# dayoladejo/GADMM

Measured on AMD Instinct MI355X. Metric: wall-clock to 1e-8 objective gap, GADMM linear regression (LinearRegression_Synthetic), lower is better.
Workload: dtype fp64; 1 GPU; model=LinearRegression_Synthetic GADMM closed-form, workers=24, features=50, samples_per_worker=50, global_batch=1200, seq_len=1, parallelism=chain24-over-1gpu

## Files before the change

csrc/kernels/chain_blocked.hip:

```cpp
#include "gadmm_common.h"
#include "gadmm_chain.h"
#include "persist_device.h"
#include "persist_launch.h"
#include <stdlib.h>

namespace {

constexpr int MAXW = 12;
constexpr int HIMG52 = 4 * 64 * 14;
constexpr int EPL = 256;
constexpr long DYN_LDS_BYTES = (long)MAXW * EPL * (16 + 8 + 4);
struct EpochLds {
  int4* sl;
  int2* fl;
  int* st;
};
__device__ __forceinline__ EpochLds epoch_lds(double* base, int v) {
  int4* sl = reinterpret_cast<int4*>(base);
  int2* fl = reinterpret_cast<int2*>(sl + MAXW * EPL);
  int* st = reinterpret_cast<int*>(fl + MAXW * EPL);
  return {sl + v * EPL, fl + v * EPL, st + v * EPL};
}

template <int QT>
__device__ __forceinline__ void quad_load_image(double (&m)[4][QT], const double* img) {
  const int lane = threadIdx.x & 63;
  const double2* p = reinterpret_cast<const double2*>(img) + lane;
#pragma unroll
  for (int t = 0; t < QT; t += 2)
#pragma unroll
    for (int r = 0; r < 4; ++r) {
      const double2 v = p[((t >> 1) * 4 + r) * 64];
      m[r][t] = v.x;
      if (t + 1 < QT) m[r][t + 1] = v.y;
    }
}

template <class PA>
__device__ __forceinline__ void stage_epochs(const PA& a, int q, const EpochLds& el, bool flush) {
  const int lane = threadIdx.x & 63;
  for (int e = lane; e < a.n_epochs; e += 64) {
    el.sl[e] = reinterpret_cast<const int4*>(a.ep_slots)[(long)e * a.n + q];
    if (flush) el.fl[e] = reinterpret_cast<const int2*>(a.ep_flush)[(long)e * a.n + q];
    el.st[e] = a.epoch_start[e];
  }
}
}



template <int QT, bool SYS, bool DYN = false, class PA = PersistArgs>
__device__ __forceinline__ void blocked_objective(const PA& a, double* lds, int v, int lane, int q,
                                                  unsigned long long deadline, __amdgpu_buffer_rsrc_t rob,
                                                  __amdgpu_buffer_rsrc_t rtab, bool local = false) {
  const int d = a.d, n = a.n;
  const long ring_base = 2L * n * 2 * d;
  const EpochLds el = epoch_lds(lds + MAXW * 64 + MAXW * QSTAGE, v);
  int* posl = reinterpret_cast<int*>(el.fl);
  if constexpr (DYN) {
    for (int e = lane; e < a.n_epochs; e += 64) {
      posl[e] = a.ep_pos[(long)e * n + q];
      el.st[e] = a.epoch_start[e];
    }
  }
  const PhaseSlot so = a.slots[DYN ? 0 : q];
  const int li = DYN ? q : so.li, gid = DYN ? q : so.gid;
  int row = DYN ? posl[0] : q;
  const bool in = lane < d;
  double Aq[4][QT];
  quad_load<QT>(Aq, a.A + (long)li * d * d, d, true);
  const double bo = in ? a.b[(long)li * d + lane] : 0.0;
  const double hy = 0.5 * a.yy[li];
  double* xo = lds + v * QSTAGE;
  int ep = 0, next_start = (DYN && a.n_epochs > 1) ? el.st[1] : 0x7fffffff;
  for (int it = a.start_iter;; ++it) {
    if (a.hard_stop > 0 && it > a.hard_stop) return;
    if constexpr (DYN) {
      if (it == next_start) {
        ++ep;
        next_start = ep + 1 < a.n_epochs ? el.st[ep + 1] : 0x7fffffff;
        row = posl[ep];
      }
    }
    const unsigned tag = make_tag(a.epoch, it);
    const long off = (ring_base + ((long)(it % a.ring) * n + row) * d + lane) * 16;
    double x = 0.0;
    for (int spin = 0;; ++spin) {
      const bool ok = !in || load_granule<SYS>(rtab, (int)off, tag, &x);
      if (__all(ok)) break;
      if ((spin & 7) == 7) {
        if (it - a.start_iter >= a.lag) {
          const unsigned long long dv = load_dec<SYS>(&a.decg[(it - a.lag) % a.ring]);
          if ((unsigned)(dv >> 32) == make_tag(a.epoch, it - a.lag) && (unsigned)(dv & 0xffffffffu) != 0u) return;
        }
        if (now_ticks() > deadline) return;
      }
      GADMM_POLL_PAUSE();
    }
    const double qv = quad_gemv<QT>(Aq, in ? x : 0.0, xo);
    const double part = in ? (0.5 * qv - bo) * x : 0.0;
    const double f = wave_sum_f64(part) + hy;
    if (lane == 0) put_granule<SYS>(local, rob, ((it % a.ring) * n + gid) * 16, tag, f);
  }
}

template <int DB, bool SYS, bool TL, bool DYN, bool HALO, bool SWEEP, class PA>
__device__ __forceinline__ void chain_blocked_body(const PA& a) {
  constexpr int QT = DB / 4;
  extern __shared__ __attribute__((aligned(16))) double lds[];
  __shared__ int abort_lds, stop_lds, stop_iter_lds;
  const int d = a.d, n = a.n;
  const int lane = threadIdx.x & 63;
  const int v = __builtin_amdgcn_readfirstlane(threadIdx.x >> 6);
  const int k = a.blk_k, L = a.blk_len, H = 2 * a.blk_k;
  const bool multi = a.nranks > 1;
  const int seg_lo = multi ? a.seg_lo : 0, seg_hi = multi ? a.seg_hi : n - 1;
  const int nseg = seg_hi - seg_lo + 1;
  const int W = (nseg + L - 1) / L;
  const int Wo = (nseg + MAXW - 1) / MAXW;
  const bool dl = SYS && multi && a.blk_dl != 0;
  const unsigned long long deadline = now_ticks() + (unsigned long long)a.timeout_ticks;
  const __amdgpu_buffer_rsrc_t rob = rsrc_of(a.objg);
  const __amdgpu_buffer_rsrc_t rtab = rsrc_of(a.blk_tab);
  const bool packed = SWEEP || (!SYS && a.xcd > 0);
  if (!SWEEP && packed && (blockIdx.x & 7u)) return;
  const int bid = packed ? (int)(blockIdx.x >> 3) : (int)blockIdx.x;
  if (SWEEP && bid > W + Wo) return;
  if (threadIdx.x == 0) {
    abort_lds = 0;
    stop_lds = 0;
  }
  lds_barrier();
  const long ring_base = 2L * n * 2 * d;
  const long etab_base = 2L * n * 2 * d + (long)a.ring * n * d;
  bool local = false;
  if (!SYS && a.xcd > 1) local = xcd_verdict(a.xchk, bid, W + Wo + 1, deadline, &stop_iter_lds, (unsigned)a.xtag);
  if (!SYS && bid == 0 && threadIdx.x == 0) a.ctl->placed = a.xcd > 0 ? (local ? 2 : 1) : 0;

  if (bid == W + Wo) {
    monitor_loop<SYS, GADMM_POLL_SLEEP>(a, lds, rob, deadline, a.start_iter, a.hard_stop,
                                        TL ? a.timeline + (long)bid * a.timeline_iters * 8 : nullptr, 8, v);
    return;
  }

  if (bid >= W) {
    const int q = seg_lo + (bid - W) * MAXW + v;
    if (q <= seg_hi) blocked_objective<QT, SYS, DYN>(a, lds, v, lane, q, deadline, rob, rtab, local);
    return;
  }

  const int g = bid;
  const int s0 = seg_lo + g * L, e0 = min(seg_hi + 1, s0 + L) - 1;
  const int hl = HALO && dl && seg_lo > 0 && (seg_lo % 2) == 1, hr = HALO && dl && seg_hi < n - 1 && (seg_hi % 2) == 1;
  const bool hosted = HALO && dl && (seg_hi - seg_lo + 1 + hl + hr > MAXW);
  const int hd = hosted ? (hr ? 1 : -1) : 0;
  const int hp = hd > 0 ? seg_hi + 1 : (hd < 0 ? seg_lo - 1 : 0);
  const int ra = max(dl ? seg_lo - (hosted ? 0 : hl) : 0, s0 - H), rb = min(dl ? seg_hi + (hosted ? 0 : hr) : n - 1, e0 + H);
  const int nv = rb - ra + 1;
  const int h0 = ra & 1;
  const int u = v < MAXW / 2 ? 2 * v + h0 : 2 * (v - MAXW / 2) + (1 - h0);
  const int p = ra + u;
  const bool active = u < nv;
  const bool owned = active && p >= s0 && p <= e0;
  PhaseSlot sl = DYN ? a.ep_slots[active ? p : 0] : a.slots[active ? p : 0];
  int li = sl.li, w = sl.gid;
  const bool has_l = active && sl.left >= 0, has_r = active && sl.right >= 0;
  const bool head = (p % 2) == 0;
  const int deg = (int)has_l + (int)has_r;
  const double rho = a.rho;
  const bool in = lane < d;
  int vdec = -1;
  for (int u = 0; u < nv && vdec < 0; ++u)
    if (((ra + u) % 2) == 0 && (ra + u < s0 || ra + u > e0)) vdec = u;
  if (vdec < 0 && nv < MAXW) vdec = nv;
  if (vdec < 0) vdec = (ra % 2 == 0) ? 0 : 1;
  const bool dec_wave = u == vdec;

  double* thS = lds;
  double* xs = thS + MAXW * 64;
  double* myx = xs + v * QSTAGE;
  const double* thL = thS + (u > 0 ? u - 1 : u) * 64;
  const double* thR = thS + (u + 1 < nv ? u + 1 : u) * 64;
  const bool nbl = has_l && u > 0, nbr = has_r && u + 1 < nv;
  const int hdir = (hosted && active && p == hp - hd) ? hd : 0;
  const int hq = (hosted && v >= MAXW / 2 && v < MAXW / 2 + 4) ? v - MAXW / 2 : -1;
  const bool rl = dl && has_l && p == ra && hdir != -1, rr = dl && has_r && p == rb && hdir != 1;
  const bool dlh = HALO && dl;
  const bool lb_tail = hl != 0, rb_tail = hr != 0;
  const bool pl = dlh ? (owned && !head && ((p == seg_lo && has_l) || (p == seg_lo + 1 && seg_lo > 0 && !lb_tail)))
                      : rl;
  const bool pr = dlh ? (owned && !head && ((p == seg_hi && has_r) || (p == seg_hi - 1 && seg_hi < n - 1 && !rb_tail)))
                      : rr;
  const bool rpush = dlh ? (pl || pr) : owned && (rl || rr);

  const EpochLds el = epoch_lds(lds + MAXW * 64 + MAXW * QSTAGE, v);
  if constexpr (DYN) {
    stage_epochs(a, active ? p : 0, el, active);
  }
  const int odist = u < s0 - ra ? (s0 - ra) - u : (u > e0 - ra ? u - (e0 - ra) : 0);
  const bool solver = active && odist <= (head ? 2 * k - 1 : 2 * k - 2);
  double Mq[4][QT];
  quad_load<QT>(Mq, a.Minv + ((long)li * a.nvar + a.deg_to_var[deg]) * (long)d * d, d, active);
  auto solve = [&](double r) -> double {
    const double y = quad_gemv<QT>(Mq, in ? r : 0.0, myx);
    return in ? y : 0.0;
  };
  double th = (active && in) ? a.theta[(long)w * d + lane] : 0.0;
  double mu = (active && in) ? a.mu[(long)li * d + lane] : 0.0;
  double bb = (active && in) ? a.b[(long)li * d + lane] : 0.0;
  thS[u * 64 + lane] = th;
  double* Mh = lds + MAXW * 64 + MAXW * QSTAGE;
  double* hst = Mh + HIMG52;
  bool hsl = false, hsr = false;
  if (HALO && hosted) {
    const PhaseSlot sh = a.slots[hp];
    hsl = sh.left >= 0;
    hsr = sh.right >= 0;
    if (hdir != 0) {
      const int deg_h = (int)hsl + (int)hsr;
      quad_store_lds<QT>(Mh, a.Minv + ((long)sh.li * a.nvar + a.deg_to_var[deg_h]) * (long)d * d, d, true);
      hst[lane] = in ? a.theta[(long)sh.gid * d + lane] : 0.0;
      hst[64 + (a.start_iter & 1) * 64 + lane] = in ? a.mu[(long)sh.li * d + lane] : 0.0;
      hst[192 + lane] = in ? a.b[(long)sh.li * d + lane] : 0.0;
    }
  }
  int pending = a.pending_in;
  int ep = 0, next_start = (DYN && a.n_epochs > 1) ? el.st[1] : 0x7fffffff;
  int next_x = a.start_iter + k, xc = 0;
  const int uo_lo = s0 - ra, uo_hi = e0 - ra;
  int blk0 = a.start_iter;
  if (threadIdx.x == 0) stop_iter_lds = 0;
  lds_barrier();

  auto publish = [&](int j) {
    const unsigned tag = make_tag(a.epoch, j + 1);
    const int sel = xc & 1;
    const int base = ((sel * n + p) * 2) * d;
    put_granule<SYS>(local, rtab, (base + lane) * 16, tag, th);
    put_granule<SYS>(local, rtab, (base + d + lane) * 16, tag, mu);
    for (int q = 0; q < a.blk_npeer; ++q)
      if (p >= a.blk_peer_lo[q] && p <= a.blk_peer_hi[q]) {
        const __amdgpu_buffer_rsrc_t rpe = rsrc_of(a.blk_peer_tab[q]);
        store_granule<SYS>(rpe, (base + lane) * 16, tag, th);
        store_granule<SYS>(rpe, (base + d + lane) * 16, tag, mu);
      }
  };
  unsigned long long dv_pref = 0;
  int it = a.start_iter;
  bool hard_stopped = false;
  long long ts[8] = {0, 0, 0, 0, 0, 0, 0, 0};
  const int ring_p = (int)((ring_base + (long)(active ? p : 0) * d + lane) * 16);
  const int ring_slot_bytes = n * d * 16;
  const bool ring_post = owned && in && !(TL && (a.dbg & 2));
  const int ring_l = (int)((ring_base + (long)(rl ? p - 1 : 0) * d + lane) * 16);
  const int ring_r = (int)((ring_base + (long)(rr ? p + 1 : 0) * d + lane) * 16);
  const __amdgpu_buffer_rsrc_t rdl0 = rsrc_of(pl && a.dl_tab[0] ? (const void*)a.dl_tab[0] : (const void*)a.blk_tab);
  const __amdgpu_buffer_rsrc_t rdl1 = rsrc_of(pr && a.dl_tab[1] ? (const void*)a.dl_tab[1] : (const void*)a.blk_tab);
  auto poll_remote = [&](int slot, int j, double& tl, double& tr) -> bool {
    const unsigned tag = make_tag(a.epoch, j);
    const int so = slot * ring_slot_bytes;
    for (int spin = 0;; ++spin) {
      bool g0 = true;
      if (in) {
        if (rl) g0 &= load_granule<SYS>(rtab, ring_l + so, tag, &tl);
        if (rr) g0 &= load_granule<SYS>(rtab, ring_r + so, tag, &tr);
      }
      if (__all(g0)) return true;
      if ((spin & 7) == 7 && now_ticks() > deadline) return false;
      GADMM_POLL_PAUSE();
    }
  };
  auto poll_far = [&](int slot, int j, double& tf) -> bool {
    const unsigned tag = make_tag(a.epoch, j);
    const int so = slot * ring_slot_bytes + (int)((ring_base + (long)(hp + hd) * d + lane) * 16);
    for (int spin = 0;; ++spin) {
      const bool g0 = !in || load_granule<SYS>(rtab, so, tag, &tf);
      if (__all(g0)) return true;
      if ((spin & 7) == 7 && now_ticks() > deadline) return false;
      GADMM_POLL_PAUSE();
    }
  };
  auto push_remote = [&](int slot, int j) {
    const unsigned tag = make_tag(a.epoch, j);
    const int off = ring_p + slot * ring_slot_bytes;
    if (pl) store_granule<SYS>(rdl0, off, tag, th);
    if (pr) store_granule<SYS>(rdl1, off, tag, th);
  };
  bool ring_defer = false;
  int rslot = a.start_iter % a.ring;
  int dslot = (a.start_iter + 1 - a.lag) % a.ring;
  if (dslot < 0) dslot += a.ring;
  for (;; ++it, rslot = rslot + 1 == a.ring ? 0 : rslot + 1, dslot = dslot + 1 == a.ring ? 0 : dslot + 1) {
    if (ring_defer) {
      put_granule<SYS>(local, rtab, ring_p + (rslot == 0 ? a.ring - 1 : rslot - 1) * ring_slot_bytes,
                       make_tag(a.epoch, it - 1), th);
      ring_defer = false;
    }
    if (it > a.max_iter + a.lag) break;
    if (a.hard_stop > 0 && it > a.hard_stop) {
      hard_stopped = true;
      break;
    }
    const bool stamp = TL && v == 0 && it - a.start_iter < a.timeline_iters;
    if (stamp) ts[0] = (long long)now_ticks();
    if constexpr (DYN) {
      if (it == next_start) {
        const unsigned tag = make_tag(a.epoch, it);
        const long eb = etab_base + (long)((ep + 1) & 1) * n * 2 * d;
        if (owned && in) {
          const long base = eb + (long)w * 2 * d;
          put_granule<SYS>(local, rtab, (int)((base + lane) * 16), tag, th);
          put_granule<SYS>(local, rtab, (int)((base + d + lane) * 16), tag, mu);
        }
        ++ep;
        next_start = ep + 1 < a.n_epochs ? el.st[ep + 1] : 0x7fffffff;
        if (active) {
          {
            const int4 s4 = el.sl[ep];
            sl.li = s4.x;
            sl.gid = s4.y;
          }
          const int2 of = el.fl[ep];
          li = sl.li;
          w = sl.gid;
          if (solver) {
            quad_load_image<QT>(Mq, a.minv_pad + ((long)li * a.nvar + a.deg_to_var[deg]) * (long)(512 * ((QT + 1) / 2)));
            bb = in ? a.b[(long)li * d + lane] : 0.0;
          }
          const bool fl = pending && of.x >= 0, fr = pending && of.y >= 0;
          double t0 = 0.0, t1 = 0.0, tl = 0.0, tr = 0.0;
          bool ok = true;
          for (int spin = 0;; ++spin) {
            bool g0 = true;
            if (in) {
              const long b0 = eb + (long)w * 2 * d;
              g0 &= load_granule<SYS>(rtab, (int)((b0 + lane) * 16), tag, &t0);
              g0 &= load_granule<SYS>(rtab, (int)((b0 + d + lane) * 16), tag, &t1);
              if (fl) g0 &= load_granule<SYS>(rtab, (int)((eb + (long)of.x * 2 * d + lane) * 16), tag, &tl);
              if (fr) g0 &= load_granule<SYS>(rtab, (int)((eb + (long)of.y * 2 * d + lane) * 16), tag, &tr);
            }
            if (__all(g0)) break;
            if ((spin & 7) == 7 && now_ticks() > deadline) {
              ok = false;
              break;
            }
            GADMM_POLL_PAUSE();
          }
          if (!ok && lane == 0) abort_lds = 1;
          th = in ? t0 : 0.0;
          double m = in ? t1 : 0.0;
          if (fl) m = m - rho * (tl - th);
          if (fr) m = m + rho * (th - tr);
          mu = in ? m : 0.0;
          thS[u * 64 + lane] = th;
        }
// ... 58 lines not shown
      if (has_l) r = r + rho * tl;
      if (has_r) r = r + rho * tr;
      if (stamp) ts[6] = (long long)now_ticks();
      th = solve(r);
      if (stamp) {
        asm volatile("" ::"v"(th));
        ts[7] = (long long)now_ticks();
      }
      if (rpush && in) push_remote(rslot, it);
      thS[u * 64 + lane] = th;
    }
    if (HALO && hq >= 0) {
      double tf = 0.0;
      if (hd > 0 ? hsr : hsl) {
        if (it == a.start_iter) {
          if (in) tf = a.theta[(long)(hp + hd) * d + lane];
        } else if (!poll_far(rslot == 0 ? a.ring - 1 : rslot - 1, it - 1, tf) && lane == 0) {
          abort_lds = 1;
        }
      }
      const double tn = thS[(hp - hd - ra) * 64 + lane];
      const double tl = hd > 0 ? tn : tf, tr = hd > 0 ? tf : tn;
      const double th_h = hst[lane];
      double m = hst[64 + (it & 1) * 64 + lane];
      if (pending) {
        if (hsl) m = m - rho * (tl - th_h);
        if (hsr) m = m + rho * (th_h - tr);
      }
      if (hq == 0) hst[64 + ((it + 1) & 1) * 64 + lane] = m;
      double r = hst[192 + lane] - m;
      if (hsl) r = r + rho * tl;
      if (hsr) r = r + rho * tr;
      hst[256 + hq * 64 + lane] = quad_rowgroup_lds<QT>(Mh, hq, in ? r : 0.0, myx);
    }
    pending = 1;
    lds_barrier();
    if (stamp) ts[4] = (long long)now_ticks();

    const bool xnext = !HALO && it + 1 == next_x && !(DYN && it + 1 == next_start);
    const bool tstamp = TL && v == MAXW / 2 + ((a.dbg >> 4) & 7) && it - a.start_iter < a.timeline_iters && g < 128;
    long long tt[4] = {0, 0, 0, 0};
    if (active && !head && u >= uo_lo - (slack - 1) && u <= uo_hi + (slack - 1)) {
      if (tstamp) tt[0] = (long long)now_ticks();
      double tl = nbl ? thL[lane] : 0.0, tr = nbr ? thR[lane] : 0.0;
      if (HALO && hdir != 0) {
        double pq[4] = {hst[256 + lane], hst[320 + lane], hst[384 + lane], hst[448 + lane]};
        const double y = quad_reduce(pq);
        const double th_h = in ? y : 0.0;
        hst[lane] = th_h;
        if (hdir > 0) tr = th_h;
        else tl = th_h;
      }
      if ((rl || rr) && !poll_remote(rslot, it, tl, tr) && lane == 0) abort_lds = 1;
      double r = bb - mu;
      if (has_l) r = r + rho * tl;
      if (has_r) r = r + rho * tr;
      if (tstamp) {
        asm volatile("" ::"v"(r));
        tt[1] = (long long)now_ticks();
      }
      const double tn = solve(r);
      if (tstamp) {
        asm volatile("" ::"v"(tn));
        tt[2] = (long long)now_ticks();
      }
      double m = mu;
      if (has_l) m = m - rho * (tl - tn);
      if (has_r) m = m + rho * (tn - tr);
      mu = m;
      th = tn;
      if (rpush && in) push_remote(rslot, it);
      thS[u * 64 + lane] = th;
      if (owned && in && xnext) publish(it);
      ring_defer = ring_post;
      if (a.rres && owned) {
        double rp = 0.0;
        if (in && has_l) rp = fma(tl - tn, tl - tn, rp);
        if (in && has_r) rp = fma(tn - tr, tn - tr, rp);
        const double rs = wave_sum_f64(rp);
        if (lane == 0 && it - 1 < a.max_iter) a.rres[(long)(it - 1) * n + w] = rs;
      }
      if (tstamp) tt[3] = (long long)now_ticks();
    } else if (active && owned && in) {
      if (xnext) publish(it);
      if (ring_post) put_granule<SYS>(local, rtab, ring_p + rslot * ring_slot_bytes, make_tag(a.epoch, it), th);
    }
    if (TL && g < 8 && it - a.start_iter < a.timeline_iters && lane == 0) {
      const long long t_end = (long long)now_ticks();
      a.timeline[((long)(160 + g * MAXW + v) * a.timeline_iters + (it - a.start_iter)) * 8] = t_end;
    }
    if (!(TL && (a.dbg & 1)) && dec_wave && !(active && !head) && lane == 0 && it + 1 - a.start_iter >= a.lag) {
      const int jdec = it + 1 - a.lag;
      const unsigned tj = make_tag(a.epoch, jdec);
      unsigned long long dv = dv_pref;
      if ((unsigned)(dv >> 32) != tj) dv = load_dec<SYS>(&a.decg[dslot]);
      for (int spin = 0; (unsigned)(dv >> 32) != tj; ++spin) {
        if ((spin & 7) == 7 && now_ticks() > deadline) {
          abort_lds = 1;
          break;
        }
        GADMM_POLL_PAUSE();
        dv = load_dec<SYS>(&a.decg[dslot]);
      }
      const unsigned code = (unsigned)(dv & 0xffffffffu);
      if (code && (unsigned)(dv >> 32) == tj) {
        stop_lds = (int)code;
        stop_iter_lds = jdec;
      }
      dv_pref = load_dec<SYS>(&a.decg[dslot + 1 == a.ring ? 0 : dslot + 1]);
    }
    lds_barrier();
    if (tstamp && lane == 0) {
      long long* tl = a.timeline + ((long)(128 + g) * a.timeline_iters + (it - a.start_iter)) * 8;
      for (int q = 0; q < 4; ++q) tl[q] = tt[q];
      tl[4] = (long long)now_ticks();
    }
    if (stamp && lane == 0) {
      long long* tl = a.timeline + ((long)g * a.timeline_iters + (it - a.start_iter)) * 8;
      for (int q = 0; q < 5; ++q) tl[q] = ts[q];
      tl[5] = (long long)now_ticks();
      tl[6] = ts[6];
      tl[7] = ts[7];
    }
    if (abort_lds || stop_lds) {
      ++it;
      break;
    }
  }

  if (ring_defer)
    put_granule<SYS>(local, rtab, ring_p + ((it - 1) % a.ring) * ring_slot_bytes, make_tag(a.epoch, it - 1), th);
  if (owned && in) {
    a.theta[(long)w * d + lane] = th;
    a.mu[(long)li * d + lane] = mu;
  }
  if (threadIdx.x == 0) {
    if (abort_lds) {
      a.ctl->done = 4;
    } else if (g == 0 && stop_lds) {
      a.ctl->done = stop_lds;
      a.ctl->conv_iter = stop_iter_lds;
      a.ctl->iter = it;
      a.ctl->pending = 1;
      a.ctl->monitored = stop_iter_lds;
    } else if (g == 0 && hard_stopped) {
      a.ctl->iter = it;
      a.ctl->pending = 1;
    }
  }
}

typedef __attribute__((address_space(4))) PersistArgs SweepArgs;

template <int DB, bool SYS, bool TL, bool DYN = false, bool HALO = false>
__global__ void __launch_bounds__(64 * MAXW) chain_blocked_kernel(PersistArgs a) {
  chain_blocked_body<DB, SYS, TL, DYN, HALO, false>(a);
}

template <int DB>
__global__ void __launch_bounds__(64 * MAXW) chain_blocked_sweep_kernel(const PersistArgs* __restrict__ batch, int nb) {
  const int j = (int)(blockIdx.x & 7u);
  if (j >= nb) return;
  chain_blocked_body<DB, false, false, false, false, true>(*(const SweepArgs*)(batch + j));
}

template <int DB>
__global__ void __launch_bounds__(64 * MAXW) chain_blocked_dyn_sweep_kernel(const PersistArgs* __restrict__ batch, int nb) {
  const int j = (int)(blockIdx.x & 7u);
  if (j >= nb) return;
  chain_blocked_body<DB, false, false, true, false, true>(*(const SweepArgs*)(batch + j));
}

constexpr int PWW = 8;
constexpr int PCAP = 2 * PWW;

template <int DB, bool SYS>
__global__ void __launch_bounds__(64 * PWW) chain_blocked_pair_kernel(PersistArgs a) {
  constexpr int QT = DB / 4;
  extern __shared__ __attribute__((aligned(16))) double lds[];
  __shared__ int abort_lds, stop_lds, stop_iter_lds;
  const int d = a.d, n = a.n;
  const int lane = threadIdx.x & 63;
  const int v = __builtin_amdgcn_readfirstlane(threadIdx.x >> 6);
  const int k = a.blk_k, L = a.blk_len, H = 2 * a.blk_k;
  const bool multi = a.nranks > 1;
  const int seg_lo = multi ? a.seg_lo : 0, seg_hi = multi ? a.seg_hi : n - 1;
  const int nseg = seg_hi - seg_lo + 1;
  const int W = (nseg + L - 1) / L;
  const int Wo = (nseg + PWW - 1) / PWW;
  const unsigned long long deadline = now_ticks() + (unsigned long long)a.timeout_ticks;
  const __amdgpu_buffer_rsrc_t rob = rsrc_of(a.objg);
  const __amdgpu_buffer_rsrc_t rtab = rsrc_of(a.blk_tab);
  if (threadIdx.x == 0) {
    abort_lds = 0;
    stop_lds = 0;
    stop_iter_lds = 0;
  }
  lds_barrier();
  if ((int)blockIdx.x == W + Wo) {
    monitor_loop<SYS, GADMM_POLL_SLEEP>(a, lds, rob, deadline, a.start_iter, a.hard_stop, nullptr, 0, v);
    return;
  }
  const long ring_base = 2L * n * 2 * d;
  if ((int)blockIdx.x >= W) {
    const int q = seg_lo + ((int)blockIdx.x - W) * PWW + v;
    if (q <= seg_hi) blocked_objective<QT, SYS>(a, lds, v, lane, q, deadline, rob, rtab);
    return;
  }

  const int g = blockIdx.x;
  const int s0 = seg_lo + g * L, e0 = min(seg_hi + 1, s0 + L) - 1;
  const int ra = max(0, s0 - H), rb = min(n - 1, e0 + H);
  const int nv = rb - ra + 1;
  const int uA = 2 * v;
  const bool aHead = ((ra + uA) & 1) == 0;
  const int uH = aHead ? uA : uA + 1, uT = aHead ? uA + 1 : uA;
  const bool actH = uH < nv, actT = uT < nv;
  const int pH = ra + uH, pT = ra + uT;
  const bool ownH = actH && pH >= s0 && pH <= e0, ownT = actT && pT >= s0 && pT <= e0;
  const PhaseSlot slH = a.slots[actH ? pH : 0], slT = a.slots[actT ? pT : 0];
  const bool hlH = actH && slH.left >= 0, hrH = actH && slH.right >= 0;
  const bool hlT = actT && slT.left >= 0, hrT = actT && slT.right >= 0;
  const double rho = a.rho;
  const bool in = lane < d;
  int vdec = 0;
  for (int vv = PWW - 1; vv >= 0; --vv) {
    const int pa = ra + 2 * vv, pb = pa + 1;
    if (2 * vv + 1 < nv && (pa < s0 || pa > e0) && (pb < s0 || pb > e0)) vdec = vv;
  }
  const bool dec_wave = v == vdec;

  double* thS = lds;
  double* bbS = thS + PCAP * 64;
  double* myx = bbS + PCAP * 64 + v * QSTAGE;
  const bool nblH = hlH && uH > 0, nbrH = hrH && uH + 1 < nv;
  const bool nblT = hlT && uT > 0, nbrT = hrT && uT + 1 < nv;

  double MH[3][QT], MT[3][QT], M3[QT];
  quad_load_pair<QT>(MH, MT, M3,
                     a.Minv + ((long)slH.li * a.nvar + a.deg_to_var[(int)hlH + (int)hrH]) * (long)d * d,
                     a.Minv + ((long)slT.li * a.nvar + a.deg_to_var[(int)hlT + (int)hrT]) * (long)d * d, d, actH,
                     actT);
  double thH = (actH && in) ? a.theta[(long)slH.gid * d + lane] : 0.0;
  double muH = (actH && in) ? a.mu[(long)slH.li * d + lane] : 0.0;
  double thT = (actT && in) ? a.theta[(long)slT.gid * d + lane] : 0.0;
  double muT = (actT && in) ? a.mu[(long)slT.li * d + lane] : 0.0;
  if (actH) {
    thS[uH * 64 + lane] = thH;
    bbS[uH * 64 + lane] = in ? a.b[(long)slH.li * d + lane] : 0.0;
  }
  if (actT) {
    thS[uT * 64 + lane] = thT;
    bbS[uT * 64 + lane] = in ? a.b[(long)slT.li * d + lane] : 0.0;
  }
  int pending = a.pending_in;
  lds_barrier();

  auto publish = [&](int j, int p, double th, double mu) {
    const unsigned tag = make_tag(a.epoch, j + 1);
    const int base = (((((j + 1 - a.start_iter) / k) & 1) * n + p) * 2) * d;
    store_granule<SYS>(rtab, (base + lane) * 16, tag, th);
    store_granule<SYS>(rtab, (base + d + lane) * 16, tag, mu);
    for (int q = 0; q < a.blk_npeer; ++q)
      if (p >= a.blk_peer_lo[q] && p <= a.blk_peer_hi[q]) {
        const __amdgpu_buffer_rsrc_t rpe = rsrc_of(a.blk_peer_tab[q]);
        store_granule<SYS>(rpe, (base + lane) * 16, tag, th);
        store_granule<SYS>(rpe, (base + d + lane) * 16, tag, mu);
      }
  };
  unsigned long long dv_pref = 0;
  int it = a.start_iter;
  for (;; ++it) {
    if (it > a.max_iter + a.lag) break;
    if (it > a.start_iter && (it - a.start_iter) % k == 0) {
      const bool needH = actH && !ownH, needT = actT && !ownT;
      if (needH || needT) {
        const unsigned tag = make_tag(a.epoch, it);
        const int bsel = ((it - a.start_iter) / k) & 1;
        const int baseH = ((bsel * n + pH) * 2) * d, baseT = ((bsel * n + pT) * 2) * d;
        double h0 = 0.0, h1 = 0.0, t0 = 0.0, t1 = 0.0;
        bool ok = true;
        for (int spin = 0;; ++spin) {
          bool g0 = true;
          if (in && needH) {
            g0 &= load_granule<SYS>(rtab, (baseH + lane) * 16, tag, &h0);
            g0 &= load_granule<SYS>(rtab, (baseH + d + lane) * 16, tag, &h1);
          }
          if (in && needT) {
            g0 &= load_granule<SYS>(rtab, (baseT + lane) * 16, tag, &t0);
            g0 &= load_granule<SYS>(rtab, (baseT + d + lane) * 16, tag, &t1);
          }
          if (__all(g0)) break;
          if ((spin & 7) == 7 && now_ticks() > deadline) {
            ok = false;
            break;
          }
          GADMM_POLL_PAUSE();
        }
        if (!ok && lane == 0) abort_lds = 1;
        if (needH) {
          thH = in ? h0 : 0.0;
          muH = in ? h1 : 0.0;
          thS[uH * 64 + lane] = thH;
        }
        if (needT) {
          thT = in ? t0 : 0.0;
          muT = in ? t1 : 0.0;
          thS[uT * 64 + lane] = thT;
        }
      }
      lds_barrier();
      if (abort_lds) break;
    }

    if (actH) {
      const double tl = nblH ? thS[(uH - 1) * 64 + lane] : 0.0, tr = nbrH ? thS[(uH + 1) * 64 + lane] : 0.0;
      double m = muH;
      if (pending) {
        if (hlH) m = m - rho * (tl - thH);
        if (hrH) m = m + rho * (thH - tr);
      }
      muH = m;
      double r = bbS[uH * 64 + lane] - m;
// ... 136 lines not shown
  if (pw == 1) {
    *pw_out = 1;
    return gadmm_chain_blocked_plan(n, d, want_k, k_out, len_out);
  }
  if (d > 52 || n < 2) return 0;
  int k = want_k > 0 ? want_k : 3;
  int len = PCAP - 4 * k;
  while (len < 1 && k > 1) {
    --k;
    len = PCAP - 4 * k;
  }
  if (len < 1) return 0;
  if (const char* e = getenv("GADMM_BLOCK_L")) {
    const int want_len = atoi(e);
    if (want_len >= 1 && want_len < len) len = want_len;
  }
  if (len > n) len = n;
  const int W = (n + len - 1) / len;
  if (W + (n + PWW - 1) / PWW + 1 > 256) return 0;
  *k_out = k;
  *len_out = len;
  *pw_out = 2;
  return W;
}

int gadmm_chain_blocked_pad_dim(int d) { return d <= 32 ? 32 : 52; }
long gadmm_chain_blocked_pad_len(int d) {
  const int qt = gadmm_chain_blocked_pad_dim(d) / 4;
  return 512L * ((qt + 1) / 2);
}
int gadmm_chain_blocked_max_epochs() { return EPL; }

int gadmm_pad_image_f64(const double* M, long mstride, const long long* src, long n_el, int batch, double* out,
                        hipStream_t st) {
  if (!M || !src || !out || n_el < 1 || batch < 1) {
    gadmm_set_error("pad_image: bad arguments");
    return -1;
  }
  const long tot = n_el * batch;
  const int grid = (int)((tot + 255) / 256 < 4096 ? (tot + 255) / 256 : 4096);
  hipLaunchKernelGGL(pad_image_kernel, dim3(grid), dim3(256), 0, st, M, mstride, src, n_el, batch, out);
  GADMM_CHECK(hipGetLastError());
  return 0;
}

int gadmm_chain_blocked_plan_dl(int nseg, int d, int want_k, int* k_out, int* len_out) {
  if (d > 52 || nseg < 1) return 0;
  const char* e = getenv("GADMM_DL_PLAN");
  const bool force_blocked = e && e[0] == 'b' && nseg >= 2;
  if (nseg <= MAXW && !force_blocked) {
    *k_out = 1 << 20;
    *len_out = nseg;
    return 1;
  }
  return gadmm_chain_blocked_plan(nseg, d, want_k, k_out, len_out);
}

long gadmm_chain_blocked_lds(int d, int len) {
  (void)d;
  (void)len;
  return (long)(MAXW * 64 + MAXW * QSTAGE) * 8;
}

long gadmm_chain_blocked_tab_granules(int n, int d, int ring) { return 2L * n * 2 * d + (long)ring * n * d; }
long gadmm_chain_blocked_tab_granules_dyn(int n, int d, int ring) { return 4L * n * 2 * d + (long)ring * n * d; }

int gadmm_chain_blocked_launch(const PersistArgs* args, hipStream_t st) {
  const PersistArgs& a = *args;
  const bool multi = a.nranks > 1;
  const bool dl = a.blk_dl != 0;
  if (dl) {
    const int nseg_dl = a.seg_hi - a.seg_lo + 1;
    const int W_dl = nseg_dl > 0 && a.blk_len > 0 ? (nseg_dl + a.blk_len - 1) / a.blk_len : 0;
    const int nhalo = a.dl_halo ? (int)(a.seg_lo > 0 && a.seg_lo % 2 == 1) + (int)(a.seg_hi < a.n - 1 && a.seg_hi % 2 == 1) : 0;
    const bool hosted_dl = a.dl_halo && nseg_dl + nhalo > MAXW;
    const long span = W_dl == 1 ? (hosted_dl ? nseg_dl : nseg_dl + nhalo) : (long)a.blk_len + 4L * a.blk_k;
    if (hosted_dl && (nhalo != 1 || nseg_dl < 8)) {
      gadmm_set_error("blocked chain kernel (data-local halo): a hosted halo needs one hosted side and >= 4 tails");
      return -1;
    }
    if (!multi || !a.sys_scope || a.blk_pw != 1 || a.n_epochs != 0 || a.blk_npeer != 0 || a.blk_k < 1 ||
        a.blk_len < 1 || nseg_dl < 1 || span > MAXW || (W_dl > 1 && a.ring < 2 * a.blk_k + 4) ||
        (a.seg_lo > 0 && !a.dl_tab[0]) || (a.seg_hi < a.n - 1 && !a.dl_tab[1]) ||
        (a.dl_halo && (W_dl != 1 || nseg_dl < 2 || a.d > 52))) {
      gadmm_set_error("blocked chain kernel (data-local): unsupported configuration (seg %d..%d, L=%d, k=%d)",
                      a.seg_lo, a.seg_hi, a.blk_len, a.blk_k);
      return -1;
    }
  }
  if (a.blk_k < 1 || a.blk_len < 1 || (!dl && a.blk_len + 4 * a.blk_k > (a.blk_pw == 2 ? PCAP : MAXW)) || a.d > 52 ||
      !a.blk_tab || !a.dec_push ||
      (!multi && (!a.has_monitor || a.n != a.n_local)) ||
      (multi && (a.seg_lo < 0 || a.seg_hi < a.seg_lo || a.seg_hi >= a.n || a.blk_npeer < 0 || a.blk_npeer > 8 ||
                 (a.blk_npeer > 0 && !a.blk_peer_tab) || a.start_iter != 1 || a.pending_in != 0 || !a.sys_scope))) {
    gadmm_set_error("blocked chain kernel: unsupported configuration");
    return -1;
  }
  if (a.lag < 1) {
    gadmm_set_error("blocked chain kernel: lag must be at least 1");
    return -1;
  }
  PersistArgs ka = a;
  void* kargs[] = {&ka};
  const int nseg = multi ? a.seg_hi - a.seg_lo + 1 : a.n;
  const int W = (nseg + a.blk_len - 1) / a.blk_len;
  if (a.blk_pw == 2 && a.n_epochs == 0) {
    if (a.blk_len + 4 * a.blk_k > PCAP || a.timeline) {
      gadmm_set_error("blocked chain kernel (pw=2): L + 4k > %d or timeline requested", PCAP);
      return -1;
    }
    const int Wo2 = (nseg + PWW - 1) / PWW;
    const int blocks2 = W + Wo2 + (a.has_monitor ? 1 : 0);
    long lds2 = (long)(2 * PCAP * 64 + PWW * QSTAGE) * 8;
    if (lds2 < (long)a.n * 8) lds2 = (long)a.n * 8;
    const void* fn2 = a.sys_scope ? (a.d <= 32 ? (const void*)chain_blocked_pair_kernel<32, true>
                                               : (const void*)chain_blocked_pair_kernel<52, true>)
                                  : (a.d <= 32 ? (const void*)chain_blocked_pair_kernel<32, false>
                                               : (const void*)chain_blocked_pair_kernel<52, false>);
    return gadmm_persist_launch({fn2, 64 * PWW, (size_t)lds2, blocks2, "blocked chain kernel", false}, &ka, kargs, st);
  }
  const int Wo = (nseg + MAXW - 1) / MAXW;
  const int blocks = W + Wo + (a.has_monitor ? 1 : 0);
  long lds = gadmm_chain_blocked_lds(a.d, a.blk_len);
  if (lds < (long)a.n * 8) lds = (long)a.n * 8;
  if (lds > 160 * 1024) {
    gadmm_set_error("blocked chain kernel: %ld B of LDS", lds);
    return -1;
  }
  const void* fn;
  const bool tl = a.timeline != nullptr;
  if (a.n_epochs > 0) {
    if (multi || tl || a.sys_scope || !a.epoch_start || !a.ep_slots || !a.ep_pos || !a.minv_pad || !a.ep_flush ||
        a.hard_stop < 0 || (a.hard_stop > 0 && a.hard_stop < a.start_iter) || a.n_epochs > EPL) {
      gadmm_set_error("blocked chain kernel: dynamic epochs need one GPU, epoch tables (at most %d epochs per "
                      "launch), the padded inverse image (gadmm_chain_blocked_pad_len), no timeline", EPL);
      return -1;
    }
    lds = gadmm_chain_blocked_lds(a.d, a.blk_len) + DYN_LDS_BYTES;
    fn = a.d <= 32 ? (const void*)chain_blocked_kernel<32, false, false, true>
                   : (const void*)chain_blocked_kernel<52, false, false, true>;
  } else if (a.sys_scope && dl && a.dl_halo) {
    if (tl) {
      gadmm_set_error("blocked chain kernel: no timeline build of the data-local halo mode");
      return -1;
    }
    fn = a.d <= 32 ? (const void*)chain_blocked_kernel<32, true, false, false, true>
                   : (const void*)chain_blocked_kernel<52, true, false, false, true>;
    lds += (long)(HIMG52 + 512) * 8;
  } else if (a.sys_scope) {
    if (tl) fn = a.d <= 32 ? (const void*)chain_blocked_kernel<32, true, true> : (const void*)chain_blocked_kernel<52, true, true>;
    else fn = a.d <= 32 ? (const void*)chain_blocked_kernel<32, true, false> : (const void*)chain_blocked_kernel<52, true, false>;
  } else {
    if (tl) fn = a.d <= 32 ? (const void*)chain_blocked_kernel<32, false, true> : (const void*)chain_blocked_kernel<52, false, true>;
    else fn = a.d <= 32 ? (const void*)chain_blocked_kernel<32, false, false> : (const void*)chain_blocked_kernel<52, false, false>;
  }
  {
    const char* e = getenv("GADMM_BLK_DBG");
    ka.dbg = e ? atoi(e) : 0;
  }
  return gadmm_persist_launch({fn, 64 * MAXW, (size_t)lds, blocks, "blocked chain kernel", true}, &ka, kargs, st);
}

int gadmm_chain_blocked_sweep_capacity() { return 8; }

int gadmm_chain_blocked_sweep_launch(const PersistArgs* batch, int nb, PersistArgs* host_stage, PersistArgs* dev_stage,
                                     hipStream_t st) {
  if (nb < 1 || nb > gadmm_chain_blocked_sweep_capacity()) {
    gadmm_set_error("blocked sweep: %d solves, one launch takes 1..%d", nb, gadmm_chain_blocked_sweep_capacity());
    return -1;
  }
  if (!batch || !host_stage || !dev_stage) {
    gadmm_set_error("blocked sweep: null batch or staging buffer");
    return -1;
  }
  int blocks[8], max_blocks = 0, sum_blocks = 0;
  long lds = gadmm_chain_blocked_lds(0, 0);
  for (int j = 1; j < nb; ++j)
    if ((batch[j].d <= 32) != (batch[0].d <= 32)) {
      gadmm_set_error("blocked sweep: solves of different register classes (d = %d and %d; d <= 32 or 33..52)",
                      batch[0].d, batch[j].d);
      return -1;
    }
  for (int j = 0; j < nb; ++j) {
    const PersistArgs& a = batch[j];
    if (a.nranks > 1 || a.sys_scope || a.n_epochs > 0 || a.blk_pw == 2 || a.timeline || a.blk_dl || a.dl_halo ||
        a.blk_npeer != 0 || a.hard_stop != 0 || a.cont) {
      gadmm_set_error("blocked sweep: solve %d is multi-rank, system-scope, dynamic, paired-wave, instrumented or "
                      "data-local (one-GPU static 12-wave solves only)", j);
      return -1;
    }
    if (!a.xchk) {
      gadmm_set_error("blocked sweep: solve %d has no placement-check buffer (xchk)", j);
      return -1;
    }
    if (a.blk_k < 1 || a.blk_len < 1 || a.blk_len + 4 * a.blk_k > MAXW || a.d < 1 || a.d > 52 || a.n < 2 ||
        !a.blk_tab || !a.dec_push || !a.objg || !a.decg || !a.ctl || !a.trace || !a.theta || !a.mu || !a.slots ||
        !a.Minv || !a.A || !a.b || !a.yy || !a.has_monitor || a.n != a.n_local) {
      gadmm_set_error("blocked sweep: solve %d: unsupported configuration", j);
      return -1;
    }
    if (a.lag < 1 || a.ring <= a.lag + 1 || a.start_iter + a.max_iter + a.lag >= (1 << 20)) {
      gadmm_set_error("blocked sweep: solve %d: ring/lag/tag range", j);
      return -1;
    }
    for (int i = 0; i < j; ++i) {
      const PersistArgs& o = batch[i];
      if (o.ctl == a.ctl || o.trace == a.trace || o.theta == a.theta || o.mu == a.mu || o.blk_tab == a.blk_tab ||
          o.objg == a.objg || o.decg == a.decg || o.xchk == a.xchk || (a.tstamp && o.tstamp == a.tstamp)) {
        gadmm_set_error("blocked sweep: solves %d and %d share a buffer that both write", i, j);
        return -1;
      }
    }
    const int W = (a.n + a.blk_len - 1) / a.blk_len, Wo = (a.n + MAXW - 1) / MAXW;
    blocks[j] = W + Wo + 1;
    if (blocks[j] > XCHK) {
      gadmm_set_error("blocked sweep: solve %d has %d workgroups, the placement check holds %d", j, blocks[j], XCHK);
      return -1;
    }
    sum_blocks += blocks[j];
    if (blocks[j] > max_blocks) max_blocks = blocks[j];
    if (lds < (long)a.n * 8) lds = (long)a.n * 8;
  }
  if (lds > 160 * 1024) {
    gadmm_set_error("blocked sweep: %ld B of LDS", lds);
    return -1;
  }
  const void* fn = batch[0].d <= 32 ? (const void*)chain_blocked_sweep_kernel<32> : (const void*)chain_blocked_sweep_kernel<52>;
  const long cap = gadmm_resident_capacity(fn, 64 * MAXW, (size_t)lds);
  const long cus_xcd = gadmm_cu_count() / 8;
  if (sum_blocks > cap) {
    gadmm_set_error("blocked sweep: %d workgroups but only %ld can be resident", sum_blocks, cap);
    return -2;
  }
  for (int j = 0; j < nb; ++j)
    if (blocks[j] > cus_xcd) {
      gadmm_set_error("blocked sweep: solve %d has %d workgroups but an XCD has %ld CUs", j, blocks[j], cus_xcd);
      return -2;
    }
  if (lds > 65536) GADMM_CHECK(hipFuncSetAttribute(fn, hipFuncAttributeMaxDynamicSharedMemorySize, (int)lds));
  int dbg = 0, xenv = -1;
  if (const char* e = getenv("GADMM_BLK_DBG")) dbg = atoi(e);
  if (const char* e = getenv("GADMM_XCD")) xenv = atoi(e);
  for (int j = 0; j < nb; ++j) {
    PersistArgs& ka = host_stage[j];
    ka = batch[j];
    ka.dbg = dbg;
    const int x = xenv >= 0 ? xenv : ka.xcd;
    ka.xcd = x >= 2 ? 2 : 1;
    ka.xtag = (int)gadmm_next_xtag();
  }
  GADMM_CHECK(hipMemcpyAsync(dev_stage, host_stage, (size_t)nb * sizeof(PersistArgs), hipMemcpyHostToDevice, st));
  const PersistArgs* dbatch = dev_stage;
  void* kargs[] = {&dbatch, &nb};
  GADMM_CHECK(hipLaunchKernel(fn, dim3(8 * max_blocks), dim3(64 * MAXW), kargs, (size_t)lds, st));
  GADMM_CHECK(hipGetLastError());
  return 0;
}

int gadmm_chain_blocked_dyn_sweep_launch(const PersistArgs* batch, int nb, PersistArgs* host_stage,
                                         PersistArgs* dev_stage, hipStream_t st) {
  if (nb < 1 || nb > gadmm_chain_blocked_sweep_capacity()) {
    gadmm_set_error("blocked dynamic sweep: %d solves, one launch takes 1..%d", nb, gadmm_chain_blocked_sweep_capacity());
    return -1;
  }
  if (!batch || !host_stage || !dev_stage) {
    gadmm_set_error("blocked dynamic sweep: null batch or staging buffer");
    return -1;
  }
  int blocks[8], max_blocks = 0, sum_blocks = 0;
  long lds = gadmm_chain_blocked_lds(0, 0) + DYN_LDS_BYTES;
  for (int j = 1; j < nb; ++j)
    if ((batch[j].d <= 32) != (batch[0].d <= 32)) {
      gadmm_set_error("blocked dynamic sweep: solves of different register classes (d = %d and %d; d <= 32 or "
                      "33..52)", batch[0].d, batch[j].d);
      return -1;
    }
  for (int j = 0; j < nb; ++j) {
    const PersistArgs& a = batch[j];
    if (a.n_epochs < 1) {
      gadmm_set_error("blocked dynamic sweep: solve %d is static (no epochs): it belongs in the static sweep", j);
      return -1;
    }
    if (a.nranks > 1 || a.sys_scope || a.blk_pw == 2 || a.timeline || a.blk_dl || a.dl_halo || a.blk_npeer != 0) {
      gadmm_set_error("blocked dynamic sweep: solve %d is multi-rank, system-scope, paired-wave, instrumented or "
                      "data-local (one-GPU 12-wave solves only)", j);
      return -1;
    }
    if (a.n_epochs > EPL) {
      gadmm_set_error("blocked dynamic sweep: solve %d has %d epochs, a launch stages at most %d", j, a.n_epochs, EPL);
      return -1;
    }
    if (!a.epoch_start || !a.ep_slots || !a.ep_pos || !a.ep_flush || !a.minv_pad) {
      gadmm_set_error("blocked dynamic sweep: solve %d lacks epoch tables or the padded inverse image "
                      "(gadmm_chain_blocked_pad_len)", j);
      return -1;
    }
    if (a.hard_stop < 0 || (a.hard_stop > 0 && a.hard_stop < a.start_iter)) {
      gadmm_set_error("blocked dynamic sweep: solve %d: hard stop %d before its start %d", j, a.hard_stop, a.start_iter);
      return -1;
    }
    if (!a.xchk) {
      gadmm_set_error("blocked dynamic sweep: solve %d has no placement-check buffer (xchk)", j);
      return -1;
    }
    if (a.blk_k < 1 || a.blk_len < 1 || a.blk_len + 4 * a.blk_k > MAXW || a.d < 1 || a.d > 52 || a.n < 2 ||
        !a.blk_tab || !a.dec_push || !a.objg || !a.decg || !a.ctl || !a.trace || !a.theta || !a.mu || !a.slots ||
// ... 67 lines not shown
```

csrc/kernels/gram.hip:

```cpp
#include <stdlib.h>
#include "gadmm_common.h"

namespace {

constexpr int BK = 16;
constexpr int PAD = 16;

__device__ __forceinline__ void tri_of(int t, int& ti, int& tj) {
  ti = (int)((sqrt(8.0 * t + 1.0) - 1.0) * 0.5);
  while ((ti + 1) * (ti + 2) / 2 <= t) ++ti;
  while (ti * (ti + 1) / 2 > t) --ti;
  tj = t - ti * (ti + 1) / 2;
}

__device__ __forceinline__ void tile_of(int tile, int nt, int ST, int& ti, int& tj) {
  if (ST <= 1 || nt <= ST) {
    tri_of(tile, ti, tj);
    return;
  }
  const int nbr = (nt + ST - 1) / ST;
  int base = 0;
  for (int I = 0; I < nbr; ++I) {
    const int rows = (I + 1) * ST <= nt ? ST : nt - I * ST;
    const int rlo = I * ST;
    const int in_row = rows * rlo + rows * (rows + 1) / 2;
    if (tile >= base + in_row) {
      base += in_row;
      continue;
    }
    const int off = tile - base;
    const int full = I * ST * rows;
    if (off < full) {
      const int J = off / (rows * ST), o = off % (rows * ST);
      ti = rlo + o / ST;
      tj = J * ST + o % ST;
    } else {
      int a, b;
      tri_of(off - full, a, b);
      ti = rlo + a;
      tj = rlo + b;
    }
    return;
  }
  ti = tj = 0;
}

template <int BT, int NT>
struct GramTile {
  static constexpr int NWAVE = NT / 64;
  static constexpr int WR = NWAVE / 2;
  static constexpr int WTR = BT / WR;
  static constexpr int WTC = BT / 2;
  static constexpr int TMR = WTR / 16;
  static constexpr int TMC = WTC / 16;
  static constexpr int LDSROW = BT + PAD;
  static constexpr int PER_THREAD = BK * BT / NT;
};

template <int BT, int NT, bool DIAG, bool CLAMP>
__device__ __forceinline__ void gram_slabs(const double* __restrict__ H, const double* __restrict__ yv, int d,
                                           long kbeg, long kend, long nfull, int row0, int col0,
                                           double (*lds)[2 * BK * GramTile<BT, NT>::LDSROW],
                                           f64x4 (&acc)[GramTile<BT, NT>::TMR][GramTile<BT, NT>::TMC]) {
  using T = GramTile<BT, NT>;
  const int tid = threadIdx.x, lane = tid & 63, wid = tid >> 6;
  const int wr = wid >> 1, wc = wid & 1;
  double ri[T::PER_THREAD], rj[T::PER_THREAD];
  auto fetch_in = [&](long k0) {
#pragma unroll
    for (int p = 0; p < T::PER_THREAD / 2; ++p) {
      const int e2 = tid + NT * p;
      const int r = e2 / (BT / 2), c = (e2 % (BT / 2)) * 2;
      const double* src = H + (k0 + r) * (long)d;
      ri[2 * p] = src[row0 + c];
      ri[2 * p + 1] = src[row0 + c + 1];
      if constexpr (!DIAG) {
        rj[2 * p] = src[col0 + c];
        rj[2 * p + 1] = src[col0 + c + 1];
      }
    }
  };
  auto fetch_cl = [&](long k0) {
#pragma unroll
    for (int p = 0; p < T::PER_THREAD / 2; ++p) {
      const int e2 = tid + NT * p;
      const int r = e2 / (BT / 2), c = (e2 % (BT / 2)) * 2;
      const long k = k0 + r;
      const long kk = k < kend ? k : (kend - 1);
      const double yk = yv[kk];
      const bool kin = k < kend;
#pragma unroll
      for (int q = 0; q < 2; ++q) {
        const int ca = row0 + c + q, cb = col0 + c + q;
        const double va = H[kk * d + (ca < d ? ca : d - 1)];
        ri[2 * p + q] = kin ? (ca < d ? va : (ca == d ? yk : 0.0)) : 0.0;
        if constexpr (!DIAG) {
          const double vb = H[kk * d + (cb < d ? cb : d - 1)];
          rj[2 * p + q] = kin ? (cb < d ? vb : (cb == d ? yk : 0.0)) : 0.0;
        }
      }
    }
  };
  double yr[CLAMP ? T::PER_THREAD / 2 : 1];
  long kraw = 0;
  auto fetch_raw = [&](long k0) {
    kraw = k0;
#pragma unroll
    for (int p = 0; p < T::PER_THREAD / 2; ++p) {
      const int e2 = tid + NT * p;
      const int r = e2 / (BT / 2), c = (e2 % (BT / 2)) * 2;
      const long k = k0 + r;
      const long kk = k < kend ? k : (kend - 1);
      yr[p] = yv[kk];
#pragma unroll
      for (int q = 0; q < 2; ++q) {
        const int ca = row0 + c + q, cb = col0 + c + q;
        ri[2 * p + q] = H[kk * d + (ca < d ? ca : d - 1)];
        if constexpr (!DIAG) rj[2 * p + q] = H[kk * d + (cb < d ? cb : d - 1)];
      }
    }
  };
  auto select_raw = [&]() {
#pragma unroll
    for (int p = 0; p < T::PER_THREAD / 2; ++p) {
      const int e2 = tid + NT * p;
      const int r = e2 / (BT / 2), c = (e2 % (BT / 2)) * 2;
      const bool kin = kraw + r < kend;
#pragma unroll
      for (int q = 0; q < 2; ++q) {
        const int ca = row0 + c + q, cb = col0 + c + q;
        ri[2 * p + q] = kin ? (ca < d ? ri[2 * p + q] : (ca == d ? yr[p] : 0.0)) : 0.0;
        if constexpr (!DIAG) rj[2 * p + q] = kin ? (cb < d ? rj[2 * p + q] : (cb == d ? yr[p] : 0.0)) : 0.0;
      }
    }
  };
  auto stash = [&](int buf) {
    if constexpr (CLAMP) select_raw();
    double* Si = lds[buf];
    double* Sj = lds[buf] + BK * T::LDSROW;
#pragma unroll
    for (int p = 0; p < T::PER_THREAD / 2; ++p) {
      const int e2 = tid + NT * p;
      const int r = e2 / (BT / 2), c = (e2 % (BT / 2)) * 2;
      *reinterpret_cast<double2*>(Si + r * T::LDSROW + c) = make_double2(ri[2 * p], ri[2 * p + 1]);
      if constexpr (!DIAG) *reinterpret_cast<double2*>(Sj + r * T::LDSROW + c) = make_double2(rj[2 * p], rj[2 * p + 1]);
    }
  };
  auto mma = [&](int buf) {
    const double* Ci = lds[buf];
    const double* Cb = DIAG ? Ci : lds[buf] + BK * T::LDSROW;
#pragma unroll
    for (int ks = 0; ks < BK / 4; ++ks) {
      const int kr = ks * 4 + (lane >> 4);
      double a[T::TMR], b[T::TMC];
#pragma unroll
      for (int t = 0; t < T::TMR; ++t) a[t] = Ci[kr * T::LDSROW + wr * T::WTR + t * 16 + (lane & 15)];
#pragma unroll
      for (int t = 0; t < T::TMC; ++t) b[t] = Cb[kr * T::LDSROW + wc * T::WTC + t * 16 + (lane & 15)];
#pragma unroll
      for (int x = 0; x < T::TMR; ++x)
#pragma unroll
        for (int yq = 0; yq < T::TMC; ++yq)
          acc[x][yq] = __builtin_amdgcn_mfma_f64_16x16x4f64(a[x], b[yq], acc[x][yq], 0, 0, 0);
    }
  };

  auto fetch = [&](long k0) {
    if constexpr (CLAMP) fetch_raw(k0);
    else fetch_in(k0);
  };
  int cur = 0;
  long k0 = kbeg;
  if (nfull > 0) {
    fetch(k0);
    stash(0);
    lds_barrier();
    for (long s = 1; s < nfull; ++s) {
      fetch(k0 + BK);
      mma(cur);
      stash(cur ^ 1);
      lds_barrier();
      cur ^= 1;
      k0 += BK;
    }
    mma(cur);
    lds_barrier();
    cur ^= 1;
    k0 += BK;
  }
  for (; k0 < kend; k0 += BK) {
    if constexpr (CLAMP) fetch_raw(k0);
    else fetch_cl(k0);
    stash(cur);
    lds_barrier();
    mma(cur);
    cur ^= 1;
  }
}

template <int BT, int NT>
__global__ void __launch_bounds__(NT)
gram_aug_kernel(const double* __restrict__ X, const double* __restrict__ Y, int m, int d,
                int ntiles, int ksplit, long rows_per_split,
                double* __restrict__ A, double* __restrict__ B, double* __restrict__ YY,
                double* __restrict__ slab, int nt, int ST) {
  using T = GramTile<BT, NT>;
  __shared__ __attribute__((aligned(16))) double lds[2][2 * BK * T::LDSROW];

  const int nwg = gridDim.x;
  const int gid = xcd_remap(blockIdx.x, nwg);
  const int tile = gid % ntiles;
  const int rest = gid / ntiles;
  const int split = rest % ksplit;
  const int n = rest / ksplit;

  int ti, tj;
  tile_of(tile, nt, ST, ti, tj);
  const bool diag = (ti == tj);
  const int row0 = ti * BT, col0 = tj * BT;

  const double* H = X + (long)n * m * d;
  const double* yv = Y + (long)n * m;
  const long kbeg = (long)split * rows_per_split;
  long kend = kbeg + rows_per_split;
  if (kend > m) kend = m;

  const int tid = threadIdx.x, lane = tid & 63, wid = tid >> 6;
  const int wr = wid >> 1, wc = wid & 1;
  const int D = d + 1;

  f64x4 acc[T::TMR][T::TMC];
#pragma unroll
  for (int a = 0; a < T::TMR; ++a)
#pragma unroll
    for (int b = 0; b < T::TMC; ++b) acc[a][b] = f64x4{0.0, 0.0, 0.0, 0.0};

  const bool cols_in = (row0 + BT <= d) && (diag || col0 + BT <= d);
  const long nfull = kend > kbeg ? (kend - kbeg) / BK : 0;
  if (kbeg < kend) {
    if (cols_in) {
      if (diag) gram_slabs<BT, NT, true, false>(H, yv, d, kbeg, kend, nfull, row0, col0, lds, acc);
      else gram_slabs<BT, NT, false, false>(H, yv, d, kbeg, kend, nfull, row0, col0, lds, acc);
    } else {
      if (diag) gram_slabs<BT, NT, true, true>(H, yv, d, kbeg, kend, nfull, row0, col0, lds, acc);
      else gram_slabs<BT, NT, false, true>(H, yv, d, kbeg, kend, nfull, row0, col0, lds, acc);
    }
  }

#pragma unroll
  for (int x = 0; x < T::TMR; ++x)
#pragma unroll
    for (int yq = 0; yq < T::TMC; ++yq)
#pragma unroll
      for (int reg = 0; reg < 4; ++reg) {
        const int lr = wr * T::WTR + x * 16 + (lane >> 4) + 4 * reg;
        const int lc = wc * T::WTC + yq * 16 + (lane & 15);
        const double v = acc[x][yq][reg];
        if (ksplit > 1) {
          slab[(((long)n * ntiles + tile) * ksplit + split) * (BT * BT) + lr * BT + lc] = v;
          continue;
        }
        const int r = row0 + lr, c = col0 + lc;
        if (r >= D || c >= D || c > r) continue;
        if (r < d && c < d) {
          double* An = A + (long)n * d * d;
          An[(long)r * d + c] = v;
          An[(long)c * d + r] = v;
        } else if (r == d && c < d) {
          B[(long)n * d + c] = v;
        } else if (r == d && c == d) {
          YY[n] = v;
        }
      }
}

template <int BT>
__global__ void __launch_bounds__(256)
gram_reduce_kernel(const double* __restrict__ slab, int d, int ntiles, int ksplit,
                   double* __restrict__ A, double* __restrict__ B, double* __restrict__ YY, int nt, int ST) {
  const int tile = blockIdx.x, n = blockIdx.y;
  int ti, tj;
  tile_of(tile, nt, ST, ti, tj);
  const int D = d + 1;
  const double* s = slab + ((long)n * ntiles + tile) * ksplit * (BT * BT);
  for (int e = threadIdx.x; e < BT * BT; e += blockDim.x) {
    const int lr = e / BT, lc = e % BT;
    const int r = ti * BT + lr, c = tj * BT + lc;
    if (r >= D || c >= D || c > r) continue;
    double v = 0.0;
    for (int k = 0; k < ksplit; ++k) v += s[(long)k * BT * BT + e];
    if (r < d && c < d) {
      double* An = A + (long)n * d * d;
      An[(long)r * d + c] = v;
      An[(long)c * d + r] = v;
    } else if (r == d && c < d) {
      B[(long)n * d + c] = v;
    } else if (r == d && c == d) {
      YY[n] = v;
    }
  }
}

template <int BT>
int launch_gram(const double* X, const double* Y, int N, int m, int d, int ksplit, double* A,
                double* B, double* YY, double* slab, hipStream_t st) {
  const int D = d + 1;
  const int nt = (D + BT - 1) / BT;
  const int ntiles = nt * (nt + 1) / 2;
  if (ksplit < 1) ksplit = 1;
  long rows = ((long)m + ksplit - 1) / ksplit;
  rows = ((rows + BK - 1) / BK) * BK;
  ksplit = (int)(((long)m + rows - 1) / rows);
  if (ksplit < 1) ksplit = 1;
  const long nwg = (long)ntiles * ksplit * N;
  static const int nt_env = getenv("GADMM_GRAM_NT") ? atoi(getenv("GADMM_GRAM_NT")) : 0;
  const int nthr = nt_env == 256 || nt_env == 512 ? nt_env : (BT == 128 ? 512 : 256);
  const int ST = 0;
  if (nthr == 512)
    hipLaunchKernelGGL((gram_aug_kernel<BT, 512>), dim3((unsigned)nwg), dim3(512), 0, st, X, Y, m, d, ntiles, ksplit,
                       rows, A, B, YY, slab, nt, ST);
  else
    hipLaunchKernelGGL((gram_aug_kernel<BT, 256>), dim3((unsigned)nwg), dim3(256), 0, st, X, Y, m, d, ntiles, ksplit,
                       rows, A, B, YY, slab, nt, ST);
  if (ksplit > 1) {
    hipLaunchKernelGGL(gram_reduce_kernel<BT>, dim3(ntiles, N), dim3(256), 0, st, slab, d, ntiles,
                       ksplit, A, B, YY, nt, ST);
  }
  GADMM_CHECK(hipGetLastError());
  return 0;
}

}

extern "C" {

long gadmm_gram_workspace(int N, int m, int d, int ksplit) {
  if (ksplit <= 1) return 0;
  const int BT = (d + 1 <= 64) ? 64 : 128;
  const int nt = (d + 1 + BT - 1) / BT;
  return (long)N * (nt * (nt + 1) / 2) * ksplit * BT * BT;
}

int gadmm_gram_pick_ksplit(int N, int m, int d) {
  const int BT = (d + 1 <= 64) ? 64 : 128;
  const int nt = (d + 1 + BT - 1) / BT;
  const long tiles = (long)N * (nt * (nt + 1) / 2);
  int cus = gadmm_cu_count();
  if (cus <= 0) cus = 256;
  const long slots = (long)cus * 2;
  long maxk = (m + 255) / 256;
  if (maxk > 64) maxk = 64;
  if (maxk < 1) maxk = 1;
  static const double target = getenv("GADMM_GRAM_EFF") ? atof(getenv("GADMM_GRAM_EFF")) : 0.97;
  long best = 1;
  double best_eff = 0.0;
  for (long k = 1; k <= maxk; ++k) {
    const long W = tiles * k;
    const long rounds = (W + slots - 1) / slots;
    const double eff = (double)W / (double)(rounds * slots);
    if (eff > best_eff + 1e-9) {
      best_eff = eff;
      best = k;
    }
    if (eff >= target && W >= slots) {
      best = k;
      break;
    }
  }
  return (int)best;
}

int gadmm_gram_f64(const double* X, const double* Y, int N, int m, int d, int ksplit, double* A,
                   double* B, double* YY, double* slab, hipStream_t st) {
  if (N <= 0 || m <= 0 || d <= 0) return 0;
  if (ksplit > 1 && slab == nullptr) {
    gadmm_set_error("gram: ksplit=%d needs a workspace", ksplit);
    return -1;
  }
  if (d + 1 <= 64) return launch_gram<64>(X, Y, N, m, d, ksplit, A, B, YY, slab, st);
  return launch_gram<128>(X, Y, N, m, d, ksplit, A, B, YY, slab, st);
}

}
```

csrc/kernels/spd_inverse.hip:

```cpp
#include "gadmm_common.h"
#include <stdlib.h>

namespace {

__global__ void __launch_bounds__(1024)
spd_inverse_gj_kernel(const double* __restrict__ A, const double* __restrict__ shift, int d,
                      int nvar, double* __restrict__ out, int* __restrict__ status) {
  extern __shared__ __attribute__((aligned(16))) double M[];
  __shared__ double piv_s;
  const int n = blockIdx.x, v = blockIdx.y;
  const double s = shift[n * nvar + v];
  const double* An = A + (long)n * d * d;
  const int dd = d * d;
  for (int e = threadIdx.x; e < dd; e += blockDim.x) {
    const int i = e / d, j = e % d;
    M[e] = An[e] + (i == j ? s : 0.0);
  }
  __syncthreads();
  for (int k = 0; k < d; ++k) {
    if (threadIdx.x == 0) {
      const double pk = M[k * d + k];
      if (!(pk > 0.0) && status) atomicExch(status, 1);
      piv_s = 1.0 / pk;
    }
    __syncthreads();
    const double p = piv_s;
    for (int j = threadIdx.x; j < d; j += blockDim.x)
      if (j != k) M[k * d + j] *= p;
    __syncthreads();
    for (int e = threadIdx.x; e < dd; e += blockDim.x) {
      const int i = e / d, j = e % d;
      if (i != k && j != k) M[e] -= M[i * d + k] * M[k * d + j];
    }
    __syncthreads();
    for (int i = threadIdx.x; i < d; i += blockDim.x) M[i * d + k] = (i == k) ? p : -M[i * d + k] * p;
    __syncthreads();
  }
  double* o = out + ((long)n * nvar + v) * dd;
  for (int e = threadIdx.x; e < dd; e += blockDim.x) {
    const int i = e / d, j = e % d;
    o[e] = 0.5 * (M[e] + M[j * d + i]);
  }
}

__global__ void __launch_bounds__(256)
spd_inverse_gj64_kernel(const double* __restrict__ A, const double* __restrict__ shift, int d, int nvar,
                        double* __restrict__ out, int* __restrict__ status) {
  __shared__ double M[64 * 64];
  __shared__ double piv_s;
  const int n = blockIdx.x, v = blockIdx.y;
  const double s = shift[n * nvar + v];
  const double* An = A + (long)n * d * d;
  const int j = threadIdx.x & 63, rb = threadIdx.x >> 6;
  const bool inj = j < d;
  for (int i = rb; i < d; i += 4)
    if (inj) M[i * d + j] = An[i * d + j] + (i == j ? s : 0.0);
  __syncthreads();
  for (int k = 0; k < d; ++k) {
    if (rb == 0) {
      const double pk = M[k * d + k];
      const double p = 1.0 / pk;
      if (j == 0) {
        if (!(pk > 0.0) && status) atomicExch(status, 1);
        piv_s = p;
      }
      if (inj && j != k) M[k * d + j] *= p;
    }
    __syncthreads();
    const double p = piv_s;
    const double mkj = inj ? M[k * d + j] : 0.0;
    double aik[16];
#pragma unroll
    for (int q = 0; q < 16; ++q) {
      const int i = rb + 4 * q;
      aik[q] = i < d ? M[i * d + k] : 0.0;
    }
#pragma unroll
    for (int q = 0; q < 16; ++q) {
      const int i = rb + 4 * q;
      if (i < d && inj) {
        if (j == k) M[i * d + k] = (i == k) ? p : -aik[q] * p;
        else if (i != k) M[i * d + j] -= aik[q] * mkj;
      }
    }
    __syncthreads();
  }
  double* o = out + ((long)n * nvar + v) * d * d;
  for (int i = rb; i < d; i += 4)
    if (inj) o[i * d + j] = 0.5 * (M[i * d + j] + M[j * d + i]);
}

__device__ __forceinline__ double readlane_f64(double v, int l) {
  const long long b = __double_as_longlong(v);
  const int lo = __builtin_amdgcn_readlane((int)b, l), hi = __builtin_amdgcn_readlane((int)(b >> 32), l);
  return __longlong_as_double(((long long)hi << 32) | (unsigned)lo);
}

template <int NW>
__global__ void __launch_bounds__(64 * NW)
spd_inverse_reg64_kernel(const double* __restrict__ A, const double* __restrict__ shift, int d, int nvar,
                         double* __restrict__ out, int* __restrict__ status) {
  constexpr int NC = 64 / NW;
  __shared__ double Ms[64 * 65];
  __shared__ double colv[2][65];
  const int n = blockIdx.x, v = blockIdx.y;
  const double s = shift[n * nvar + v];
  const double* An = A + (long)n * d * d;
  const int i = threadIdx.x & 63, w = threadIdx.x >> 6;
  double h[NC];
#pragma unroll
  for (int c = 0; c < NC; ++c) {
    const int j = w + NW * c;
    h[c] = (i < d && j < d) ? An[i * d + j] + (i == j ? s : 0.0) : 0.0;
  }
  if (w == 0) {
    colv[0][i] = h[0];
    const double p0 = 1.0 / readlane_f64(h[0], 0);
    if (i == 0) colv[0][64] = p0;
  }
  __syncthreads();
  bool bad = false;
  for (int k = 0; k < d; ++k) {
    const double* cb = colv[k & 1];
    const double pk = cb[k], aik = cb[i], p = cb[64];
    bad |= !(pk > 0.0);
#pragma unroll
    for (int c = 0; c < NC; ++c) {
      const int j = w + NW * c;
      const double mkj = readlane_f64(h[c], k) * p;
      double val = h[c];
      if (j == k) val = (i == k) ? p : -aik * p;
      else if (i == k) val = mkj;
      else val -= aik * mkj;
      h[c] = val;
    }
    const int kn = k + 1;
    if (kn < d && w == kn % NW) {
      double nxt = 0.0;
#pragma unroll
      for (int c = 0; c < NC; ++c) nxt = (c == kn / NW) ? h[c] : nxt;
      colv[kn & 1][i] = nxt;
      const double pn = 1.0 / readlane_f64(nxt, kn);
      if (i == 0) colv[kn & 1][64] = pn;
    }
    __syncthreads();
  }
  if (threadIdx.x == 0 && bad && status) atomicExch(status, 1);
#pragma unroll
  for (int c = 0; c < NC; ++c) Ms[i * 65 + w + NW * c] = h[c];
  __syncthreads();
  double* o = out + ((long)n * nvar + v) * d * d;
  for (int r = w; r < d; r += NW)
    if (i < d) o[r * d + i] = 0.5 * (Ms[r * 65 + i] + Ms[i * 65 + r]);
}

}

extern "C" int gadmm_spd_inverse_small_f64(const double* A, const double* shift, int N, int d, int nvar,
                                           double* out, int* status, hipStream_t st) {
  if (d > 128) {
    gadmm_set_error("spd_inverse_small: d=%d > 128 (use the blocked path)", d);
    return -1;
  }
  if (N <= 0) return 0;
  const char* gje = getenv("GADMM_GJ64");
  const bool gj64 = !(gje && gje[0] == '0');
  const char* rge = getenv("GADMM_INV_REG");
  const bool reg = !(rge && rge[0] == '0');
  if (d <= 64 && gj64 && reg) {
    hipLaunchKernelGGL(spd_inverse_reg64_kernel<8>, dim3(N, nvar), dim3(512), 0, st, A, shift, d, nvar, out, status);
    GADMM_CHECK(hipGetLastError());
    return 0;
  }
  if (d <= 64 && gj64) {
    hipLaunchKernelGGL(spd_inverse_gj64_kernel, dim3(N, nvar), dim3(256), 0, st, A, shift, d, nvar, out, status);
    GADMM_CHECK(hipGetLastError());
    return 0;
  }
  const size_t lds = (size_t)d * d * sizeof(double);
  const int threads = d <= 32 ? 256 : 1024;
  if (lds > 65536)
    GADMM_CHECK(hipFuncSetAttribute((const void*)spd_inverse_gj_kernel,
                                    hipFuncAttributeMaxDynamicSharedMemorySize, (int)lds));
  hipLaunchKernelGGL(spd_inverse_gj_kernel, dim3(N, nvar), dim3(threads), lds, st, A, shift, d, nvar, out,
                     status);
  GADMM_CHECK(hipGetLastError());
  return 0;
}

#include "quad_gemv.h"

namespace {
template <int T>
__global__ void __launch_bounds__(64) quad_gemv_test_kernel(const double* M, const double* x, double* y, int rows,
                                                            int cols) {
  __shared__ __attribute__((aligned(16))) double st[QSTAGE];
  const int b = blockIdx.x, lane = threadIdx.x;
  const double* Mb = M + (long)b * rows * cols;
  double m[4][T];
  const int i = lane & 15, c = lane >> 4;
#pragma unroll
  for (int r = 0; r < 4; ++r)
#pragma unroll
    for (int t = 0; t < T; ++t) {
      const int row = i + 16 * r, col = c + 4 * t;
      m[r][t] = (row < rows && col < cols) ? Mb[(long)row * cols + col] : 0.0;
    }
  const double xv = lane < cols ? x[(long)b * cols + lane] : 0.0;
  const double v = quad_gemv<T>(m, xv, st);
  if (lane < rows) y[(long)b * rows + lane] = v;
}
}

extern "C" int gadmm_quad_gemv_test(const double* M, const double* x, double* y, int batch, int rows, int cols,
                                    hipStream_t st) {
  if (rows < 1 || rows > 64 || cols < 1 || cols > 64 || batch < 1) {
    gadmm_set_error("quad_gemv_test: rows/cols must be in [1, 64]");
    return -1;
  }
  if (cols <= 32) hipLaunchKernelGGL(quad_gemv_test_kernel<8>, dim3(batch), dim3(64), 0, st, M, x, y, rows, cols);
  else if (cols <= 52) hipLaunchKernelGGL(quad_gemv_test_kernel<13>, dim3(batch), dim3(64), 0, st, M, x, y, rows, cols);
  else hipLaunchKernelGGL(quad_gemv_test_kernel<16>, dim3(batch), dim3(64), 0, st, M, x, y, rows, cols);
  GADMM_CHECK(hipGetLastError());
  return 0;
}
```

gadmm_amd/algorithms/gadmm.py:

```python
from __future__ import annotations

import time
from typing import List, Optional, Sequence

import numpy as np
import torch

from ..parallel.comm import Comm, LocalComm
from ..parallel.topology import rechain_iterations, PathSchedule, Placement, chain_plan
from .base import global_objective_and_residual, RunResult, Stopper, total_bytes, global_objective, run_bytes
from ..utils import timing as _timing
from ..utils.timing import roctx_range
from ..utils.env import getenv


def _gather_rows(theta: torch.Tensor, ids: List[int]) -> torch.Tensor:
    idx = torch.tensor([max(i, 0) for i in ids], dtype=torch.long, device=theta.device)
    rows = theta.index_select(0, idx)
    mask = torch.tensor([1.0 if i >= 0 else 0.0 for i in ids], dtype=theta.dtype, device=theta.device)
    return rows * mask.unsqueeze(-1), mask


def chain_admm(model, local_ids: Sequence[int], n_total: int, rho: float, obj0: float, tol: float,
               max_iter: int, comm: Optional[Comm] = None, placement: Optional[Placement] = None,
# ... 349 lines not shown
        if native.available():
            with roctx_range("%s native-Q N=%d b=%d" % (name, n_total, bits)):
                return _chain_admm_native_quant(model, local_ids, n_total, rho, obj0, tol, max_iter, placement,
                                                schedule, cost_quirk, name, engine_opts or {}, bits, seed)
        if backend == "native":
            raise RuntimeError("native backend requested but unavailable for this comm/device")
        why = "native library unavailable"
    elif backend == "native":
        raise RuntimeError("Q-GADMM: the native backend does not cover this case (%s)" % why)
    res = _chain_admm_torch(model, local_ids, n_total, rho, obj0, tol, max_iter, comm, placement, schedule,
                            local_solver, step, max_inner, inner_tol, cost_quirk, name, record_theta, state,
                            check_exchange, failures, quantize=(bits, seed))
    res.extra["quant_fallback"] = why
    return res


def _chain_admm_native_quant(model, local_ids, n_total, rho, obj0, tol, max_iter, placement, schedule, cost_quirk,
                             name, opts, bits, seed) -> RunResult:
    from ..engine.chain_engine import NativeChainEngine, ResidencyError, HandoffTimeout
    from . import quantize as Q

    d = model.d
    block = int(opts.get("block", 32))
    key = ("quant", n_total, tuple(map(int, local_ids)), float(rho), int(max_iter), block, bits, seed,
           int(opts.get("xcd", 2)))
    cache = getattr(model, "_chain_engines", None)
    eng = cache.get(key) if cache is not None else None
    if eng is None:
        eng = NativeChainEngine(model.X, model.y, local_ids, n_total, "linear", rho=rho, obj0=obj0, tol=tol,
                                max_iter=max_iter, block=block, precomputed=(model.A, model.b, model.yy),
                                xcd=int(opts.get("xcd", 2)), quant=(bits, seed))
        if opts.get("cache", True):
            if cache is None:
                cache = {}
                model._chain_engines = cache
            cache[key] = eng
    else:
        eng.set_targets(obj0, tol)
    eng.set_path(schedule.path, placement, 0)
    eng.reset()
    torch.cuda.synchronize(model.device)
    t0 = time.perf_counter()
    r = None
    kernel = None
    engine_kind = None
    if opts.get("persistent", "auto") in (True, "auto") and eng.persistent_q_eligible():
        try:
            r = eng.run_persistent(fetch_trace=True)
            engine_kind, kernel = "persistent", eng.last_kernel
        except (ResidencyError, HandoffTimeout) as e:
            eng.reset()
            engine_kind = "graph(fallback: %s)" % type(e).__name__
    if r is None:
        r = eng.run(use_graph=opts.get("graph", True))
        kernel = "graph-Q"
        if engine_kind is None:
            engine_kind = "graph" if eng.graph_ok() else "eager"
        eng.stream.synchronize()
    wall = time.perf_counter() - t0
    iters, done = int(r.iters), int(r.done)
    tr, tt = eng.traces(iters)
    per = float(np.sum(schedule.cost)) * ((n_total + 1) // 2 if cost_quirk else 1)
    G = Q.granules_per_row(d, bits)
    res = RunResult(algorithm=name, obj=tr, loss=np.abs(tr - obj0), iters=iters, converged=(done == 1), wall_s=wall,
                    time_trace=tt, comm_units=np.arange(1, iters + 1, dtype=np.float64) * n_total,
                    com_cost=np.arange(1, iters + 1) * per, bytes_sent=0, bytes_total=0, primal_res=None,
                    extra={"backend": "native", "engine": engine_kind, "kernel": kernel, "rank": 0, "nranks": 1,
                           "solver": "closed", "monitor_bytes": 0, "wire_bytes": 0, "transport": "local",
                           "obj_mode": eng.obj_mode_name, "engine_obj": eng, "q_granules": G,
                           "q_wire_bytes": iters * n_total * G * 16,
                           "placed": int(getattr(eng, "last_placed", 0)) if engine_kind == "persistent" else 0})
    _quant_accounting(res, bits, seed, n_total, d)
    return res


_RECHAINS: dict = {}


def _rechains(max_iter: int, coherence) -> np.ndarray:
    key = (int(max_iter), float(coherence))
    r = _RECHAINS.get(key)
    if r is None:
        r = rechain_iterations(max_iter, coherence)
        r.setflags(write=False)
        if len(_RECHAINS) < 64:
            _RECHAINS[key] = r
    return r


def _max_epochs(eng) -> int:
    v = eng.__dict__.get("_max_epochs")
    if v is None:
        v = eng._max_epochs = int(eng.lib.gadmm_chain_blocked_max_epochs())
    return v


def _dyn_early_draw(eng, schedule, max_iter, fabric, n_total):
    if not eng.dynamic_eligible(fabric):
        return None
    rechains = _rechains(max_iter, schedule.coherence)
    if len(rechains) >= (1 << 20):
        return None
    hints = eng.__dict__.get("_dyn_epoch_hint", {})
    hk = (float(schedule.coherence), schedule.kind, int(max_iter), int(n_total))
    chunk = max(16, int(hints[hk]) + 8) if hk in hints else 128
    if eng.dynamic_uses_blocked(fabric, schedule.coherence):
        chunk = min(chunk, _max_epochs(eng) - 1)
    E_total = 1 + len(rechains)
    e1 = min(chunk, E_total)
    look = e1 if e1 < E_total else e1 - 1
    if look <= 0:
        return None
    saved = schedule.save()
    join = schedule.prefetch_async(look)
    if join is None:
        return None
    return saved, look, join


def _static_schedule(schedule, max_iter) -> bool:
    return not schedule.coherence or not np.isfinite(schedule.coherence) or schedule.coherence <= 0 \
        or schedule.coherence >= max_iter + 1


def _chain_admm_native(model, local_ids, n_total, rho, obj0, tol, max_iter, comm, placement, schedule, local_solver,
                       step, max_inner, inner_tol, cost_quirk, name, opts, state=None):
    from ..engine.chain_engine import NativeChainEngine, ResidencyError, HandoffTimeout

    _timing.host_stamp("native:start")
    rank = comm.rank
    rcomm = comm if comm.nranks > 1 else None
    fabric = opts.get("fabric")
    kind = "linear" if local_solver == "closed" else "logistic"
    block = int(opts.get("block", 16 if comm.nranks > 1 else (8 if kind == "logistic" else 32)))
    pre = (model.A, model.b, model.yy) if kind == "linear" else None
    key = (kind, local_solver, n_total, tuple(map(int, local_ids)), float(rho), int(max_iter), block,
           float(step), int(max_inner), float(inner_tol), float(getattr(model, "lam", 0.0)),
           opts.get("chord"), bool(opts.get("residual", True)))
    cache = getattr(model, "_chain_engines", None) if rcomm is None else None
    eng = cache.get(key) if cache is not None else None
    fresh = eng is None
    refresh = bool(opts.get("refresh", False)) and kind == "linear"
    if eng is None and refresh:
        from ..ops.linalg import gram
        gram(model.X, model.y, out=(model.A, model.b, model.yy))
    early = None
    if eng is not None and state is None and not _static_schedule(schedule, max_iter) \
            and opts.get("persistent", "auto") in (True, "auto") and "epoch_chunk" not in opts \
            and getenv("GADMM_DGADMM_EARLY", "1") != "0":
        early = _dyn_early_draw(eng, schedule, max_iter, fabric, n_total)
        _timing.host_stamp("native:early_draw")
    try:
        if eng is not None and refresh:
            eng.refresh(model.X, model.y)
            _timing.host_stamp("native:refresh")
        if eng is None:
            eng = NativeChainEngine(model.X, model.y, local_ids, n_total, kind, rho=rho, obj0=obj0, tol=tol,
                                    max_iter=max_iter, lam=getattr(model, "lam", 0.0), step=step, max_inner=max_inner,
                                    inner_tol=inner_tol, comm=rcomm, block=block, precomputed=pre,
                                    local_solver="newton" if local_solver == "newton" else "gd",
                                    chord=None if opts.get("chord") is None else float(opts["chord"]),
                                    residual=bool(opts.get("residual", True)),
                                    obj_mode=str(opts.get("obj_mode", "auto")))
            if rcomm is None and opts.get("cache", True):
                if cache is None:
                    cache = {}
                    model._chain_engines = cache
                cache[key] = eng
        else:
            eng.set_targets(obj0, tol)
        _timing.host_stamp("native:engine")
        eng.set_path(schedule.path, placement, rank)
        _timing.host_stamp("native:set_path")
        start = 1 if state is None else int(state[2])
        static = _static_schedule(schedule, max_iter)
        if state is not None and not (static and comm.nranks == 1):
            raise ValueError("native resume: one rank, static chain")

        def load_state():
            eng.reset(start_iter=start)
            if state is not None:
                eng.stream.wait_stream(torch.cuda.current_stream(model.device))
                with torch.cuda.stream(eng.stream):
                    eng.theta.copy_(state[0].to(eng.theta.device, torch.float64).reshape(eng.theta.shape))
                    eng.mu.copy_(state[1].to(eng.mu.device, torch.float64).reshape(eng.mu.shape))

        load_state()
        _timing.host_stamp("native:reset")
        stop_iter = int(opts.get("stop_iter", 0))
        if fresh or state is not None:
            torch.cuda.synchronize(model.device)
    except BaseException:
        if early is not None:
            early[2]()
            schedule.restore(early[0])
        raise
    if fabric is not None and comm.nranks > 1:
        import torch.distributed as dist
        elig = opts.get("persistent", "auto") in (True, "auto") and (
            eng.persistent_eligible(fabric) if static else eng.dynamic_eligible(fabric))
        t = torch.tensor([0.0 if elig else 1.0], dtype=torch.float64)
        dist.all_reduce(t, group=getattr(comm, "control_group", None))
        if float(t.item()) != 0.0:
            eng.close()
            fb = opts.get("fallback_comm")
            if fb is None:
                raise RuntimeError("%s: the xGMI kernel is not eligible on some rank and no data-plane "
                                   "fallback was given" % name)
            o2 = {k: v for k, v in opts.items() if k not in ("fabric", "fallback_comm")}
            res = _chain_admm_native(model, local_ids, n_total, rho, obj0, tol, max_iter, fb, placement, schedule,
                                     local_solver, step, max_inner, inner_tol, cost_quirk, name, o2, state=state)
            res.extra["fabric_fallback"] = "xgmi kernel not eligible on some rank: %s" % getattr(fb, "backend", "")
            return res
    t0 = time.perf_counter()
    cc = 0.0
    com_cost = []
    n_heads = (n_total + 1) // 2
    p2p = 0
    mon = 0
    wire = 0
    want_persistent = opts.get("persistent", "auto") in (True, "auto")
    if static:
        r = None
        engine_kind = None
        if want_persistent and stop_iter <= 0 and eng.persistent_eligible(fabric):
            try:
                r = eng.run_persistent(fabric=fabric, start_iter=start, fetch_trace=True)
                engine_kind = "persistent"
            except (ResidencyError, HandoffTimeout) as e:
                if comm.nranks > 1:
                    raise
                load_state()
                engine_kind = "graph(fallback: %s)" % type(e).__name__
        if r is None:
            r = eng.run(stop_iter=stop_iter, use_graph=opts.get("graph", True))
            if engine_kind is None:
                engine_kind = "graph" if eng.graph_ok() else "eager"
        iters, done = r.iters, r.done
        p2p, mon, wire = r.p2p_bytes, r.monitor_bytes, r.wire_bytes
        per = float(np.sum(schedule.cost)) * (n_heads if cost_quirk else 1)
        com_cost = np.arange(1, iters - start + 2) * per
        if local_solver == "newton" and not opts.get("_exact_retry"):
            fails = int(eng.ctl[7].item())
            chord_used = eng.chord_persistent if engine_kind == "persistent" else eng.chord
            if comm.nranks > 1:
                import torch.distributed as dist
                t = torch.tensor([float(fails)], dtype=torch.float64)
                dist.all_reduce(t, group=getattr(comm, "control_group", None))
                fails = int(t.item())
            if fails > 0 and chord_used > 0.0:
                res2 = _chain_admm_native(model, local_ids, n_total, rho, obj0, tol, max_iter, comm, placement,
                                          schedule, local_solver, step, max_inner, inner_tol, cost_quirk, name,
                                          dict(opts, chord=0.0, cache=False, _exact_retry=fails), state=state)
                res2.extra["chord_fallback"] = "%d unconverged chord-Newton local solves: re-run exact" % fails
                return res2
    elif want_persistent and eng.dynamic_eligible(fabric) \
            and len(_rechains(max_iter, schedule.coherence)) < (1 << 20):
        engine_kind = "persistent-dynamic"
        rechains = _rechains(max_iter, schedule.coherence)
        hint_key = (float(schedule.coherence), schedule.kind, int(max_iter), int(n_total))
        hints = eng.__dict__.setdefault("_dyn_epoch_hint", {})
        if "epoch_chunk" in opts:
            chunk = max(1, int(opts["epoch_chunk"]))
        elif hint_key in hints:
            chunk = max(16, int(hints[hint_key]) + 8)
        else:
            chunk = 128
        use_blk = eng.dynamic_uses_blocked(fabric, schedule.coherence)
        cap = _max_epochs(eng) - 1 if use_blk else 1 << 30
        chunk = min(chunk, cap)
        saved = early[0] if early is not None else schedule.save()
        E_total = 1 + len(rechains)
        Pall = np.empty((E_total, n_total), dtype=np.int64)
        Pall[0] = saved[1]
        ep_start = np.concatenate([np.ones(1, dtype=np.int64), rechains])
        drawn_C = []
        n_drawn = [1]

        pend = [early]

        def ensure(upto):
            need = upto + 1 - n_drawn[0]
            if pend[0] is not None:
                e_ = pend[0]
                pend[0] = None
                if n_drawn[0] == 1 and need >= e_[1]:
                    Pn_, Cn_ = e_[2]()
                    Pall[1:1 + e_[1]] = Pn_
                    n_drawn[0] += e_[1]
                    drawn_C.append(Cn_)
                    need -= e_[1]
                else:
                    e_[2]()
                    schedule.restore(e_[0])
            if need > 0:
                Pn_, Cn_ = schedule.prefetch_arrays(need)
                Pall[n_drawn[0]:n_drawn[0] + need] = Pn_
                n_drawn[0] += need
                drawn_C.append(Cn_)

        e0, start_iter, pending_in, cont = 0, 1, 0, False
        done = iters = 0
        last_launched = 0
        pre = {}
        ep_all = ep_start

        def cost_arrays():
# ... 453 lines not shown
```

gadmm_amd/engine/chain_engine.py:

```python
from __future__ import annotations

import ctypes
from dataclasses import dataclass
from typing import List, Optional, Sequence

import numpy as np
import torch

from ..ops import native
from ..utils import timing as _timing
from ..ops.linalg import gram, spd_inverse, sym_pack
from ..parallel.topology import Placement, chain_plan, RankPlan
from ..utils.env import getenv


class ResidencyError(RuntimeError):
    """A persistent kernel's workgroups cannot all be resident on this device at once."""


class HandoffTimeout(RuntimeError):
    """A persistent kernel's hand-off spin passed its deadline (done == 4) on some workgroup."""


@dataclass
# ... 116 lines not shown
        if force_monitor:
            if comm is None:
                raise ValueError("force_monitor needs a communicator")
            self.nranks = 2
        self.block = int(block)
        self.ring = max(self.block, 1)
        self.stream = stream if stream is not None else torch.cuda.Stream(self.device)
        self.stream.wait_stream(torch.cuda.current_stream(self.device))
        self.rho, self.obj0, self.tol, self.max_iter = float(rho), float(obj0), float(tol), int(max_iter)
        dev, f64 = self.device, torch.float64
        d, nl = self.d, self.n_local

        with torch.cuda.stream(self.stream):
            self.theta = torch.zeros((self.n_total, d), dtype=f64, device=dev)
            self.mu = torch.zeros((nl, d), dtype=f64, device=dev)
            self.objw = torch.zeros((nl,), dtype=f64, device=dev)
            mi = self.max_iter
            self._rb = torch.zeros((8 + 2 * mi,), dtype=f64, device=dev)
            self.ctl = self._rb[0:4].view(torch.int32)
            self.t0stamp = self._rb[4:5].view(torch.int64)
            self.trace = self._rb[8:8 + mi]
            self.trace.fill_(float("nan"))
            self.part = torch.zeros((self.ring * self.n_total,), dtype=f64, device=dev)
            self.reduced = torch.zeros((self.ring * self.n_total,), dtype=f64, device=dev)
            self.lgid = torch.tensor(self.local_ids, dtype=torch.int32, device=dev)
            self.tstamp = self._rb[8 + mi:8 + 2 * mi].view(torch.int64)
            self.slots = torch.zeros((max(2 * nl, 2) * 4,), dtype=torch.int32, device=dev)
            self.inner_iters = torch.zeros((max(nl, 1),), dtype=torch.int32, device=dev)
            self.A = self.b = self.yy = self.Minv = None
            self.X = self.Y = None
            self.rbuf = None
            self.hinv = torch.zeros((nl, 64 * 64 + 8), dtype=f64, device=dev) \
                if local_solver == "newton" and nl > 0 else None
            self.newton_img = torch.zeros((max(nl, 1) * int(native.require().gadmm_newton_rec_scratch_doubles()),),
                                          dtype=f64, device=dev) if local_solver == "newton" and nl > 0 else None
            self.chord = 0.02 if chord is None else float(chord)
            self.chord_persistent = 0.3 if chord is None else float(chord)
            self.xcd = int(xcd)
            self.rres = torch.zeros((self.max_iter * self.n_total,), dtype=f64, device=dev) if residual else None
            self.theta_true = self.q_msg = None
            if self.quant is not None:
                self.theta_true = torch.zeros((nl, d), dtype=f64, device=dev)
                self.q_msg = torch.zeros((self.n_total, 1 + self.q_words), dtype=torch.int64, device=dev)
            if d > 256:
                stride = int(native.require().gadmm_chain_big_rbuf_stride(d))
                self.rbuf = torch.zeros((max(nl, 1) * stride,), dtype=f64, device=dev)
            elif local_solver == "newton" and getenv("GADMM_NEWTON_TL") == "1":
                self.rbuf = torch.zeros((max(nl, 1) * 50 * 5,), dtype=torch.int64, device=dev)
            if model == "linear":
                if precomputed is not None:
                    self.A, self.b, self.yy = precomputed
                else:
                    self.A, self.b, self.yy = gram(X_loc, y_loc)
                self._shared_inverses = inverses is not None
                if inverses is not None:
                    self.Minv, self.nvar, self.deg_to_var = inverses[0], int(inverses[1]), tuple(inverses[2])
                    self._minv_version = 1
                else:
                    self._build_inverses()
            elif model == "logistic":
                self.X = X_loc.contiguous()
                self.Y = y_loc.contiguous()
                self.nvar, self.deg_to_var = 1, (0, 0, 0)
            else:
                raise ValueError("unknown model %r" % model)

        args = native.PhaseArgs()
        args.d, args.n_local = d, nl
        args.nvar = self.nvar if model == "linear" else 1
        for i, v in enumerate(self.deg_to_var if model == "linear" else (0, 0, 0)):
            args.deg_to_var[i] = v
        args.model = native.MODEL_LINEAR if model == "linear" else native.MODEL_LOGISTIC
        args.Minv = native.ptr(self.hinv if self.hinv is not None else self._kernel_minv())
        args.A = native.ptr(self.A)
        args.b = native.ptr(self.b)
        args.yy = native.ptr(self.yy)
        args.mu = self.mu.data_ptr()
        args.theta = self.theta.data_ptr()
        args.rho = self.rho
        args.objw = self.objw.data_ptr()
        args.ctl = self.ctl.data_ptr()
        args.trace = self.trace.data_ptr()
        args.part = self.part.data_ptr()
        args.ring = self.ring
        args.max_iter = self.max_iter
        args.obj0, args.tol = self.obj0, self.tol
        args.X = native.ptr(self.X)
        args.Y = native.ptr(self.Y)
        args.m = self.m
        args.max_inner = int(max_inner)
        args.lam, args.step, args.inner_tol = float(lam), float(step), float(inner_tol)
        if local_solver == "newton":
            args.step = self.chord
        args.inner_iters = self.inner_iters.data_ptr()
        args.rbuf = native.ptr(self.rbuf)
        if obj_mode not in ("auto", "exact", "identity"):
            raise ValueError("unknown obj_mode %r" % obj_mode)
        args.obj_mode = 0 if (obj_mode == "exact" or (obj_mode == "auto" and d <= 256)) else 1
        self.obj_mode_name = "exact" if args.obj_mode == 0 else "identity"
        args.solver = 1 if local_solver == "newton" else 0
        args.n_total = self.n_total
        args.lgid = self.lgid.data_ptr()
        args.tstamp = self.tstamp.data_ptr()
        args.rres = native.ptr(self.rres)
        if self.quant is not None:
            args.q_bits, args.q_seed = self.quant
            args.q_true, args.q_msg = self.theta_true.data_ptr(), self.q_msg.data_ptr()
        desc = native.EngineDesc()
        desc.base = args
        desc.d_slots = self.slots.data_ptr()
        desc.reduced = self.reduced.data_ptr()
        desc.comm = comm.handle if comm is not None else None
        desc.stream = self.stream.cuda_stream
        desc.nranks = self.nranks
        desc.xport = self.xport
        self._desc = desc
        self.handle = self.lib.gadmm_chain_engine_create(ctypes.byref(desc))
        if not self.handle:
            native.check(-1, "chain_engine_create")
        self.plan: Optional[RankPlan] = None
        self.path: Optional[List[int]] = None
        self._pbuf = None

    def _build_inverses(self, in_place: bool = False, check: bool = True):
        self._minv_version = getattr(self, "_minv_version", 0) + 1
        rho = self.rho
        if self.n_total == 1:
            shifts, self.deg_to_var = [0.0], (0, 0, 0)
        elif self.n_total == 2:
            shifts, self.deg_to_var = [rho], (0, 0, 0)
        else:
            shifts, self.deg_to_var = [rho, 2.0 * rho], (0, 0, 1)
        self.nvar = len(shifts)
        key = (tuple(shifts), self.A.shape[0])
        if getattr(self, "_shift_key", None) != key or not in_place:
            self._refresh_fast = None
        if getattr(self, "_shift_key", None) != key:
            self._shift_key = key
            self._shifts = torch.tensor(shifts, dtype=torch.float64, device=self.device).unsqueeze(0).expand(
                self.A.shape[0], -1).contiguous()
            self._inv_status = torch.zeros((1,), dtype=torch.int32, device=self.device)
        st = None if check else self._inv_status
        if in_place and self.Minv is not None:
            spd_inverse(self.A, self._shifts, out=self.Minv, check_status=check, status=st)
        else:
            self.Minv = spd_inverse(self.A, self._shifts, check_status=check, status=st)
        if self.d > 256:
            self.Mpk = sym_pack(self.Minv, out=self.Mpk if in_place and getattr(self, "Mpk", None) is not None
                                else None)

    def _kernel_minv(self):
        return getattr(self, "Mpk", None) if self.d > 256 else self.Minv

    def refresh(self, X_loc: torch.Tensor, y_loc: torch.Tensor):
        if getattr(self, "_shared_inverses", False):
            raise RuntimeError("this engine's inverses belong to a shared table: refresh its owner")
        fast = getattr(self, "_refresh_fast", None)
        if fast is not None and fast[0] is X_loc and fast[1] is y_loc:
            lib, g_args, i_args = fast[2], fast[3], fast[4]
            native.check(lib.gadmm_gram_f64(*g_args), "gram_f64")
            native.check(lib.gadmm_spd_inverse_small_f64(*i_args), "spd_inverse_small_f64")
            self._minv_version = getattr(self, "_minv_version", 0) + 1
            pf = getattr(self, "_pad_fast", None)
            if pf is not None and pf[0] is self.Minv and pf[1] is getattr(self, "_minv_pad", None):
                native.check(lib.gadmm_pad_image_f64(*pf[2]), "pad_image")
                self._minv_pad_version = self._minv_version
            return
        if (self.model == "linear" and X_loc.is_cuda and self.d <= 128 and X_loc.dtype == torch.float64
                and y_loc.dtype == torch.float64 and X_loc.is_contiguous() and y_loc.is_contiguous()
                and tuple(X_loc.shape) == (self.n_local, self.m, self.d) and self.Minv is not None
                and getattr(self, "_shifts", None) is not None and getattr(self, "_inv_status", None) is not None):
            lib = self.lib
            N, m, d = int(X_loc.shape[0]), int(X_loc.shape[1]), int(X_loc.shape[2])
            ks = int(lib.gadmm_gram_pick_ksplit(N, m, d))
            ws_n = int(lib.gadmm_gram_workspace(N, m, d, ks))
            self._refresh_ws = torch.empty((max(ws_n, 1),), dtype=torch.float64, device=self.device) \
                if ws_n > 0 else None
            st = self.stream.cuda_stream
            g_args = (X_loc.data_ptr(), y_loc.data_ptr(), N, m, d, ks, self.A.data_ptr(), self.b.data_ptr(),
                      self.yy.data_ptr(), self._refresh_ws.data_ptr() if self._refresh_ws is not None else None, st)
            i_args = (self.A.data_ptr(), self._shifts.data_ptr(), N, d, int(self._shifts.shape[1]),
                      self.Minv.data_ptr(), self._inv_status.data_ptr(), st)
            self._refresh_fast = (X_loc, y_loc, lib, g_args, i_args)
            return self.refresh(X_loc, y_loc)
        with torch.cuda.stream(self.stream):
            if self.model == "linear":
                gram(X_loc, y_loc, out=(self.A, self.b, self.yy))
                self._build_inverses(in_place=True, check=False)
            else:
                self.X.copy_(X_loc)
                self.Y.copy_(y_loc)

    def set_rho(self, rho: float):
        if getattr(self, "_shared_inverses", False):
            raise RuntimeError("this engine's inverses belong to a shared table: rho is fixed")
        self.rho = float(rho)
        if self.model == "linear":
            with torch.cuda.stream(self.stream):
                self._build_inverses()
            self._desc.base.Minv = self._kernel_minv().data_ptr()
        self._desc.base.rho = self.rho
        self._recreate()

    def _recreate(self):
        self.lib.gadmm_chain_engine_destroy(self.handle)
        self.handle = self.lib.gadmm_chain_engine_create(ctypes.byref(self._desc))
        if self.plan is not None:
            self._install(self.plan)
            self._plan_dirty = False

    def set_targets(self, obj0: float, tol: float, max_iter: Optional[int] = None):
        self.obj0, self.tol = float(obj0), float(tol)
        if max_iter is not None and max_iter != self.max_iter:
            raise ValueError("max_iter is fixed at construction (trace buffer size)")
        native.check(self.lib.gadmm_chain_engine_set_scalars(self.handle, self.rho, self.obj0, self.tol,
                                                             self.max_iter), "set_scalars")
        self._desc.base.obj0, self._desc.base.tol = self.obj0, self.tol

    def set_path(self, path: Sequence[int], placement: Placement, rank: int):
        pl = path.tolist() if isinstance(path, np.ndarray) else [int(w) for w in path]
        ok = getattr(self, "_owner_memo", None)
        if ok is None or ok[0] is not placement:
            ok = (placement, tuple(int(o) for o in placement.owner))
            self._owner_memo = ok
        key = (tuple(pl), int(rank), ok[1])
        memo = self.__dict__.setdefault("_plan_memo", {})
        plan = memo.get(key)
        if plan is None:
            plan = chain_plan(pl, placement, rank)
            lidx = {w: i for i, w in enumerate(self.local_ids)}
            for s in plan.head + plan.tail:
                if self.local_ids[s.li] != s.gid or lidx[s.gid] != s.li:
                    raise ValueError("placement/local_ids mismatch")
            if len(memo) > 4096:
                memo.clear()
            memo[key] = plan
        if plan is not getattr(self, "plan", None):
            self._plan_dirty = True
        self.plan = plan
        self.path = pl
        self.rank = rank
        self._placement_owner = list(ok[1])

    def _sync_plan(self):
        if getattr(self, "_plan_dirty", False) and self.plan is not None:
            self._install(self.plan)
            self._plan_dirty = False

    def _install(self, plan: RankPlan):
        def slots(lst):
            arr = (native.PhaseSlot * max(len(lst), 1))()
            for i, s in enumerate(lst):
                arr[i].li, arr[i].gid, arr[i].left, arr[i].right = s.li, s.gid, s.left, s.right
            return arr

        def ops(lst):
            arr = (native.XchgOp * max(len(lst), 1))()
            for i, (peer, row, snd) in enumerate(lst):
                arr[i].peer, arr[i].row, arr[i].is_send, arr[i].count = peer, row, snd, 0
            return arr

        if len(plan.head) + len(plan.tail) > 2 * max(self.n_local, 1):
            raise ValueError("plan larger than slot buffer")
        rc = self.lib.gadmm_chain_engine_set_plan(self.handle, len(plan.head), slots(plan.head), len(plan.tail),
                                                  slots(plan.tail), len(plan.xchg_head), ops(plan.xchg_head),
                                                  len(plan.xchg_tail), ops(plan.xchg_tail))
        native.check(rc, "set_plan")

    def reset(self, start_iter: int = 1, pending: int = 0, zero_state: bool = True):
        self._tr_valid = False
        if self.xport:
            native.check(self.lib.gadmm_ipc_new_epoch(self.xport, self.stream.cuda_stream), "ipc_new_epoch")
        if not zero_state:
            native.check(self.lib.gadmm_write_stamp(self.t0stamp.data_ptr(), self.stream.cuda_stream), "write_stamp")
        if self.hinv is not None and zero_state:
            with torch.cuda.stream(self.stream):
                self.hinv[:, 64 * 64].zero_()
        if self.rres is not None and zero_state:
            with torch.cuda.stream(self.stream):
                self.rres.zero_()
        if zero_state:
            native.check(self.lib.gadmm_chain_reset_state_stamp(
                self.ctl.data_ptr(), int(start_iter), int(pending), self.theta.data_ptr(), self.theta.numel(),
                self.mu.data_ptr(), self.mu.numel(), self.trace.data_ptr(), self.trace.numel(),
                self.part.data_ptr(), self.part.numel(), self.t0stamp.data_ptr(), self.stream.cuda_stream),
                "reset_state")
        else:
            native.check(self.lib.gadmm_chain_engine_reset(self.handle, int(start_iter), int(pending)), "reset")

    def exchange(self, which: str = "tail"):
        self._sync_plan()
        native.check(self.lib.gadmm_chain_engine_exchange(self.handle, 0 if which == "head" else 1), "exchange")

    def flush_duals(self):
        self._sync_plan()
        native.check(self.lib.gadmm_chain_engine_flush(self.handle), "flush")

    def run(self, stop_iter: int = 0, use_graph: bool = True, block: Optional[int] = None) -> EngineRun:
        self._tr_valid = False
        st = native.RunStats()
        blk = self.block if block is None else int(block)
        if blk > self.ring and self.nranks > 1:
            raise ValueError("block must be <= ring for multi-rank runs")
        self._sync_plan()
        tmo = float(getattr(self.comm, "timeout_s", 0.0) or 0.0) if getattr(self.comm, "backend", "") == "rccl" else 0.0
        native.check(self.lib.gadmm_chain_engine_set_timeout(self.handle, tmo), "chain_engine_set_timeout")
        rc = self.lib.gadmm_chain_engine_run(self.handle, blk, int(stop_iter), 1 if use_graph else 0,
                                             ctypes.byref(st))
        native.check(rc, "chain_engine_run")
        return EngineRun(st.iters, st.done, st.iterations_launched, st.replays, st.wall_ms, st.p2p_bytes,
                         st.p2p_msgs, st.monitor_bytes, st.wire_bytes)

    def resident_capacity(self, dynamic: bool = False, sys_scope: bool = False) -> int:
        key = (bool(dynamic), bool(sys_scope), getenv("GADMM_CU_BUDGET"), getenv("GADMM_PERSIST_LDS"))
        memo = self.__dict__.setdefault("_cap_memo", {})
        if key not in memo:
            pa = native.PersistArgs()
            pa.d, pa.n, pa.nvar, pa.obj_mode = self.d, self.n_total, self.nvar, self._obj_mode(dynamic)
            pa.n_epochs = 1 if dynamic else 0
            pa.sys_scope = 1 if sys_scope else 0
            memo[key] = int(self.lib.gadmm_chain_persistent_capacity(ctypes.byref(pa)))
        return memo[key]

    def _logi_args(self) -> native.LogiArgs:
        g = native.LogiArgs()
        b = self._desc.base
        g.X, g.Y, g.m, g.max_inner = native.ptr(self.X), native.ptr(self.Y), self.m, int(b.max_inner)
        g.lam, g.step, g.inner_tol = float(b.lam), float(b.step), float(b.inner_tol)
        if self.local_solver == "newton":
            g.step = self.chord_persistent
        g.inner_iters = self.inner_iters.data_ptr()
        g.scratch = self.newton_img.data_ptr() if self.newton_img is not None else None
        return g

    def persistent_q_eligible(self) -> bool:
        if self.quant is None or self.plan is None or self.path is None or self.model != "linear":
            return False
        if self.nranks != 1 or self.n_local != self.n_total or self.d > 64:
            return False
        key = ("q", getenv("GADMM_CU_BUDGET"))
        memo = self.__dict__.setdefault("_cap_memo", {})
        if key not in memo:
            pa = native.PersistArgs()
            pa.d, pa.n = self.d, self.n_total
            memo[key] = int(self.lib.gadmm_chain_persistent_q_capacity(ctypes.byref(pa)))
        return self.n_local + 1 <= memo[key]

    def _run_persistent_q(self, lag: int, timeout_s: float, start_iter: int, fetch_trace: bool) -> EngineRun:
        import time as _time
        if not self.persistent_q_eligible():
            raise RuntimeError("persistent Q kernel not eligible for this engine/config")
        if start_iter != 1:
            raise ValueError("persistent Q kernel: a fresh solve only (start_iter 1)")
        ring = lag + 4
        pa, slots, pos, _ = self._persist_args(lag, ring, timeout_s, start_iter, 0, None, False, 0, False)
        G = self.q_words + 1
        if getattr(self, "_qg", None) is None:
            with torch.cuda.stream(self.stream):
                self._qg = torch.zeros((self.n_total * G * 4,), dtype=torch.int32, device=self.device)
        pa.obj_mode = 0
        pa.qg, pa.q_true = self._qg.data_ptr(), self.theta_true.data_ptr()
        pa.q_bits, pa.q_seed = self.quant
        self.last_kernel = "persistent-Q(b=%d,G=%d)" % (self.quant[0], G)
        t0 = _time.perf_counter()
        rc = int(self.lib.gadmm_chain_persistent_q_launch(ctypes.byref(pa), self.stream.cuda_stream))
        if rc == -2:
            raise ResidencyError(self.lib.gadmm_last_error().decode())
        native.check(rc, "chain_persistent_q_launch")
        fetch = self._queue_readback(fetch_trace)
        self.stream.synchronize()
        self._tr_valid = fetch
        t1 = _time.perf_counter()
        self.last_timeline = self.last_timeline_slots = None
        done, conv, nxt = self._decode_ctl("persistent Q kernel")
        return EngineRun(conv, done, nxt - start_iter, 1, (t1 - t0) * 1e3, 0, 0, 0, 0)

    def persistent_eligible(self, fabric=None) -> bool:
        if self.plan is None or self.path is None:
            return False
        if self.quant is not None:
            return fabric is None and self.persistent_q_eligible()
        if self.nranks != 1 and fabric is None:
            return False
        if self.model == "logistic":
            if max(self.d, self.m) > 64:
                return False
            pa = native.PersistArgs()
            pa.d, pa.n, pa.sys_scope = self.d, self.n_total, 1 if fabric is not None else 0
            g = self._logi_args()
            if self.local_solver == "newton":
                if getenv("GADMM_NEWTON_PERSISTENT", "1") == "0":
                    return False
                cap = int(self.lib.gadmm_chain_persistent_newton_capacity(ctypes.byref(pa), ctypes.byref(g)))
            else:
                cap = int(self.lib.gadmm_chain_persistent_logistic_capacity(ctypes.byref(pa), ctypes.byref(g)))
            return self.n_local + 1 <= cap
        if self.model != "linear":
            return False
        if self._lds_need(False, self._obj_mode()) <= 0:
            return False
        return self.n_local + 1 <= self.resident_capacity(sys_scope=fabric is not None)

    def _lds_need(self, dynamic: bool, obj_mode: int) -> int:
        memo = self.__dict__.setdefault("_lds_memo", {})
        key = (bool(dynamic), int(obj_mode))
        v = memo.get(key)
        if v is None:
            v = int(self.lib.gadmm_chain_persistent_lds_dyn(self.d, obj_mode, self.nvar) if dynamic
                    else self.lib.gadmm_chain_persistent_lds(self.d, obj_mode))
            memo[key] = v
        return v

    def _obj_mode(self, dynamic: bool = False) -> int:
        return 0 if self._lds_need(dynamic, 0) > 0 else 1

    BLOCKED_DYN_MIN_COHERENCE = 3

    def dynamic_uses_blocked(self, fabric=None, coherence=None) -> bool:
        plan = self.blocked_plan(fabric) if self.model == "linear" else None
        if plan is None or plan[3] != 1 or self.n_local != self.n_total:
            return False
        env = getenv("GADMM_BLOCKED_DYN", "")
        if env in ("0", "1"):
            return env == "1"
        return coherence is not None and float(coherence) >= self.BLOCKED_DYN_MIN_COHERENCE

    def dynamic_eligible(self, fabric=None) -> bool:
        if self.model != "linear" or self.quant is not None:
            return False
        if self.nranks != 1 and (fabric is None or getattr(fabric, "table_slots", 1) < 2):
            return False
        if self.nranks == 1 and self.n_local != self.n_total:
            return False
        if self._lds_need(True, self._obj_mode(True)) <= 0:
            return False
        return self.n_local + 1 <= self.resident_capacity(dynamic=True, sys_scope=fabric is not None)

    def blocked_plan(self, fabric=None, timeline: bool = False):
        if fabric is not None or self.nranks > 1 or self.d > 64 or getenv("GADMM_BLOCKED", "1") == "0" \
                or self.quant is not None:
            return None
        key = (bool(timeline), getenv("GADMM_BLOCK_K"), getenv("GADMM_BLOCK_L"),
               getenv("GADMM_BLOCK_PW"), getenv("GADMM_CU_BUDGET"))
        memo = self.__dict__.setdefault("_plan2_memo", {})
        if key not in memo:
            kk, ll, pp = ctypes.c_int(0), ctypes.c_int(0), ctypes.c_int(0)
            want = int(getenv("GADMM_BLOCK_K", "0"))
            W = int(self.lib.gadmm_chain_blocked_plan2(self.n_total, self.d, want, 1 if timeline else 0,
                                                       ctypes.byref(kk), ctypes.byref(ll), ctypes.byref(pp)))
            memo[key] = (kk.value, ll.value, W, pp.value) if W > 0 else None
        return memo[key]

    def _persist_args(self, lag, ring, timeout_s, start_iter, pending_in, fabric, dynamic, hard_stop, cont):
        dev = self.device
        pk = (id(self.plan), tuple(self.path))
        memo = getattr(self, "_slot_memo", None)
        if memo is None or memo[0] != pk:
            pos_of = {g: i for i, g in enumerate(self.path)}
            sl = sorted(self.plan.head + self.plan.tail, key=lambda s: pos_of[s.gid])
            memo = (pk, sl, [pos_of[s.gid] for s in sl], tuple((s.li, s.gid, s.left, s.right) for s in sl), self.plan)
            self._slot_memo = memo
        _, slots, pos, slot_key, _ = memo
        key = (ring, slot_key, id(fabric), dynamic)
        if getattr(self, "_pbuf", None) is None or self._pbuf[0] != key:
            with torch.cuda.stream(self.stream):
                slot_t = torch.tensor([[s.li, s.gid, s.left, s.right] for s in slots], dtype=torch.int32,
                                      device=dev).reshape(-1)
                pos_t = torch.tensor(pos, dtype=torch.int32, device=dev)
                if fabric is None:
                    thg = torch.zeros(((ring if dynamic else 1) * self.n_total * self.d * 4,),
                                      dtype=torch.int32, device=dev)
                    objg = torch.zeros((ring * self.n_total * 4,), dtype=torch.int32, device=dev)
                    decg = torch.zeros((ring,), dtype=torch.int64, device=dev)
                    ptrs = (thg.data_ptr(), objg.data_ptr(), decg.data_ptr())
                    push = None
                    dec_push = torch.tensor([decg.data_ptr()], dtype=torch.int64, device=dev)
                    keep = (thg, objg, decg)
                elif dynamic:
                    if getattr(fabric, "table_slots", 1) < ring:
                        raise RuntimeError("fabric theta tables hold %d slots, D-GADMM needs %d"
                                           % (getattr(fabric, "table_slots", 1), ring))
                    push = None
                else:
                    owner = self._placement_owner
                    pl = []
                    for s in slots:
                        peers = sorted({int(owner[u]) for u in (s.left, s.right) if u >= 0} - {self.rank})
                        ps = [fabric.thg_peer[r] for r in peers] + [0, 0]
                        pl += ps[:2]
                    push = torch.tensor(pl, dtype=torch.int64, device=dev)
                if fabric is not None:
                    ptrs = (fabric.thg.ptr.value, fabric.objg_mon, fabric.decg.ptr.value)
                    dec_push = torch.tensor(fabric.dec_all if fabric.dec_all else [0], dtype=torch.int64,
                                            device=dev)
                    keep = (torch.tensor(fabric.table_ptrs(), dtype=torch.int64, device=dev),) \
                        if dynamic else ()
            self._pbuf = (key, slot_t, pos_t, ptrs, push, dec_push, keep, [0])
        _, slot_t, pos_t, ptrs, push, dec_push, keep, epoch_box = self._pbuf
        if cont:
            epoch = self._salt
            native.check(self.lib.gadmm_chain_engine_reset(self.handle, int(start_iter), int(pending_in)), "reset")
        elif fabric is not None:
            epoch = fabric.next_epoch()
        else:
            epoch_box[0] = epoch_box[0] % 4095 + 1
            epoch = epoch_box[0]
        self._salt = epoch
        if fabric is None and getattr(self, "_xchk", None) is None:
            with torch.cuda.stream(self.stream):
                self._xchk = torch.zeros((256 * 4,), dtype=torch.int32, device=dev)
        objs = (self._pbuf, self.Minv, self.A, self.b, self.yy, self.theta, self.mu, self.trace, self.ctl,
                self.tstamp, self.rres, fabric, getattr(self, "_xchk", None))
        nums = (int(lag), ring, self.rho, self.obj0, self.tol, float(timeout_s), dynamic, self.rank,
                self.nranks, int(self.xcd), self.nvar, tuple(self.deg_to_var), self.max_iter, len(slots))
        tmpl = self.__dict__.get("_pa_tmpl")
        if tmpl is None or tmpl[1] != nums or any(x is not y for x, y in zip(tmpl[0], objs)):
            pt = native.PersistArgs()
            pt.d, pt.n, pt.n_local, pt.max_iter = self.d, self.n_total, len(slots), self.max_iter
            pt.lag, pt.ring, pt.nvar, pt.obj_mode = int(lag), ring, self.nvar, self._obj_mode(dynamic)
            for i, v in enumerate(self.deg_to_var):
                pt.deg_to_var[i] = v
            pt.has_monitor = 1 if (fabric is None or self.rank == 0) else 0
            pt.nranks = 1 if fabric is None else self.nranks
            pt.sys_scope = 0 if fabric is None else 1
            pt.rho, pt.obj0, pt.tol = self.rho, self.obj0, self.tol
            pt.timeout_ticks = int(timeout_s * 1e8)
            pt.slots, pt.pos = slot_t.data_ptr(), pos_t.data_ptr()
            pt.Minv, pt.A, pt.b, pt.yy = native.ptr(self.Minv), native.ptr(self.A), native.ptr(self.b), native.ptr(self.yy)
            pt.theta, pt.mu = self.theta.data_ptr(), self.mu.data_ptr()
            pt.thg, pt.objg, pt.decg = ptrs
            pt.push = push.data_ptr() if push is not None else None
            pt.dec_push = dec_push.data_ptr()
            pt.trace, pt.ctl = self.trace.data_ptr(), self.ctl.data_ptr()
            pt.tstamp = self.tstamp.data_ptr()
            pt.rres = native.ptr(self.rres)
            if fabric is None:
                pt.xchk, pt.xcd = self._xchk.data_ptr(), int(self.xcd)
            tmpl = (objs, nums, pt)
            self._pa_tmpl = tmpl
        pa = native.PersistArgs.from_buffer_copy(tmpl[2])
        pa.start_iter, pa.pending_in, pa.epoch = int(start_iter), int(pending_in), int(epoch)
        pa.hard_stop, pa.cont = int(hard_stop), 1 if cont else 0
        return pa, slots, pos, keep

    def _attach_blocked(self, pa, plan, ring, dynamic):
        ng = int((self.lib.gadmm_chain_blocked_tab_granules_dyn if dynamic else
                  self.lib.gadmm_chain_blocked_tab_granules)(self.n_total, self.d, ring))
        if getattr(self, "_blk_tab", None) is None or self._blk_tab.numel() != ng * 4:
            with torch.cuda.stream(self.stream):
                self._blk_tab = torch.zeros((ng * 4,), dtype=torch.int32, device=self.device)
        pa.blk_k, pa.blk_len, pa.blk_pw = plan[0], plan[1], plan[3]
        pa.blk_tab = self._blk_tab.data_ptr()

    def _queue_readback(self, fetch_trace: bool) -> bool:
        nt = self.trace.numel()
        fetch = fetch_trace and nt <= 16384
        if getattr(self, "_rb_host", None) is None:
            self._rb_host = torch.empty(self._rb.shape, dtype=torch.float64, pin_memory=True)
            self._rb_host_np = self._rb_host.numpy()
            self._ctl_host = self._rb_host[0:4].view(torch.int32)
        nb = self._rb.numel() * 8 if fetch else 32
        native.check(self.lib.gadmm_readback_d2h(self._rb_host.data_ptr(), self._rb.data_ptr(), nb,
                                                 self.stream.cuda_stream), "readback")
        return fetch

    def _decode_ctl(self, what: str = "persistent chain kernel"):
        c = self._ctl_host.tolist()
        done, conv, nxt = c[1], c[2], c[0]
        self.last_placed = c[6]
        if done == 4:
            raise HandoffTimeout("%s timed out (hand-off never completed)" % what)
        return done, conv, nxt

    def prepare_blocked(self, lag: int = 4, timeout_s: float = 20.0, start_iter: int = 1):
        if self.nranks != 1 or self.n_local != self.n_total or not self.persistent_eligible(None):
            raise ValueError("persistent kernel not eligible for this engine/config")
        plan = self.blocked_plan(None) if self.model == "linear" else None
        if plan is None or plan[3] != 1:
            raise ValueError("no 12-wave blocked plan for this engine (n=%d, d=%d)" % (self.n_total, self.d))
        lag = max(lag, 8)
        ring = lag + 4
        pa, _, _, _ = self._persist_args(lag, ring, timeout_s, start_iter, 0, None, False, 0, False)
        self._attach_blocked(pa, plan, ring, False)
        return pa, plan

    def _stage_epochs_fused(self, pa, starts: np.ndarray, P: np.ndarray, start_iter: int, cont: bool):
        E, n = P.shape
        total = E + 7 * E * n
        stage = getattr(self, "_ep_stage", None)
        if stage is None or stage[0].numel() < total:
            cap = max(total, 4096)
            h_t = torch.empty((cap,), dtype=torch.int32, pin_memory=True)
            d_t = torch.empty((cap,), dtype=torch.int32, device=self.device)
            stage = (h_t, d_t, h_t.numpy(), h_t.data_ptr(), d_t.data_ptr())
            self._ep_stage = stage
        if len(starts) != E:
            raise ValueError("epochs: one chain per start")
        got = int(self.lib.gadmm_epoch_stage_blocked(starts.ctypes.data, P.ctypes.data, E, n, int(start_iter),
                                                     1 if cont else 0, stage[3], stage[0].numel(), stage[4],
                                                     self.stream.cuda_stream))
        if got < 0:
            raise ValueError(self.lib.gadmm_last_error().decode())
        dptr = stage[4]
        pa.n_epochs = E
        pa.epoch_start, pa.ep_slots = dptr, dptr + 4 * E
        pa.ep_pos, pa.ep_flush = dptr + 4 * (E + 4 * E * n), dptr + 4 * (E + 5 * E * n)

    def _attach_minv_pad(self, pa):
        if getattr(self, "_minv_pad", None) is None or self._minv_pad_version != self._minv_version:
            pf = getattr(self, "_pad_fast", None)
            if pf is not None and pf[0] is self.Minv and pf[1] is self._minv_pad:
                native.check(self.lib.gadmm_pad_image_f64(*pf[2]), "pad_image")
            else:
                with torch.cuda.stream(self.stream):
                    self._minv_pad = quad_pad_image(self.Minv.reshape(self.n_local * self.nvar, self.d, self.d),
                                                    int(self.lib.gadmm_chain_blocked_pad_dim(self.d)),
                                                    out=getattr(self, "_minv_pad", None))
                src = _QUAD_SRC.get((self.d, int(self.lib.gadmm_chain_blocked_pad_dim(self.d)), self.device))
                if src is not None and self.Minv.is_contiguous():
                    self._pad_fast = (self.Minv, self._minv_pad,
                                      (self.Minv.data_ptr(), self.d * self.d, src.data_ptr(), int(src.numel()),
                                       self.n_local * self.nvar, self._minv_pad.data_ptr(),
                                       self.stream.cuda_stream))
            self._minv_pad_version = self._minv_version
        pa.minv_pad = self._minv_pad.data_ptr()

    def prepare_blocked_dyn(self, starts: np.ndarray, P: np.ndarray, lag: int = 4, timeout_s: float = 20.0,
                            start_iter: int = 1, pending_in: int = 0, hard_stop: int = 0, cont: bool = False):
        if self.nranks != 1 or not self.dynamic_eligible(None):
            raise ValueError("dynamic persistent kernel not eligible for this engine/config")
        plan = self.blocked_plan(None) if self.model == "linear" else None
        if plan is None or plan[3] != 1:
            raise ValueError("no 12-wave blocked plan for this engine (n=%d, d=%d)" % (self.n_total, self.d))
        lag = max(lag, 8)
        ring = lag + 4
        pa, _, _, _ = self._persist_args(lag, ring, timeout_s, start_iter, pending_in, None, True, hard_stop, cont)
        self._stage_epochs_fused(pa, starts, P, start_iter, cont)
        self._attach_blocked(pa, plan, ring, True)
        self._attach_minv_pad(pa)
        return pa, plan

    def finish_blocked(self, start_iter: int, wall_ms: float, fetch: bool, what: str) -> EngineRun:
        self._tr_valid = fetch
        self.last_timeline = self.last_timeline_slots = None
        done, conv, nxt = self._decode_ctl(what)
        return EngineRun(conv, done, nxt - start_iter, 1, wall_ms, 0, 0, 0, 0)

    def adopt_stream(self, stream: torch.cuda.Stream):
        stream.wait_stream(self.stream)
        self.stream = stream
        self._desc.stream = stream.cuda_stream
        self._refresh_fast = None
        self._pad_fast = None
        self._recreate()

    def run_persistent(self, lag: int = 4, timeout_s: float = 20.0, start_iter: int = 1,
                       pending_in: int = 0, fabric=None, timeline_iters: int = 0,
                       epochs: Optional[Sequence] = None, hard_stop: int = 0, cont: bool = False,
                       fetch_trace: bool = False, blocked_dyn: Optional[bool] = None,
                       on_enqueued=None) -> EngineRun:
        _timing.host_stamp("rp:start")
        if self.quant is not None:
            if fabric is not None or epochs is not None or pending_in or hard_stop or cont or timeline_iters:
                raise RuntimeError("persistent Q kernel: a static chain on one GPU, one launch per solve")
            return self._run_persistent_q(lag, timeout_s, start_iter, fetch_trace)
        if epochs is not None:
            if not self.dynamic_eligible(fabric):
                raise RuntimeError("dynamic persistent kernel not eligible for this engine/config")
        elif not self.persistent_eligible(fabric):
            raise RuntimeError("persistent kernel not eligible for this engine/config")
        plan = self.blocked_plan(fabric, timeline=timeline_iters > 0) if self.model == "linear" else None
        if blocked_dyn is None:
            blocked_dyn = self.dynamic_uses_blocked(fabric)
        if epochs is not None and (not blocked_dyn or timeline_iters > 0):
            plan = None
        if plan is not None:
            lag = max(lag, 8)
        ring = lag + 4
        dev = self.device
        pa, slots, pos, keep = self._persist_args(lag, ring, timeout_s, start_iter, pending_in, fabric,
                                                  epochs is not None, hard_stop, cont)
        _timing.host_stamp("rp:args")
        fused = epochs is not None and plan is not None and fabric is None and isinstance(epochs, tuple) \
            and len(epochs) == 2 and isinstance(epochs[1], np.ndarray) and isinstance(epochs[0], np.ndarray) \
            and epochs[0].dtype == np.int64 and epochs[1].dtype == np.int64 and epochs[1].flags.c_contiguous \
            and epochs[0].flags.c_contiguous
        if fused:
            self._stage_epochs_fused(pa, epochs[0], epochs[1], start_iter, cont)
        elif epochs is not None:
            if isinstance(epochs, tuple) and len(epochs) == 2 and isinstance(epochs[1], np.ndarray):
                starts = np.asarray(epochs[0], dtype=np.int64)
                P = np.asarray(epochs[1], dtype=np.int64)
            else:
                starts = np.asarray([int(e[0]) for e in epochs], dtype=np.int64)
                P = np.asarray([list(e[1]) for e in epochs], dtype=np.int64)
            if (starts[0] > int(start_iter) if cont else starts[0] != int(start_iter)) or np.any(starts[1:] <= starts[:-1]):
                raise ValueError("epochs must start at start_iter (continuations: at or before it) and increase")
            E, n = P.shape
            if E != len(starts):
                raise ValueError("epochs: one chain per start")
            loc = np.asarray([int(w) for w in self.local_ids], dtype=np.int64)
            if plan is not None:
                P = np.ascontiguousarray(P)
                es = np.empty((E * n * 4,), dtype=np.int32)
                pp = np.empty((E * n,), dtype=np.int32)
                fl = np.empty((E * n * 2,), dtype=np.int32)
                native.check(self.lib.gadmm_epoch_tables_blocked(P.ctypes.data, E, n, es.ctypes.data, pp.ctypes.data,
                                                                 fl.ctypes.data), "epoch_tables_blocked")
            else:
                P = np.ascontiguousarray(P)
                es = np.empty((E * len(loc) * 4,), dtype=np.int32)
                pp = np.empty((E * len(loc),), dtype=np.int32)
                native.check(self.lib.gadmm_epoch_tables(P.ctypes.data, E, n, loc.ctypes.data, len(loc),
                                                         es.ctypes.data, pp.ctypes.data), "epoch_tables")
            if fabric is not None:
                owner = np.asarray(self._placement_owner, dtype=np.int64)
                sl4 = es.reshape(E, len(loc), 4)
                mask = np.zeros((E, len(loc)), dtype=np.int64)
                for col in (2, 3):
                    nb = sl4[:, :, col].astype(np.int64)
                    ow = np.where(nb >= 0, owner[np.maximum(nb, 0)], self.rank)
                    mask |= np.where(ow != self.rank, np.left_shift(1, ow), 0)
                pm = mask.astype(np.int32).reshape(-1)
            else:
                pm = np.zeros((0,), dtype=np.int32)
            if plan is None:
                fl = np.zeros((0,), dtype=np.int32)
            ns, nes = len(starts), es.size
            total = ns + nes + pp.size + pm.size + fl.size
            stage = getattr(self, "_ep_stage", None)
            if stage is None or stage[0].numel() < total:
                cap = max(total, 4096)
                h_t = torch.empty((cap,), dtype=torch.int32, pin_memory=True)
                d_t = torch.empty((cap,), dtype=torch.int32, device=dev)
                stage = (h_t, d_t, h_t.numpy(), h_t.data_ptr(), d_t.data_ptr())
                self._ep_stage = stage
            host, hptr, dptr = stage[2], stage[3], stage[4]
            o_es, o_pp, o_pm, o_fl = ns, ns + nes, ns + nes + pp.size, total - fl.size
            host[:ns] = starts
            host[o_es:o_pp] = es
            host[o_pp:o_pm] = pp
            host[o_pm:o_fl] = pm
            host[o_fl:total] = fl
            native.check(self.lib.gadmm_memcpy_h2d_async(dptr, hptr, total * 4, self.stream.cuda_stream), "h2d")
            if fl.size:
                pa.ep_flush = dptr + 4 * o_fl
            pa.n_epochs = len(starts)
            pa.epoch_start, pa.ep_slots, pa.ep_pos = dptr, dptr + 4 * o_es, dptr + 4 * o_pp
            if fabric is not None:
                pa.ep_push, pa.peer_thg = dptr + 4 * o_pm, keep[0].data_ptr()
        _timing.host_stamp("rp:tables")
        tl = None
        if timeline_iters > 0:
            with torch.cuda.stream(self.stream):
                tl = torch.zeros((max(len(slots), 256) + 1, int(timeline_iters), 8), dtype=torch.int64, device=dev)
            pa.timeline, pa.timeline_iters = tl.data_ptr(), int(timeline_iters)
        import time as _time
        if plan is not None:
            self._attach_blocked(pa, plan, ring, epochs is not None)
            if epochs is not None:
                self._attach_minv_pad(pa)
        self.last_kernel = ("blocked%s(k=%d,L=%d,W=%d,pw=%d)" % ((("-dyn" if epochs is not None else ""),) + tuple(plan))
                            if plan is not None else "per-worker")
        t0 = _time.perf_counter()
        rc = None
        _timing.host_stamp("rp:prelaunch")
        if plan is not None:
            rc = int(self.lib.gadmm_chain_blocked_launch(ctypes.byref(pa), self.stream.cuda_stream))
            _timing.host_stamp("rp:launched")
            if rc == -2 and epochs is None:
                plan, rc = None, None
                self.last_kernel = "per-worker"
            else:
                native.check(rc, "chain_blocked_launch")
        if plan is None and self.model == "logistic":
            if epochs is not None:
                raise RuntimeError("persistent logistic kernel: static chains only")
            self._logi = self._logi_args()
            if self.local_solver == "newton":
                which = int(self.lib.gadmm_chain_persistent_newton_kernel(ctypes.byref(pa), ctypes.byref(self._logi)))
                self.last_kernel = "per-worker-newton" + {1: "(one-wave)", 2: "(pipeline)"}.get(which, "")
                launch = self.lib.gadmm_chain_persistent_newton_launch
            else:
                self.last_kernel = "per-worker-logistic"
                launch = self.lib.gadmm_chain_persistent_logistic_launch
            rc = int(launch(ctypes.byref(pa), ctypes.byref(self._logi), self.stream.cuda_stream))
            if rc == -2:
                raise ResidencyError(self.lib.gadmm_last_error().decode())
            native.check(rc, "chain_persistent_logistic_launch")
        elif plan is None:
            rc = int(self.lib.gadmm_chain_persistent_launch(ctypes.byref(pa), self.stream.cuda_stream))
            if rc == -2:
                raise ResidencyError(self.lib.gadmm_last_error().decode())
            native.check(rc, "chain_persistent_launch")
        fetch = self._queue_readback(fetch_trace)
        _timing.host_stamp("rp:copies_queued")
        if on_enqueued is not None:
            on_enqueued()
            _timing.host_stamp("rp:overlapped")
        self.stream.synchronize()
        _timing.host_stamp("rp:synced")
        self._tr_valid = fetch
        t1 = _time.perf_counter()
        self.last_timeline = tl.cpu().numpy() if tl is not None else None
        self.last_timeline_slots = [(s.gid, p) for s, p in zip(slots, pos)] if tl is not None else None
        done, conv, nxt = self._decode_ctl()
        last = conv if done in (1, 2, 3) else (int(hard_stop) if hard_stop > 0 else conv)
        p2p = msgs = mon = 0
        if fabric is not None and last >= start_iter:
            conv_b = last
            ran = conv_b - start_iter + 1
            if epochs is None:
                owner = self._placement_owner
                per_it = sum(len({int(owner[u]) for u in (s.left, s.right) if u >= 0} - {self.rank}) for s in slots)
# ... 69 lines not shown
```

gadmm_amd/engine/multigpu.py:

```python
from __future__ import annotations

import sys
import time
from dataclasses import dataclass
from typing import Optional, Sequence

import numpy as np
import torch
import torch.distributed as dist


@dataclass
class SolveOut:
    iters: int
    done: int
    theta_bytes: int
    wire_bytes: int
    monitor_bytes: int


def all_ok(flag: bool, world: int) -> bool:
    if world == 1:
        return flag
    t = torch.tensor([0.0 if flag else 1.0], dtype=torch.float64)
# ... 13 lines not shown
    return st


class DistributedChainSolver:
    def __init__(self, X_loc: torch.Tensor, y_loc: torch.Tensor, local: Sequence[int], n_total: int, placement,
                 rank: int, world: int, device: torch.device, rho: float, obj0: float, tol: float,
                 max_iter: int = 20000, engine: str = "auto", fabric: str = "auto", share: bool = False,
                 block: int = 0, halo_data=None, timeout_s: float = 20.0, use_graph: bool = True,
                 dl_halo: Optional[bool] = None, strict: bool = False, halo_k: int = 0, halo_pw: int = 0,
                 plane=None):
        from .chain_engine import NativeChainEngine

        self.X, self.y = X_loc, y_loc
        self.local = [int(w) for w in local]
        self.n, self.placement, self.rank, self.world, self.device = n_total, placement, rank, world, device
        self.rho, self.obj0, self.tol, self.max_iter = rho, obj0, tol, max_iter
        self.share, self.fabric_req, self.timeout_s, self.use_graph = share, fabric, timeout_s, use_graph
        self.block = block if block > 0 else (32 if world == 1 else 16)
        self.d = int(X_loc.shape[2])
        self.path = list(range(n_total))
        self.eng = self.comm = self.fab = self.blk = None
        self.kind, self.persistent, self.replicated_bytes = "local", False, 0
        self.fallbacks = []
        self.dl_halo = dl_halo
        self.plane, self._own_comm = plane, True
        self.delay_next_s = 0.0
        self._NCE = NativeChainEngine
        if world == 1:
            self.eng = self._engine(None)
            self.persistent = engine in ("auto", "persistent") and self.eng.persistent_eligible()
        elif engine == "replicated-halo":
            from .blocked_xgmi import BlockedXgmiEngine
            if halo_data is None:
                raise ValueError("replicated-halo needs the halo workers' shards (halo_data=(X_all, y_all))")
            self.blk = BlockedXgmiEngine(halo_data[0], halo_data[1], n_total, placement, rank, rho, obj0, tol,
                                         max_iter, device, stream=solver_stream(device), want_k=halo_k,
                                         want_pw=halo_pw)
            self.replicated_bytes = self.blk.replicated_shard_bytes()
            self.persistent = True
            self.kind = "xgmi(replicated-halo,k=%d,pw=%d)" % (self.blk.k, self.blk.pw)
        else:
            if fabric in ("auto", "xgmi") and engine in ("auto", "persistent", "blocked-dl"):
                self._try_blocked_dl()
            if self.blk is None and fabric in ("auto", "xgmi") and engine in ("auto", "persistent", "per-worker"):
                self._try_xgmi()
            if self.eng is None and self.blk is None:
                if strict and engine != "graph":
                    raise RuntimeError("engine %r unavailable on some rank" % engine)
                self._graph_engine()

    def _engine(self, comm):
        e = self._NCE(self.X, self.y, self.local, self.n, "linear", rho=self.rho, obj0=self.obj0, tol=self.tol,
                      max_iter=self.max_iter, comm=comm, block=self.block, stream=solver_stream(self.device))
        e.set_path(self.path, self.placement, self.rank)
        return e

    def _try_blocked_dl(self):
        from .blocked_xgmi import BlockedXgmiEngine

        lo, hi = min(self.local), max(self.local)
        eligible = self.local == list(range(lo, hi + 1)) and self.d <= 52 and self.n >= 2
        if not all_ok(eligible, self.world):
            return
        try:
            blk = BlockedXgmiEngine(self.X, self.y, self.n, self.placement, self.rank, self.rho, self.obj0, self.tol,
                                    self.max_iter, self.device, data_local=True, dl_halo=self.dl_halo,
                                    stream=solver_stream(self.device))
        except Exception as e:
            if self.rank == 0:
                print("DistributedChainSolver: data-local blocked fabric unavailable (%s)" % e, file=sys.stderr)
            return
        self.blk, self.persistent = blk, True
        self.kind = "xgmi(blocked-dl-halo)" if blk._halo_mode() else "xgmi(blocked-dl)"
        self.replicated_bytes = blk.replicated_shard_bytes()

    def _try_xgmi(self):
        from ..parallel.comm import RankInfo
        from ..parallel.xgmi import XgmiFabric

        ok, err = False, ""
        eng = self._engine(RankInfo(self.rank, self.world))
        try:
            need = sorted({int(self.placement.owner[u]) for w in self.local for u in (w - 1, w + 1)
                           if 0 <= u < self.n} - {self.rank})
            self.fab = XgmiFabric(self.n, self.d, 8, self.rank, self.world, self.device, peers_needed=need)
            ok = eng.persistent_eligible(self.fab)
            err = "" if ok else "persistent kernel not eligible (residency)"
        except Exception as e:
            err = str(e)
        if all_ok(ok, self.world):
            self.eng, self.persistent, self.kind = eng, True, "xgmi"
            return
        if self.rank == 0:
            print("DistributedChainSolver: xgmi fabric unavailable (%s); graph engine" % (err or "another rank"),
                  file=sys.stderr)
        if self.fab is not None:
            self.fab.close()
        self.fab = None
        eng.close()

    def _graph_engine(self, force_ipc: bool = False):
        from ..parallel.dataplane import make_data_plane
        fabric = "ipc" if force_ipc else self.fabric_req
        if getattr(self, "plane", None) is not None and not (force_ipc and getattr(self.plane, "backend", "") != "ipc"):
            self.comm, self._own_comm = self.plane, False
        else:
            self.comm, self._own_comm = make_data_plane(fabric, self.world, self.device, self.share, self.n,
                                                        self.d, self.block, timeout_s=self.timeout_s), True
        self.kind = self.comm.selection["data_plane"]
        if getattr(self.comm, "backend", "") == "host-gloo":
            self.eng = TorchPathEngine(self.X, self.y, self.local, self.n, self.placement, self.comm, self.rho,
                                       self.obj0, self.tol, self.max_iter)
        else:
            self.eng = self._engine(self.comm)
        self.persistent = False

    def can_fall_back(self) -> bool:
        return self.world > 1 and (self.persistent or self.kind == "rccl")

    def fall_back(self, why: str):
        self.fallbacks.append(why)
        from_rccl = (not self.persistent) and self.kind == "rccl"
        if self.blk is not None:
            self.blk.close()
            self.blk = None
        if self.fab is not None:
            self.fab.close()
            self.fab = None
        if self.eng is not None:
            self.eng.close()
            self.eng = None
        if self.comm is not None:
            if from_rccl:
                self.comm.abort()
            own = getattr(self, "_own_comm", True)
            if own or from_rccl:
                self.comm.close()
            if not own:
                self.plane = None
            self.comm = None
        self._graph_engine(force_ipc=from_rccl)

    def solve(self) -> SolveOut:
        if self.delay_next_s > 0:
            time.sleep(self.delay_next_s)
            self.delay_next_s = 0.0
        if self.blk is not None:
            self.blk.refresh()
            it, done, self.last_wall_ms = self.blk.run(timeout_s=self.timeout_s)
            if done == 4:
                raise RuntimeError("blocked kernel: a hand-off timed out")
            pay = self.blk.exchange_bytes_per_solve(it)
            return SolveOut(it, done, pay, 2 * pay, self.blk.monitor_bytes_per_solve(it))
        self.eng.refresh(self.X, self.y)
        self.eng.reset()
        if self.persistent:
            r = self.eng.run_persistent(fabric=self.fab, timeout_s=self.timeout_s)
        else:
            r = self.eng.run(use_graph=self.use_graph)
        self.last_wall_ms = float(getattr(r, "wall_ms", 0.0))
        return SolveOut(r.iters, r.done, r.p2p_bytes, r.wire_bytes, r.monitor_bytes)

    def guarded_solve(self) -> SolveOut:
        try:
            return self.solve()
        except RuntimeError as e:
            print("DistributedChainSolver[rank %d]: %s" % (self.rank, e), file=sys.stderr)
            return SolveOut(0, 4, 0, 0, 0)

    def solve_agreed(self) -> SolveOut:
        out = self.guarded_solve()
        if all_ok(out.done == 1, self.world):
            return out
        if self.can_fall_back():
            self.fall_back("%s solve failed on some rank (done=%d here)" % (self.kind, out.done))
            out = self.guarded_solve()
        return out

    @property
    def kernel(self) -> Optional[str]:
        if not self.persistent:
            return None
        return self.blk.last_kernel if self.blk is not None else getattr(self.eng, "last_kernel", None)

    def engine_name(self) -> str:
        if self.persistent:
            return "persistent"
        return "graph" if (self.eng is not None and self.eng.graph_ok() and self.use_graph) else "eager"

    def objective_trace(self, iters: int):
        return self.blk.objective_trace(iters) if self.blk is not None else self.eng.objective_trace(iters)

    def close(self):
        for o in (self.eng, self.blk, self.fab, self.comm if getattr(self, "_own_comm", True) else None):
            if o is not None:
                o.close()
        self.eng = self.blk = self.fab = self.comm = None


class TorchPathEngine:

    def __init__(self, X, y, local, n_total, placement, comm, rho, obj0, tol, max_iter):
        from ..models import LinearRegression
        self.X, self.y, self.local, self.n, self.placement, self.comm = X, y, list(local), n_total, placement, comm
        self.rho, self.obj0, self.tol, self.max_iter = rho, obj0, tol, max_iter
        self.model = LinearRegression(X, y)
        self.last = None

    def refresh(self, X, y):
        from ..ops.linalg import gram
        gram(X, y, out=(self.model.A, self.model.b, self.model.yy))
        self.model._chol = {}

    def reset(self, start_iter: int = 1):
        self.last = None

    def run(self, stop_iter: int = 0, use_graph: bool = True):
        import time as _t
        from ..algorithms.gadmm import chain_admm
        t0 = _t.perf_counter()
        snap = self.comm.stats.snapshot()
        r = chain_admm(self.model, self.local, self.n, self.rho, self.obj0, self.tol, self.max_iter, comm=self.comm,
                       placement=self.placement, backend="torch")
        self.last = r
        pay = int(self.comm.stats.delta(snap)["bytes_sent"])
        mon = int(self.comm.stats.delta(snap)["monitor_bytes"])

        class _R:
            pass
        o = _R()
        o.iters, o.done = int(r.iters), (1 if r.converged else 2)
        o.p2p_bytes, o.wire_bytes, o.monitor_bytes = pay, pay, mon
        o.wall_ms = (_t.perf_counter() - t0) * 1e3
        return o

    def objective_trace(self, upto=None):
        tr = self.last.obj if self.last is not None else np.zeros(0)
        return tr if upto is None else tr[:upto]

    def traces(self, upto: int):
        return self.objective_trace(upto), np.asarray(self.last.time_trace[:upto])

    def graph_ok(self) -> bool:
        return False

    def close(self):
        self.last = None


def node_chain_admm(model, local_ids: Sequence[int], n_total: int, placement, rank: int, world: int,
                    device: torch.device, rho: float, obj0: float, tol: float, max_iter: int,
                    fabric: str = "auto", share: bool = False, plane=None, timeout_s: float = 20.0,
                    name: str = "GADMM"):
    import numpy as np
    from ..algorithms.base import RunResult

    local = [int(w) for w in local_ids]
    sol = DistributedChainSolver(model.X, model.y, local, n_total, placement, rank, world, device, rho, obj0, tol,
                                 max_iter=max_iter, fabric=fabric, share=share, timeout_s=timeout_s, plane=plane)
    try:
        if sol.blk is not None:
            sol.blk.stamps = True
        out = sol.guarded_solve()
        if not all_ok(out.done in (1, 2), world) and sol.can_fall_back():
            sol.fall_back("%s solve failed on some rank (done=%d here)" % (sol.kind, out.done))
            out = sol.guarded_solve()
        if not all_ok(out.done in (1, 2), world):
            raise RuntimeError("node GADMM solve failed (done=%d here, engine %s)" % (out.done, sol.kind))
        iters = int(out.iters)
        if sol.blk is not None:
            tr, tt = sol.blk.objective_trace(iters), sol.blk.time_trace(iters)
        else:
            tr, tt = sol.eng.traces(iters)
        buf = torch.from_numpy(np.stack([np.asarray(tr, np.float64), np.asarray(tt, np.float64)]))
        dist.broadcast(buf, src=0)
        tr, tt = buf[0].numpy().copy(), buf[1].numpy().copy()
        tot = torch.tensor([float(out.theta_bytes), float(out.wire_bytes), float(out.monitor_bytes),
                            float(sol.replicated_bytes)], dtype=torch.float64)
        dist.all_reduce(tot)
        transport = "xgmi" if sol.persistent else sol.kind
        res = RunResult(algorithm=name, obj=tr, loss=np.abs(tr - obj0), iters=iters, converged=(out.done == 1),
                        wall_s=float(getattr(sol, "last_wall_ms", 0.0)) / 1e3, time_trace=tt,
                        comm_units=np.arange(1, iters + 1, dtype=np.float64) * n_total,
                        com_cost=np.zeros(iters), bytes_sent=int(out.theta_bytes), bytes_total=int(tot[0].item()),
                        extra={"backend": "native", "engine": sol.engine_name(), "kernel": sol.kernel or "",
                               "engine_kind": sol.kind, "transport": transport, "rank": rank, "nranks": world,
                               "solver": "closed", "wire_bytes": int(out.wire_bytes),
                               "monitor_bytes": int(out.monitor_bytes),
                               "wire_bytes_all_ranks": int(tot[1].item()),
                               "monitor_bytes_all_ranks": int(tot[2].item()),
                               "replicated_shard_bytes": int(tot[3].item()),
                               "fallbacks": "; ".join(sol.fallbacks)})
        return res
    finally:
        sol.close()
```

gadmm_amd/ops/native.py:

```python
from __future__ import annotations

import ctypes
import os
from typing import Optional

import torch

_LIB_PATH = os.environ.get("GADMM_NATIVE_LIB") or os.path.join(
    os.path.dirname(os.path.dirname(os.path.abspath(__file__))), "_native", "libgadmm_native.so")
_lib: Optional[ctypes.CDLL] = None
_load_error: Optional[str] = None

c_int, c_long, c_double, c_void_p, c_char_p = ctypes.c_int, ctypes.c_long, ctypes.c_double, ctypes.c_void_p, ctypes.c_char_p
c_longlong = ctypes.c_longlong


class PhaseSlot(ctypes.Structure):
    _fields_ = [("li", c_int), ("gid", c_int), ("left", c_int), ("right", c_int)]


class XchgOp(ctypes.Structure):
    _fields_ = [("peer", c_int), ("row", c_int), ("is_send", c_int), ("count", c_int)]


# ... 38 lines not shown
    _fields_ = [
        ("alg", c_int), ("model", c_int), ("n", c_int), ("d", c_int), ("m", c_int), ("max_iter", c_int),
        ("faithful", c_int), ("jacobi", c_int), ("has_tol", c_int), ("ring", c_int),
        ("epoch", ctypes.c_uint), ("slots", c_int),
        ("step", c_double), ("lam", c_double), ("obj0", c_double), ("tol", c_double), ("thrd", c_double),
        ("timeout_ticks", c_longlong),
        ("A", c_void_p), ("b", c_void_p), ("yy", c_void_p), ("X", c_void_p), ("Y", c_void_p),
        ("hsq", c_void_p), ("sched", c_void_p), ("tab", c_void_p), ("part", c_void_p),
        ("obj_trace", c_void_p), ("cnt_trace", c_void_p), ("time_trace", c_void_p), ("theta_out", c_void_p),
        ("ctl", c_void_p), ("xchk", c_void_p), ("xcd", c_int), ("pad_x", c_int),
        ("nranks", c_int), ("my_rank", c_int), ("w_lo", c_int), ("n_local", c_int),
        ("has_monitor", c_int), ("pad_m", c_int),
        ("owner", c_void_p), ("tab_push", c_void_p), ("wmon", c_void_p), ("wstop", c_void_p),
        ("wpush", c_void_p), ("pushc", c_void_p),
    ]


class RunStats(ctypes.Structure):
    _fields_ = [("iters", c_int), ("done", c_int), ("iterations_launched", c_int), ("replays", c_int),
                ("wall_ms", c_double), ("p2p_bytes", c_longlong), ("p2p_msgs", c_longlong),
                ("monitor_bytes", c_longlong), ("wire_bytes", c_longlong)]


class PersistArgs(ctypes.Structure):
    _fields_ = [
        ("d", c_int), ("n", c_int), ("n_local", c_int), ("start_iter", c_int), ("max_iter", c_int),
        ("lag", c_int), ("ring", c_int), ("nvar", c_int), ("obj_mode", c_int), ("deg_to_var", c_int * 3),
        ("pending_in", c_int), ("has_monitor", c_int), ("nranks", c_int), ("sys_scope", c_int),
        ("epoch", ctypes.c_uint), ("blk_pw", c_int),
        ("rho", c_double), ("obj0", c_double), ("tol", c_double), ("timeout_ticks", c_longlong),
        ("slots", c_void_p), ("pos", c_void_p), ("Minv", c_void_p), ("A", c_void_p), ("b", c_void_p),
        ("yy", c_void_p), ("theta", c_void_p), ("mu", c_void_p), ("thg", c_void_p), ("push", c_void_p),
        ("objg", c_void_p), ("decg", c_void_p), ("dec_push", c_void_p), ("trace", c_void_p), ("ctl", c_void_p),
        ("timeline", c_void_p), ("timeline_iters", c_int), ("blk_k", c_int), ("blk_len", c_int), ("n_epochs", c_int),
        ("blk_tab", c_void_p), ("epoch_start", c_void_p), ("ep_slots", c_void_p), ("ep_pos", c_void_p),
        ("seg_lo", c_int), ("seg_hi", c_int), ("blk_npeer", c_int), ("dbg", c_int),
        ("blk_peer_lo", c_int * 8), ("blk_peer_hi", c_int * 8), ("blk_peer_tab", c_void_p),
        ("tstamp", c_void_p), ("ep_push", c_void_p), ("peer_thg", c_void_p), ("rres", c_void_p),
        ("hard_stop", c_int), ("cont", c_int),
        ("xchk", c_void_p), ("xcd", c_int), ("xtag", c_int),
        ("blk_dl", c_int), ("dl_halo", c_int), ("dl_tab", c_void_p * 2), ("minv_pad", c_void_p),
        ("ep_flush", c_void_p),
        ("qg", c_void_p), ("q_true", c_void_p), ("q_bits", c_int), ("q_seed", ctypes.c_ulonglong),
    ]


class LogiArgs(ctypes.Structure):
    _fields_ = [("X", c_void_p), ("Y", c_void_p), ("m", c_int), ("max_inner", c_int),
                ("lam", c_double), ("step", c_double), ("inner_tol", c_double), ("inner_iters", c_void_p),
                ("scratch", c_void_p)]


class StarArgs(ctypes.Structure):
    _fields_ = [
        ("d", c_int), ("n", c_int), ("n_local", c_int), ("max_iter", c_int),
        ("lag", c_int), ("ring", c_int), ("has_monitor", c_int), ("nranks", c_int),
        ("sys_scope", c_int), ("hub_rank", c_int), ("my_rank", c_int), ("timeline_iters", c_int),
        ("epoch", ctypes.c_uint), ("pad1", c_int),
        ("rho", c_double), ("obj0", c_double), ("tol", c_double), ("timeout_ticks", c_longlong),
        ("gid", c_void_p), ("Minv", c_void_p), ("A", c_void_p), ("b", c_void_p), ("yy", c_void_p),
        ("theta", c_void_p), ("lam", c_void_p), ("lam_hub", c_void_p), ("thg", c_void_p), ("peer_thg", c_void_p),
        ("objg", c_void_p), ("decg", c_void_p), ("dec_push", c_void_p), ("trace", c_void_p), ("tstamp", c_void_p),
        ("ctl", c_void_p), ("timeline", c_void_p), ("xchk", c_void_p), ("xcd", c_int), ("pad2", c_int),
    ]


MODEL_LINEAR, MODEL_LOGISTIC = 0, 1


def _declare(lib: ctypes.CDLL) -> None:
    sig = {
        "gadmm_last_error": (c_char_p, []),
        "gadmm_native_version": (c_int, []),
        "gadmm_device_info": (c_int, [c_int, c_char_p, c_int, ctypes.POINTER(c_int), ctypes.POINTER(c_longlong),
                                      ctypes.POINTER(c_int), ctypes.POINTER(c_int)]),
        "gadmm_gram_f64": (c_int, [c_void_p, c_void_p, c_int, c_int, c_int, c_int, c_void_p, c_void_p, c_void_p,
                                   c_void_p, c_void_p]),
        "gadmm_gram_workspace": (c_long, [c_int, c_int, c_int, c_int]),
        "gadmm_gram_pick_ksplit": (c_int, [c_int, c_int, c_int]),
        "gadmm_spd_inverse_small_f64": (c_int, [c_void_p, c_void_p, c_int, c_int, c_int, c_void_p, c_void_p,
                                                c_void_p]),
        "gadmm_spd_inverse_blocked_workspace": (c_long, [c_int, c_int]),
        "gadmm_spd_inverse_blocked_f64": (c_int, [c_void_p, c_void_p, c_int, c_int, c_int, c_void_p, c_void_p,
                                                  c_void_p, c_int, c_void_p]),
        "gadmm_gemm_f64_test": (c_int, [c_int, c_int, c_int, c_void_p, c_void_p, c_void_p, c_void_p]),
        "gadmm_chain_phase": (c_int, [ctypes.POINTER(PhaseArgs), c_void_p]),
        "gadmm_chain_reset": (c_int, [c_void_p, c_int, c_int, c_void_p]),
        "gadmm_chain_reset_state": (c_int, [c_void_p, c_int, c_int, c_void_p, c_long, c_void_p, c_long, c_void_p,
                                            c_long, c_void_p, c_long, c_void_p]),
        "gadmm_chain_reset_state_stamp": (c_int, [c_void_p, c_int, c_int, c_void_p, c_long, c_void_p, c_long, c_void_p,
                                            c_long, c_void_p, c_long, c_void_p, c_void_p]),
        "gadmm_chain_engine_create": (c_void_p, [ctypes.POINTER(EngineDesc)]),
        "gadmm_chain_engine_destroy": (None, [c_void_p]),
        "gadmm_chain_engine_set_plan": (c_int, [c_void_p, c_int, ctypes.POINTER(PhaseSlot), c_int,
                                                ctypes.POINTER(PhaseSlot), c_int, ctypes.POINTER(XchgOp), c_int,
                                                ctypes.POINTER(XchgOp)]),
        "gadmm_chain_engine_set_scalars": (c_int, [c_void_p, c_double, c_double, c_double, c_int]),
        "gadmm_chain_engine_reset": (c_int, [c_void_p, c_int, c_int]),
        "gadmm_chain_engine_flush": (c_int, [c_void_p]),
        "gadmm_chain_engine_run": (c_int, [c_void_p, c_int, c_int, c_int, ctypes.POINTER(RunStats)]),
        "gadmm_chain_engine_graph_ok": (c_int, [c_void_p]),
        "gadmm_chain_engine_exchange": (c_int, [c_void_p, c_int]),
        "gadmm_abi_layout": (c_int, [ctypes.POINTER(c_longlong), c_int]),
        "gadmm_chain_persistent_lds": (c_long, [c_int, c_int]),
        "gadmm_chain_persistent_lds_dyn": (c_long, [c_int, c_int, c_int]),
        "gadmm_chain_big_rbuf_stride": (c_long, [c_int]),
        "gadmm_xgmi_alloc": (c_int, [ctypes.c_size_t, ctypes.POINTER(c_void_p), ctypes.c_char_p]),
        "gadmm_xgmi_open": (c_int, [ctypes.c_char_p, ctypes.POINTER(c_void_p)]),
        "gadmm_xgmi_close": (c_int, [c_void_p]),
        "gadmm_xgmi_free": (c_int, [c_void_p]),
        "gadmm_device_can_access_peer": (c_int, [c_int, c_int]),
        "gadmm_chain_persistent_launch": (c_int, [ctypes.POINTER(PersistArgs), c_void_p]),
        "gadmm_chain_persistent_capacity": (c_long, [ctypes.POINTER(PersistArgs)]),
        "gadmm_chain_persistent_q_launch": (c_int, [ctypes.POINTER(PersistArgs), c_void_p]),
        "gadmm_chain_persistent_q_capacity": (c_long, [ctypes.POINTER(PersistArgs)]),
        "gadmm_quant_abi_layout": (c_int, [ctypes.POINTER(c_longlong), c_int]),
        "gadmm_chain_persistent_logistic_capacity": (c_long, [ctypes.POINTER(PersistArgs), ctypes.POINTER(LogiArgs)]),
        "gadmm_chain_persistent_logistic_launch": (c_int, [ctypes.POINTER(PersistArgs), ctypes.POINTER(LogiArgs),
                                                           c_void_p]),
        "gadmm_logi_abi_layout": (c_int, [ctypes.POINTER(c_longlong), c_int]),
        "gadmm_chain_persistent_newton_capacity": (c_long, [ctypes.POINTER(PersistArgs), ctypes.POINTER(LogiArgs)]),
        "gadmm_chain_persistent_newton_kernel": (c_int, [ctypes.POINTER(PersistArgs), ctypes.POINTER(LogiArgs)]),
        "gadmm_newton_rec_scratch_doubles": (c_long, []),
        "gadmm_chain_persistent_newton_launch": (c_int, [ctypes.POINTER(PersistArgs), ctypes.POINTER(LogiArgs),
                                                         c_void_p]),
        "gadmm_write_stamp": (c_int, [c_void_p, c_void_p]),
        "gadmm_star_capacity": (c_long, [ctypes.POINTER(StarArgs)]),
        "gadmm_star_launch": (c_int, [ctypes.POINTER(StarArgs), c_void_p]),
        "gadmm_star_abi_layout": (c_int, [ctypes.POINTER(c_longlong), c_int]),
        "gadmm_star_big_abi_layout": (c_int, [ctypes.POINTER(c_longlong), c_int]),
        "gadmm_sym_pack_f64": (c_int, [c_void_p, c_void_p, c_int, c_int, c_void_p]),
        "gadmm_sym_packed_doubles": (c_long, [c_int]),
        "gadmm_ipc_box_bytes": (c_long, [c_int, c_int, c_int, c_int]),
        "gadmm_ipc_collective": (c_int, [c_void_p, c_int, c_int, c_void_p, c_void_p, c_int, ctypes.c_uint, c_void_p,
                                         c_void_p]),
        "gadmm_ipc_coll_counters": (c_int, [c_void_p, ctypes.POINTER(c_longlong)]),
        "gadmm_ipc_hop_probe": (c_int, [c_void_p, c_void_p, c_int, c_int, ctypes.c_uint, c_double,
                                        ctypes.POINTER(ctypes.c_ulonglong)]),
        "gadmm_ipc_xport_create": (c_void_p, [c_int, c_int, c_int, c_int, c_int, c_void_p, c_void_p, c_double]),
        "gadmm_ipc_xport_destroy": (c_int, [c_void_p]),
        "gadmm_ipc_new_epoch": (c_int, [c_void_p, c_void_p]),
        "gadmm_ipc_counters": (c_int, [c_void_p, ctypes.POINTER(c_longlong)]),
        "gadmm_chain_blocked_plan": (c_int, [c_int, c_int, c_int, ctypes.POINTER(c_int), ctypes.POINTER(c_int)]),
        "gadmm_chain_blocked_plan2": (c_int, [c_int, c_int, c_int, c_int, ctypes.POINTER(c_int), ctypes.POINTER(c_int),
                                              ctypes.POINTER(c_int)]),
        "gadmm_chain_blocked_lds": (c_long, [c_int, c_int]),
        "gadmm_chain_blocked_plan_dl": (c_int, [c_int, c_int, c_int, ctypes.POINTER(c_int), ctypes.POINTER(c_int)]),
        "gadmm_chain_blocked_pad_dim": (c_int, [c_int]),
        "gadmm_chain_blocked_pad_len": (c_long, [c_int]),
        "gadmm_chain_blocked_max_epochs": (c_int, []),
        "gadmm_memcpy_h2d_async": (c_int, [c_void_p, c_void_p, ctypes.c_size_t, c_void_p]),
        "gadmm_memcpy_d2h_async": (c_int, [c_void_p, c_void_p, ctypes.c_size_t, c_void_p]),
        "gadmm_readback_d2h": (c_int, [c_void_p, c_void_p, ctypes.c_size_t, c_void_p]),
        "gadmm_chain_blocked_tab_granules": (c_long, [c_int, c_int, c_int]),
        "gadmm_chain_blocked_tab_granules_dyn": (c_long, [c_int, c_int, c_int]),
        "gadmm_epoch_tables": (c_int, [c_void_p, c_int, c_int, c_void_p, c_int, c_void_p, c_void_p]),
        "gadmm_epoch_tables_blocked": (c_int, [c_void_p, c_int, c_int, c_void_p, c_void_p, c_void_p]),
        "gadmm_epoch_stage_blocked": (c_long, [c_void_p, c_void_p, c_int, c_int, c_int, c_int, c_void_p, c_long,
                                               c_void_p, c_void_p]),
        "gadmm_chain_blocked_launch": (c_int, [ctypes.POINTER(PersistArgs), c_void_p]),
        "gadmm_chain_blocked_sweep_capacity": (c_int, []),
        "gadmm_chain_blocked_sweep_launch": (c_int, [ctypes.POINTER(PersistArgs), c_int, c_void_p, c_void_p, c_void_p]),
        "gadmm_chain_blocked_dyn_sweep_launch": (c_int, [ctypes.POINTER(PersistArgs), c_int, c_void_p, c_void_p,
                                                         c_void_p]),
        "gadmm_fo_lds": (c_long, [c_int, c_int, c_int, c_int, c_int]),
        "gadmm_fo_kernel_class": (c_int, [c_int, c_int, c_int]),
        "gadmm_fo_tab_granules": (c_long, [c_int, c_int, c_int]),
        "gadmm_fo_abi_layout": (c_int, [ctypes.POINTER(c_longlong), c_int]),
        "gadmm_fo_launch": (c_int, [ctypes.POINTER(FoArgs), c_void_p]),
        "gadmm_quad_gemv_test": (c_int, [c_void_p, c_void_p, c_void_p, c_int, c_int, c_int, c_void_p]),
        "gadmm_greedy_chains": (c_int, [c_void_p, c_int, c_int, c_double, c_int, c_double, c_double, c_double,
                                        c_void_p, c_void_p]),
        "gadmm_greedy_chains_async": (c_int, [c_void_p, c_int, c_int, c_double, c_int, c_double, c_double,
                                              c_double, c_void_p, c_void_p]),
        "gadmm_greedy_chains_wait": (c_int, []),
        "gadmm_pcg64_uniform": (c_int, [ctypes.c_ulonglong] * 5 + [c_long, c_void_p]),
        "gadmm_draw_chains_async": (c_int, [ctypes.c_ulonglong] * 5 + [c_void_p, c_int, c_int, c_double, c_int, c_double,
                                                                        c_double, c_double, c_void_p, c_void_p]),
        "gadmm_rccl_unique_id": (c_int, [ctypes.c_char_p]),
        "gadmm_rccl_version": (c_int, []),
        "gadmm_rccl_init": (c_void_p, [ctypes.c_char_p, c_int, c_int, c_int]),
        "gadmm_rccl_init_timeout": (c_void_p, [ctypes.c_char_p, c_int, c_int, c_int, ctypes.c_double]),
        "gadmm_rccl_set_timeout": (c_int, [c_void_p, ctypes.c_double]),
        "gadmm_rccl_alive": (c_int, [c_void_p]),
        "gadmm_rccl_abort": (c_int, [c_void_p]),
        "gadmm_rccl_wait": (c_int, [c_void_p, c_void_p, ctypes.c_double]),
        "gadmm_debug_busy_wait": (c_int, [ctypes.c_double, c_void_p]),
        "gadmm_gram_ozaki_workspace": (c_long, [c_long, c_int]),
        "gadmm_gram_crt_workspace": (c_long, [c_long, c_int]),
        "gadmm_gram_crt_max_rows": (c_long, []),
        "gadmm_gram_crt_f64": (c_int, [c_void_p, c_void_p, c_int, c_long, c_int, c_void_p, c_void_p, c_void_p,
                                       c_void_p, c_long, c_void_p, c_void_p]),
        "gadmm_gram_ozaki_f64": (c_int, [c_void_p, c_void_p, c_int, c_long, c_int, c_void_p, c_void_p, c_void_p,
                                         c_void_p, c_long, c_void_p, c_void_p]),
        "gadmm_chain_engine_set_timeout": (c_int, [c_void_p, ctypes.c_double]),
        "gadmm_rccl_destroy": (c_int, [c_void_p]),
        "gadmm_rccl_exchange_rows": (c_int, [c_void_p, ctypes.POINTER(XchgOp), c_int, c_void_p, c_int, c_void_p]),
        "gadmm_rccl_allreduce_sum_f64": (c_int, [c_void_p, c_void_p, c_void_p, c_long, c_void_p]),
        "gadmm_rccl_reduce_sum_f64": (c_int, [c_void_p, c_void_p, c_void_p, c_long, c_int, c_void_p]),
        "gadmm_rccl_bcast_f64": (c_int, [c_void_p, c_void_p, c_long, c_int, c_void_p]),
        "gadmm_rccl_counters": (c_int, [c_void_p, ctypes.POINTER(c_longlong)]),
        "gadmm_rccl_reset_counters": (c_int, [c_void_p]),
        "gadmm_poison_lds": (c_int, [c_long, c_int, c_void_p]),
        "gadmm_poison_buffer": (c_int, [c_void_p, c_long, c_void_p]),
        "gadmm_lds_probe": (c_int, [c_void_p, c_int, c_int, c_void_p]),
        "gadmm_memset_async": (c_int, [c_void_p, c_int, c_long, c_void_p]),
    }
    for name, (res, args) in sig.items():
        fn = getattr(lib, name, None)
        if fn is None:
            continue
        fn.restype = res
        fn.argtypes = args


def library_path() -> str:
    return _LIB_PATH


def load(build_if_missing: bool = True) -> Optional[ctypes.CDLL]:
    global _lib, _load_error
    if _lib is not None:
        return _lib
    try:
        if build_if_missing:
            from .. import _build
            try:
                _build.build(verbose=False)
            except Exception as e:
                if not os.path.exists(_LIB_PATH):
                    raise RuntimeError("native build failed: %s" % e)
        lib = ctypes.CDLL(_LIB_PATH, mode=ctypes.RTLD_GLOBAL)
        _declare(lib)
        _lib = lib
    except Exception as e:
        _load_error = str(e)
        _lib = None
    return _lib


def available() -> bool:
    return load() is not None


def require() -> ctypes.CDLL:
    lib = load()
    if lib is None:
        raise RuntimeError("gadmm_amd native library unavailable (%s): build it with "
                           "`python -m gadmm_amd._build`" % _load_error)
    return lib


RCCL_DEAD = -77


class RcclDead(RuntimeError):
    """An RCCL communicator's watchdog deadline passed (or RCCL reported an asynchronous error): the
    communicator was aborted and refuses further calls; the caller falls back to another data plane."""


class NativeTimeout(RuntimeError):
    """A bounded host wait of the native engine passed its deadline (a stalled peer or collective)."""


ENGINE_TIMEOUT = -78
RCCL_WEDGED = -79


class DeviceWedged(SystemExit):
    """The device stream did not drain after a watchdog abort: no fallback may run on this device.
    A SystemExit (not caught by the ``except RuntimeError`` fallbacks): the process exits non-zero."""


def check(rc: int, what: str = "native call") -> None:
    if rc != 0:
        msg = require().gadmm_last_error()
        text = "%s failed (rc=%d): %s" % (what, rc, msg.decode() if msg else "?")
        if rc == RCCL_DEAD:
            raise RcclDead(text)
        if rc == ENGINE_TIMEOUT:
            raise NativeTimeout(text)
        if rc == RCCL_WEDGED:
            import sys
            print("gadmm_amd: " + text, file=sys.stderr, flush=True)
            raise DeviceWedged(5)
        raise RuntimeError(text)


def poison_lds(per_cu: int = 4, sync: bool = True) -> None:
    check(require().gadmm_poison_lds(0, per_cu, stream_handle()), "poison_lds")
    if sync:
        torch.cuda.synchronize()


def ptr(t: Optional[torch.Tensor]) -> Optional[int]:
    if t is None:
        return None
    return t.data_ptr()


def stream_handle(stream: Optional[torch.cuda.Stream] = None) -> int:
    s = stream if stream is not None else torch.cuda.current_stream()
    return s.cuda_stream
```

Before: 1.701 ms.

## Fuse Gram, SPD inverse and state reset into one setup kernel with padded Minv

Adds a fused small-problem setup kernel that computes the Gram matrix with MFMA tiles, inverts the shifted SPD systems with register-resident Gauss-Jordan, writes a pre-padded inverse image and optionally resets the state. It also defers refresh so refresh and reset can merge into one launch. The blocked chain kernel gains an image-load path that reads the padded inverse directly instead of re-laying it out. This cuts launch count and setup latency ahead of the solve, at the cost of version tracking and more template variants.

```diff
diff --git a/csrc/include/gj_reg64.h b/csrc/include/gj_reg64.h
--- /dev/null
+++ b/csrc/include/gj_reg64.h
@@ -0,0 +1,65 @@
+#pragma once
+#include "gadmm_common.h"
+
+namespace gj_reg64 {
+
+constexpr int MS_DOUBLES = 64 * 65;
+constexpr int COLV_DOUBLES = 2 * 65;
+
+__device__ __forceinline__ double readlane_f64(double v, int l) {
+  const long long b = __double_as_longlong(v);
+  const int lo = __builtin_amdgcn_readlane((int)b, l), hi = __builtin_amdgcn_readlane((int)(b >> 32), l);
+  return __longlong_as_double(((long long)hi << 32) | (unsigned)lo);
+}
+
+template <int NW>
+__device__ __forceinline__ bool pivots(double (&h)[64 / NW], int d, double (*colv)[65]) {
+  constexpr int NC = 64 / NW;
+  const int i = threadIdx.x & 63, w = threadIdx.x >> 6;
+  if (w == 0) {
+    colv[0][i] = h[0];
+    const double p0 = 1.0 / readlane_f64(h[0], 0);
+    if (i == 0) colv[0][64] = p0;
+  }
+  __syncthreads();
+  bool bad = false;
+  for (int k = 0; k < d; ++k) {
+    const double* cb = colv[k & 1];
+    const double pk = cb[k], aik = cb[i], p = cb[64];
+    bad |= !(pk > 0.0);
+#pragma unroll
+    for (int c = 0; c < NC; ++c) {
+      const int j = w + NW * c;
+      const double mkj = readlane_f64(h[c], k) * p;
+      double val = h[c];
+      if (j == k) val = (i == k) ? p : -aik * p;
+      else if (i == k) val = mkj;
+      else val -= aik * mkj;
+      h[c] = val;
+    }
+    const int kn = k + 1;
+    if (kn < d && w == kn % NW) {
+      double nxt = 0.0;
+#pragma unroll
+      for (int c = 0; c < NC; ++c) nxt = (c == kn / NW) ? h[c] : nxt;
+      colv[kn & 1][i] = nxt;
+      const double pn = 1.0 / readlane_f64(nxt, kn);
+      if (i == 0) colv[kn & 1][64] = pn;
+    }
+    __syncthreads();
+  }
+  return bad;
+}
+
+template <int NW>
+__device__ __forceinline__ void write_out(const double (&h)[64 / NW], int d, double* Ms, double* __restrict__ o) {
+  constexpr int NC = 64 / NW;
+  const int i = threadIdx.x & 63, w = threadIdx.x >> 6;
+#pragma unroll
+  for (int c = 0; c < NC; ++c) Ms[i * 65 + w + NW * c] = h[c];
+  __syncthreads();
+  for (int r = w; r < d; r += NW)
+    if (i < d) o[r * d + i] = 0.5 * (Ms[r * 65 + i] + Ms[i * 65 + r]);
+}
+
+}
diff --git a/csrc/include/gram_tile.h b/csrc/include/gram_tile.h
--- /dev/null
+++ b/csrc/include/gram_tile.h
@@ -0,0 +1,186 @@
+#pragma once
+#include "gadmm_common.h"
+
+namespace gram_tile {
+
+constexpr int BK = 16;
+constexpr int PAD = 16;
+
+template <int BT, int NT>
+struct GramTile {
+  static constexpr int NWAVE = NT / 64;
+  static constexpr int WR = NWAVE / 2;
+  static constexpr int WTR = BT / WR;
+  static constexpr int WTC = BT / 2;
+  static constexpr int TMR = WTR / 16;
+  static constexpr int TMC = WTC / 16;
+  static constexpr int LDSROW = BT + PAD;
+  static constexpr int PER_THREAD = BK * BT / NT;
+  static constexpr int LDS_DOUBLES = 2 * 2 * BK * LDSROW;
+};
+
+template <int BT, int NT, bool DIAG, bool CLAMP>
+__device__ __forceinline__ void gram_slabs(const double* __restrict__ H, const double* __restrict__ yv, int d,
+                                           long kbeg, long kend, long nfull, int row0, int col0,
+                                           double (*lds)[2 * BK * GramTile<BT, NT>::LDSROW],
+                                           f64x4 (&acc)[GramTile<BT, NT>::TMR][GramTile<BT, NT>::TMC]) {
+  using T = GramTile<BT, NT>;
+  const int tid = threadIdx.x, lane = tid & 63, wid = tid >> 6;
+  const int wr = wid >> 1, wc = wid & 1;
+  double ri[T::PER_THREAD], rj[T::PER_THREAD];
+  auto fetch_in = [&](long k0) {
+#pragma unroll
+    for (int p = 0; p < T::PER_THREAD / 2; ++p) {
+      const int e2 = tid + NT * p;
+      const int r = e2 / (BT / 2), c = (e2 % (BT / 2)) * 2;
+      const double* src = H + (k0 + r) * (long)d;
+      ri[2 * p] = src[row0 + c];
+      ri[2 * p + 1] = src[row0 + c + 1];
+      if constexpr (!DIAG) {
+        rj[2 * p] = src[col0 + c];
+        rj[2 * p + 1] = src[col0 + c + 1];
+      }
+    }
+  };
+  auto fetch_cl = [&](long k0) {
+#pragma unroll
+    for (int p = 0; p < T::PER_THREAD / 2; ++p) {
+      const int e2 = tid + NT * p;
+      const int r = e2 / (BT / 2), c = (e2 % (BT / 2)) * 2;
+      const long k = k0 + r;
+      const long kk = k < kend ? k : (kend - 1);
+      const double yk = yv[kk];
+      const bool kin = k < kend;
+#pragma unroll
+      for (int q = 0; q < 2; ++q) {
+        const int ca = row0 + c + q, cb = col0 + c + q;
+        const double va = H[kk * d + (ca < d ? ca : d - 1)];
+        ri[2 * p + q] = kin ? (ca < d ? va : (ca == d ? yk : 0.0)) : 0.0;
+        if constexpr (!DIAG) {
+          const double vb = H[kk * d + (cb < d ? cb : d - 1)];
+          rj[2 * p + q] = kin ? (cb < d ? vb : (cb == d ? yk : 0.0)) : 0.0;
+        }
+      }
+    }
+  };
+  double yr[CLAMP ? T::PER_THREAD / 2 : 1];
+  long kraw = 0;
+  auto fetch_raw = [&](long k0) {
+    kraw = k0;
+#pragma unroll
+    for (int p = 0; p < T::PER_THREAD / 2; ++p) {
+      const int e2 = tid + NT * p;
+      const int r = e2 / (BT / 2), c = (e2 % (BT / 2)) * 2;
+      const long k = k0 + r;
+      const long kk = k < kend ? k : (kend - 1);
+      yr[p] = yv[kk];
+#pragma unroll
+      for (int q = 0; q < 2; ++q) {
+        const int ca = row0 + c + q, cb = col0 + c + q;
+        ri[2 * p + q] = H[kk * d + (ca < d ? ca : d - 1)];
+        if constexpr (!DIAG) rj[2 * p + q] = H[kk * d + (cb < d ? cb : d - 1)];
+      }
+    }
+  };
+  auto select_raw = [&]() {
+#pragma unroll
+    for (int p = 0; p < T::PER_THREAD / 2; ++p) {
+      const int e2 = tid + NT * p;
+      const int r = e2 / (BT / 2), c = (e2 % (BT / 2)) * 2;
+      const bool kin = kraw + r < kend;
+#pragma unroll
+      for (int q = 0; q < 2; ++q) {
+        const int ca = row0 + c + q, cb = col0 + c + q;
+        ri[2 * p + q] = kin ? (ca < d ? ri[2 * p + q] : (ca == d ? yr[p] : 0.0)) : 0.0;
+        if constexpr (!DIAG) rj[2 * p + q] = kin ? (cb < d ? rj[2 * p + q] : (cb == d ? yr[p] : 0.0)) : 0.0;
+      }
+    }
+  };
+  auto stash = [&](int buf) {
+    if constexpr (CLAMP) select_raw();
+    double* Si = lds[buf];
+    double* Sj = lds[buf] + BK * T::LDSROW;
+#pragma unroll
+    for (int p = 0; p < T::PER_THREAD / 2; ++p) {
+      const int e2 = tid + NT * p;
+      const int r = e2 / (BT / 2), c = (e2 % (BT / 2)) * 2;
+      *reinterpret_cast<double2*>(Si + r * T::LDSROW + c) = make_double2(ri[2 * p], ri[2 * p + 1]);
+      if constexpr (!DIAG) *reinterpret_cast<double2*>(Sj + r * T::LDSROW + c) = make_double2(rj[2 * p], rj[2 * p + 1]);
+    }
+  };
+  auto mma = [&](int buf) {
+    const double* Ci = lds[buf];
+    const double* Cb = DIAG ? Ci : lds[buf] + BK * T::LDSROW;
+#pragma unroll
+    for (int ks = 0; ks < BK / 4; ++ks) {
+      const int kr = ks * 4 + (lane >> 4);
+      double a[T::TMR], b[T::TMC];
+#pragma unroll
+      for (int t = 0; t < T::TMR; ++t) a[t] = Ci[kr * T::LDSROW + wr * T::WTR + t * 16 + (lane & 15)];
+#pragma unroll
+      for (int t = 0; t < T::TMC; ++t) b[t] = Cb[kr * T::LDSROW + wc * T::WTC + t * 16 + (lane & 15)];
+#pragma unroll
+      for (int x = 0; x < T::TMR; ++x)
+#pragma unroll
+        for (int yq = 0; yq < T::TMC; ++yq)
+          acc[x][yq] = __builtin_amdgcn_mfma_f64_16x16x4f64(a[x], b[yq], acc[x][yq], 0, 0, 0);
+    }
+  };
+
+  auto fetch = [&](long k0) {
+    if constexpr (CLAMP) fetch_raw(k0);
+    else fetch_in(k0);
+  };
+  int cur = 0;
+  long k0 = kbeg;
+  if (nfull > 0) {
+    fetch(k0);
+    stash(0);
+    lds_barrier();
+    for (long s = 1; s < nfull; ++s) {
+      fetch(k0 + BK);
+      mma(cur);
+      stash(cur ^ 1);
+      lds_barrier();
+      cur ^= 1;
+      k0 += BK;
+    }
+    mma(cur);
+    lds_barrier();
+    cur ^= 1;
+    k0 += BK;
+  }
+  for (; k0 < kend; k0 += BK) {
+    if constexpr (CLAMP) fetch_raw(k0);
+    else fetch_cl(k0);
+    stash(cur);
+    lds_barrier();
+    mma(cur);
+    cur ^= 1;
+  }
+}
+
+template <int BT, int NT>
+__device__ __forceinline__ void gram_tile_acc(const double* __restrict__ H, const double* __restrict__ yv, int d,
+                                              long kbeg, long kend, int row0, int col0, bool diag,
+                                              double (*lds)[2 * BK * GramTile<BT, NT>::LDSROW],
+                                              f64x4 (&acc)[GramTile<BT, NT>::TMR][GramTile<BT, NT>::TMC]) {
+  using T = GramTile<BT, NT>;
+#pragma unroll
+  for (int a = 0; a < T::TMR; ++a)
+#pragma unroll
+    for (int b = 0; b < T::TMC; ++b) acc[a][b] = f64x4{0.0, 0.0, 0.0, 0.0};
+  const bool cols_in = (row0 + BT <= d) && (diag || col0 + BT <= d);
+  const long nfull = kend > kbeg ? (kend - kbeg) / BK : 0;
+  if (kbeg < kend) {
+    if (cols_in) {
+      if (diag) gram_slabs<BT, NT, true, false>(H, yv, d, kbeg, kend, nfull, row0, col0, lds, acc);
+      else gram_slabs<BT, NT, false, false>(H, yv, d, kbeg, kend, nfull, row0, col0, lds, acc);
+    } else {
+      if (diag) gram_slabs<BT, NT, true, true>(H, yv, d, kbeg, kend, nfull, row0, col0, lds, acc);
+      else gram_slabs<BT, NT, false, true>(H, yv, d, kbeg, kend, nfull, row0, col0, lds, acc);
+    }
+  }
+}
+
+}
diff --git a/csrc/kernels/chain_blocked.hip b/csrc/kernels/chain_blocked.hip
--- a/csrc/kernels/chain_blocked.hip
+++ b/csrc/kernels/chain_blocked.hip
@@ -104,7 +104,7 @@
   }
 }
 
-template <int DB, bool SYS, bool TL, bool DYN, bool HALO, bool SWEEP, class PA>
+template <int DB, bool SYS, bool TL, bool DYN, bool HALO, bool SWEEP, bool IMG, class PA>
 __device__ __forceinline__ void chain_blocked_body(const PA& a) {
   constexpr int QT = DB / 4;
   extern __shared__ __attribute__((aligned(16))) double lds[];
@@ -200,7 +200,15 @@
   const int odist = u < s0 - ra ? (s0 - ra) - u : (u > e0 - ra ? u - (e0 - ra) : 0);
   const bool solver = active && odist <= (head ? 2 * k - 1 : 2 * k - 2);
   double Mq[4][QT];
-  quad_load<QT>(Mq, a.Minv + ((long)li * a.nvar + a.deg_to_var[deg]) * (long)d * d, d, active);
+  if constexpr (IMG) {
+    quad_load_image<QT>(Mq, a.minv_pad + ((long)li * a.nvar + a.deg_to_var[deg]) * (long)(512 * ((QT + 1) / 2)));
+#pragma unroll
+    for (int r = 0; r < 4; ++r)
+#pragma unroll
+      for (int t = 0; t < QT; ++t) Mq[r][t] = active ? Mq[r][t] : 0.0;
+  } else {
+    quad_load<QT>(Mq, a.Minv + ((long)li * a.nvar + a.deg_to_var[deg]) * (long)d * d, d, active);
+  }
   auto solve = [&](double r) -> double {
     const double y = quad_gemv<QT>(Mq, in ? r : 0.0, myx);
     return in ? y : 0.0;
@@ -565,23 +573,23 @@
 
 typedef __attribute__((address_space(4))) PersistArgs SweepArgs;
 
-template <int DB, bool SYS, bool TL, bool DYN = false, bool HALO = false>
+template <int DB, bool SYS, bool TL, bool DYN = false, bool HALO = false, bool IMG = false>
 __global__ void __launch_bounds__(64 * MAXW) chain_blocked_kernel(PersistArgs a) {
-  chain_blocked_body<DB, SYS, TL, DYN, HALO, false>(a);
+  chain_blocked_body<DB, SYS, TL, DYN, HALO, false, IMG>(a);
 }
 
 template <int DB>
 __global__ void __launch_bounds__(64 * MAXW) chain_blocked_sweep_kernel(const PersistArgs* __restrict__ batch, int nb) {
   const int j = (int)(blockIdx.x & 7u);
   if (j >= nb) return;
-  chain_blocked_body<DB, false, false, false, false, true>(*(const SweepArgs*)(batch + j));
+  chain_blocked_body<DB, false, false, false, false, true, false>(*(const SweepArgs*)(batch + j));
 }
 
 template <int DB>
 __global__ void __launch_bounds__(64 * MAXW) chain_blocked_dyn_sweep_kernel(const PersistArgs* __restrict__ batch, int nb) {
   const int j = (int)(blockIdx.x & 7u);
   if (j >= nb) return;
-  chain_blocked_body<DB, false, false, true, false, true>(*(const SweepArgs*)(batch + j));
+  chain_blocked_body<DB, false, false, true, false, true, false>(*(const SweepArgs*)(batch + j));
 }
 
 constexpr int PWW = 8;
@@ -1024,6 +1032,9 @@
     else fn = a.d <= 32 ? (const void*)chain_blocked_kernel<32, true, false> : (const void*)chain_blocked_kernel<52, true, false>;
   } else {
     if (tl) fn = a.d <= 32 ? (const void*)chain_blocked_kernel<32, false, true> : (const void*)chain_blocked_kernel<52, false, true>;
+    else if (a.minv_pad)
+      fn = a.d <= 32 ? (const void*)chain_blocked_kernel<32, false, false, false, false, true>
+                     : (const void*)chain_blocked_kernel<52, false, false, false, false, true>;
     else fn = a.d <= 32 ? (const void*)chain_blocked_kernel<32, false, false> : (const void*)chain_blocked_kernel<52, false, false>;
   }
   {
diff --git a/csrc/kernels/gram.hip b/csrc/kernels/gram.hip
--- a/csrc/kernels/gram.hip
+++ b/csrc/kernels/gram.hip
@@ -1,10 +1,11 @@
 #include <stdlib.h>
 #include "gadmm_common.h"
+#include "gram_tile.h"
 
 namespace {
 
-constexpr int BK = 16;
-constexpr int PAD = 16;
+using gram_tile::BK;
+using gram_tile::GramTile;
 
 __device__ __forceinline__ void tri_of(int t, int& ti, int& tj) {
   ti = (int)((sqrt(8.0 * t + 1.0) - 1.0) * 0.5);
@@ -46,159 +47,6 @@
 }
 
 template <int BT, int NT>
-struct GramTile {
-  static constexpr int NWAVE = NT / 64;
-  static constexpr int WR = NWAVE / 2;
-  static constexpr int WTR = BT / WR;
-  static constexpr int WTC = BT / 2;
-  static constexpr int TMR = WTR / 16;
-  static constexpr int TMC = WTC / 16;
-  static constexpr int LDSROW = BT + PAD;
-  static constexpr int PER_THREAD = BK * BT / NT;
-};
-
-template <int BT, int NT, bool DIAG, bool CLAMP>
-__device__ __forceinline__ void gram_slabs(const double* __restrict__ H, const double* __restrict__ yv, int d,
-                                           long kbeg, long kend, long nfull, int row0, int col0,
-                                           double (*lds)[2 * BK * GramTile<BT, NT>::LDSROW],
-                                           f64x4 (&acc)[GramTile<BT, NT>::TMR][GramTile<BT, NT>::TMC]) {
-  using T = GramTile<BT, NT>;
-  const int tid = threadIdx.x, lane = tid & 63, wid = tid >> 6;
-  const int wr = wid >> 1, wc = wid & 1;
-  double ri[T::PER_THREAD], rj[T::PER_THREAD];
-  auto fetch_in = [&](long k0) {
-#pragma unroll
-    for (int p = 0; p < T::PER_THREAD / 2; ++p) {
-      const int e2 = tid + NT * p;
-      const int r = e2 / (BT / 2), c = (e2 % (BT / 2)) * 2;
-      const double* src = H + (k0 + r) * (long)d;
-      ri[2 * p] = src[row0 + c];
-      ri[2 * p + 1] = src[row0 + c + 1];
-      if constexpr (!DIAG) {
-        rj[2 * p] = src[col0 + c];
-        rj[2 * p + 1] = src[col0 + c + 1];
-      }
-    }
-  };
-  auto fetch_cl = [&](long k0) {
-#pragma unroll
-    for (int p = 0; p < T::PER_THREAD / 2; ++p) {
-      const int e2 = tid + NT * p;
-      const int r = e2 / (BT / 2), c = (e2 % (BT / 2)) * 2;
-      const long k = k0 + r;
-      const long kk = k < kend ? k : (kend - 1);
-      const double yk = yv[kk];
-      const bool kin = k < kend;
-#pragma unroll
-      for (int q = 0; q < 2; ++q) {
-        const int ca = row0 + c + q, cb = col0 + c + q;
-        const double va = H[kk * d + (ca < d ? ca : d - 1)];
-        ri[2 * p + q] = kin ? (ca < d ? va : (ca == d ? yk : 0.0)) : 0.0;
-        if constexpr (!DIAG) {
-          const double vb = H[kk * d + (cb < d ? cb : d - 1)];
-          rj[2 * p + q] = kin ? (cb < d ? vb : (cb == d ? yk : 0.0)) : 0.0;
-        }
-      }
-    }
-  };
-  double yr[CLAMP ? T::PER_THREAD / 2 : 1];
-  long kraw = 0;
-  auto fetch_raw = [&](long k0) {
-    kraw = k0;
-#pragma unroll
-    for (int p = 0; p < T::PER_THREAD / 2; ++p) {
-      const int e2 = tid + NT * p;
-      const int r = e2 / (BT / 2), c = (e2 % (BT / 2)) * 2;
-      const long k = k0 + r;
-      const long kk = k < kend ? k : (kend - 1);
-      yr[p] = yv[kk];
-#pragma unroll
-      for (int q = 0; q < 2; ++q) {
-        const int ca = row0 + c + q, cb = col0 + c + q;
-        ri[2 * p + q] = H[kk * d + (ca < d ? ca : d - 1)];
-        if constexpr (!DIAG) rj[2 * p + q] = H[kk * d + (cb < d ? cb : d - 1)];
-      }
-    }
-  };
-  auto select_raw = [&]() {
-#pragma unroll
-    for (int p = 0; p < T::PER_THREAD / 2; ++p) {
-      const int e2 = tid + NT * p;
-      const int r = e2 / (BT / 2), c = (e2 % (BT / 2)) * 2;
-      const bool kin = kraw + r < kend;
-#pragma unroll
-      for (int q = 0; q < 2; ++q) {
-        const int ca = row0 + c + q, cb = col0 + c + q;
-        ri[2 * p + q] = kin ? (ca < d ? ri[2 * p + q] : (ca == d ? yr[p] : 0.0)) : 0.0;
-        if constexpr (!DIAG) rj[2 * p + q] = kin ? (cb < d ? rj[2 * p + q] : (cb == d ? yr[p] : 0.0)) : 0.0;
-      }
-    }
-  };
-  auto stash = [&](int buf) {
-    if constexpr (CLAMP) select_raw();
-    double* Si = lds[buf];
-    double* Sj = lds[buf] + BK * T::LDSROW;
-#pragma unroll
-    for (int p = 0; p < T::PER_THREAD / 2; ++p) {
-      const int e2 = tid + NT * p;
-      const int r = e2 / (BT / 2), c = (e2 % (BT / 2)) * 2;
-      *reinterpret_cast<double2*>(Si + r * T::LDSROW + c) = make_double2(ri[2 * p], ri[2 * p + 1]);
-      if constexpr (!DIAG) *reinterpret_cast<double2*>(Sj + r * T::LDSROW + c) = make_double2(rj[2 * p], rj[2 * p + 1]);
-    }
-  };
-  auto mma = [&](int buf) {
-    const double* Ci = lds[buf];
-    const double* Cb = DIAG ? Ci : lds[buf] + BK * T::LDSROW;
-#pragma unroll
-    for (int ks = 0; ks < BK / 4; ++ks) {
-      const int kr = ks * 4 + (lane >> 4);
-      double a[T::TMR], b[T::TMC];
-#pragma unroll
-      for (int t = 0; t < T::TMR; ++t) a[t] = Ci[kr * T::LDSROW + wr * T::WTR + t * 16 + (lane & 15)];
-#pragma unroll
-      for (int t = 0; t < T::TMC; ++t) b[t] = Cb[kr * T::LDSROW + wc * T::WTC + t * 16 + (lane & 15)];
-#pragma unroll
-      for (int x = 0; x < T::TMR; ++x)
-#pragma unroll
-        for (int yq = 0; yq < T::TMC; ++yq)
-          acc[x][yq] = __builtin_amdgcn_mfma_f64_16x16x4f64(a[x], b[yq], acc[x][yq], 0, 0, 0);
-    }
-  };
-
-  auto fetch = [&](long k0) {
-    if constexpr (CLAMP) fetch_raw(k0);
-    else fetch_in(k0);
-  };
-  int cur = 0;
-  long k0 = kbeg;
-  if (nfull > 0) {
-    fetch(k0);
-    stash(0);
-    lds_barrier();
-    for (long s = 1; s < nfull; ++s) {
-      fetch(k0 + BK);
-      mma(cur);
-      stash(cur ^ 1);
-      lds_barrier();
-      cur ^= 1;
-      k0 += BK;
-    }
-    mma(cur);
-    lds_barrier();
-    cur ^= 1;
-    k0 += BK;
-  }
-  for (; k0 < kend; k0 += BK) {
-    if constexpr (CLAMP) fetch_raw(k0);
-    else fetch_cl(k0);
-    stash(cur);
-    lds_barrier();
-    mma(cur);
-    cur ^= 1;
-  }
-}
-
-template <int BT, int NT>
 __global__ void __launch_bounds__(NT)
 gram_aug_kernel(const double* __restrict__ X, const double* __restrict__ Y, int m, int d,
                 int ntiles, int ksplit, long rows_per_split,
@@ -230,22 +78,7 @@
   const int D = d + 1;
 
   f64x4 acc[T::TMR][T::TMC];
-#pragma unroll
-  for (int a = 0; a < T::TMR; ++a)
-#pragma unroll
-    for (int b = 0; b < T::TMC; ++b) acc[a][b] = f64x4{0.0, 0.0, 0.0, 0.0};
-
-  const bool cols_in = (row0 + BT <= d) && (diag || col0 + BT <= d);
-  const long nfull = kend > kbeg ? (kend - kbeg) / BK : 0;
-  if (kbeg < kend) {
-    if (cols_in) {
-      if (diag) gram_slabs<BT, NT, true, false>(H, yv, d, kbeg, kend, nfull, row0, col0, lds, acc);
-      else gram_slabs<BT, NT, false, false>(H, yv, d, kbeg, kend, nfull, row0, col0, lds, acc);
-    } else {
-      if (diag) gram_slabs<BT, NT, true, true>(H, yv, d, kbeg, kend, nfull, row0, col0, lds, acc);
-      else gram_slabs<BT, NT, false, true>(H, yv, d, kbeg, kend, nfull, row0, col0, lds, acc);
-    }
-  }
+  gram_tile::gram_tile_acc<BT, NT>(H, yv, d, kbeg, kend, row0, col0, diag, lds, acc);
 
 #pragma unroll
   for (int x = 0; x < T::TMR; ++x)
diff --git a/csrc/kernels/setup_small.hip b/csrc/kernels/setup_small.hip
--- /dev/null
+++ b/csrc/kernels/setup_small.hip
@@ -0,0 +1,173 @@
+#include <stddef.h>
+
+#include "gadmm_common.h"
+#include "gadmm_chain.h"
+#include "gj_reg64.h"
+#include "gram_tile.h"
+
+extern "C" int gadmm_gram_pick_ksplit(int N, int m, int d);
+extern "C" int gadmm_chain_blocked_pad_dim(int d);
+
+namespace {
+
+constexpr int NT = 512, NW = NT / 64;
+
+struct SetupSmallArgs {
+  const double* X;
+  const double* Y;
+  const double* shift;
+  double* A;
+  double* B;
+  double* YY;
+  double* Minv;
+  double* minv_pad;
+  int* status;
+  int m, d, nvar, pad_qt;
+  int reset, start_iter, pending;
+  ChainCtl* ctl;
+  double* theta;
+  double* mu;
+  double* trace;
+  double* part;
+  long n_theta, n_mu, n_trace, n_part;
+  long long* stamp;
+};
+
+template <int BT>
+__global__ void __launch_bounds__(NT) setup_small_kernel(SetupSmallArgs a) {
+  using T = gram_tile::GramTile<BT, NT>;
+  static_assert(T::LDS_DOUBLES >= gj_reg64::MS_DOUBLES, "the result tile aliases the Gram staging buffers");
+  extern __shared__ __attribute__((aligned(16))) double lds[];
+  double* Ms = lds;
+  double (*colv)[65] = reinterpret_cast<double (*)[65]>(lds + T::LDS_DOUBLES);
+  const int n = blockIdx.x, v = blockIdx.y, N = gridDim.x;
+  const int d = a.d, m = a.m, D = d + 1;
+  const int tid = threadIdx.x, lane = tid & 63, wid = tid >> 6;
+  const bool first = v == 0;
+
+  if (a.reset && first) {
+    const long i0 = (long)n * NT + tid, step = (long)N * NT;
+    for (long i = i0; i < a.n_theta; i += step) a.theta[i] = 0.0;
+    for (long i = i0; i < a.n_mu; i += step) a.mu[i] = 0.0;
+    for (long i = i0; i < a.n_part; i += step) a.part[i] = 0.0;
+    const double qnan = __longlong_as_double(0x7ff8000000000000ll);
+    for (long i = i0; i < a.n_trace; i += step) a.trace[i] = qnan;
+    if (i0 == 0) {
+      a.ctl->iter = a.start_iter;
+      a.ctl->done = 0;
+      a.ctl->conv_iter = 0;
+      a.ctl->pending = a.pending;
+      a.ctl->ticket = 0u;
+      a.ctl->monitored = a.start_iter - 1;
+      a.ctl->inner_fail = 0;
+    }
+  }
+
+  f64x4 acc[T::TMR][T::TMC];
+  gram_tile::gram_tile_acc<BT, NT>(a.X + (long)n * m * d, a.Y + (long)n * m, d, 0, m, 0, 0, true,
+                                   reinterpret_cast<double (*)[2 * gram_tile::BK * T::LDSROW]>(lds), acc);
+  __syncthreads();
+  const int wr = wid >> 1, wc = wid & 1;
+  double* An = a.A + (long)n * d * d;
+#pragma unroll
+  for (int x = 0; x < T::TMR; ++x)
+#pragma unroll
+    for (int yq = 0; yq < T::TMC; ++yq)
+#pragma unroll
+      for (int reg = 0; reg < 4; ++reg) {
+        const int r = wr * T::WTR + x * 16 + (lane >> 4) + 4 * reg;
+        const int c = wc * T::WTC + yq * 16 + (lane & 15);
+        const double val = acc[x][yq][reg];
+        if (r >= D || c >= D || c > r) continue;
+        if (r < d && c < d) {
+          Ms[r * 65 + c] = val;
+          Ms[c * 65 + r] = val;
+          if (first) {
+            An[(long)r * d + c] = val;
+            An[(long)c * d + r] = val;
+          }
+        } else if (first) {
+          if (c < d) a.B[(long)n * d + c] = val;
+          else a.YY[n] = val;
+        }
+      }
+  __syncthreads();
+
+  constexpr int NC = 64 / NW;
+  const double s = a.shift[n * a.nvar + v];
+  double h[NC];
+#pragma unroll
+  for (int c = 0; c < NC; ++c) {
+    const int j = wid + NW * c;
+    h[c] = (lane < d && j < d) ? Ms[lane * 65 + j] + (lane == j ? s : 0.0) : 0.0;
+  }
+  const bool bad = gj_reg64::pivots<NW>(h, d, colv);
+  if (tid == 0 && bad && a.status) atomicExch(a.status, 1);
+  const long mat = (long)n * a.nvar + v;
+  gj_reg64::write_out<NW>(h, d, Ms, a.Minv + mat * d * d);
+  if (a.minv_pad) {
+    const int n_el = 512 * ((a.pad_qt + 1) / 2);
+    double* img = a.minv_pad + mat * n_el;
+    for (int e = tid; e < n_el; e += NT) {
+      const int blk = e >> 7, l = (e & 127) >> 1;
+      const int t = 2 * (blk >> 2) + (e & 1), r = blk & 3;
+      const int row = (l & 15) + 16 * r, col = (l >> 4) + 4 * t;
+      img[e] = (row < d && col < d && t < a.pad_qt) ? 0.5 * (Ms[row * 65 + col] + Ms[col * 65 + row]) : 0.0;
+    }
+  }
+  if (a.reset && first && n == 0 && tid == 0 && a.stamp)
+    *a.stamp = (long long)__builtin_amdgcn_s_memrealtime();
+}
+
+}
+
+extern "C" {
+
+int gadmm_setup_small_ok(int N, int m, int d) {
+  if (N < 1 || m < 1 || d < 1 || d > 64 || m > 256) return 0;
+  return gadmm_gram_pick_ksplit(N, m, d) == 1 ? 1 : 0;
+}
+
+int gadmm_setup_small_f64(const double* X, const double* Y, int N, int m, int d, const double* shift, int nvar,
+                          double* A, double* B, double* YY, double* Minv, double* minv_pad, int* status, int reset,
+                          ChainCtl* ctl, int start_iter, int pending, double* theta, long n_theta, double* mu,
+                          long n_mu, double* trace, long n_trace, double* part, long n_part, long long* stamp,
+                          hipStream_t st) {
+  if (N <= 0) return 0;
+  if (m < 1 || d < 1 || d > 64 || nvar < 1 || !X || !Y || !shift || !A || !B || !YY || !Minv) {
+    gadmm_set_error("setup_small: needs 1 <= d <= 64, m >= 1 and every Gram / inverse buffer (d=%d, m=%d)", d, m);
+    return -1;
+  }
+  if (minv_pad && d > 52) {
+    gadmm_set_error("setup_small: the padded inverse image exists for d <= 52 (d=%d)", d);
+    return -1;
+  }
+  if (reset && (!ctl || (n_theta > 0 && !theta) || (n_mu > 0 && !mu) || (n_trace > 0 && !trace) ||
+                (n_part > 0 && !part))) {
+    gadmm_set_error("setup_small: the state reset needs the control block and every state buffer");
+    return -1;
+  }
+  SetupSmallArgs a;
+  a.X = X, a.Y = Y, a.shift = shift, a.A = A, a.B = B, a.YY = YY, a.Minv = Minv, a.minv_pad = minv_pad;
+  a.status = status, a.m = m, a.d = d, a.nvar = nvar;
+  a.pad_qt = minv_pad ? gadmm_chain_blocked_pad_dim(d) / 4 : 0;
+  a.reset = reset ? 1 : 0, a.start_iter = start_iter, a.pending = pending;
+  a.ctl = ctl, a.theta = theta, a.mu = mu, a.trace = trace, a.part = part;
+  a.n_theta = n_theta, a.n_mu = n_mu, a.n_trace = n_trace, a.n_part = n_part;
+  a.stamp = stamp;
+  if (d + 1 <= 64) {
+    const size_t shm = (size_t)(gram_tile::GramTile<64, NT>::LDS_DOUBLES + gj_reg64::COLV_DOUBLES) * sizeof(double);
+    hipLaunchKernelGGL(setup_small_kernel<64>, dim3(N, nvar), dim3(NT), shm, st, a);
+  } else {
+    const size_t shm = (size_t)(gram_tile::GramTile<128, NT>::LDS_DOUBLES + gj_reg64::COLV_DOUBLES) * sizeof(double);
+    static_assert((gram_tile::GramTile<128, NT>::LDS_DOUBLES + gj_reg64::COLV_DOUBLES) * sizeof(double) <= 160 * 1024,
+                  "the d = 64 tile fits in LDS");
+    GADMM_CHECK(hipFuncSetAttribute((const void*)setup_small_kernel<128>, hipFuncAttributeMaxDynamicSharedMemorySize,
+                                    (int)shm));
+    hipLaunchKernelGGL(setup_small_kernel<128>, dim3(N, nvar), dim3(NT), shm, st, a);
+  }
+  GADMM_CHECK(hipGetLastError());
+  return 0;
+}
+
+}
diff --git a/csrc/kernels/spd_inverse.hip b/csrc/kernels/spd_inverse.hip
--- a/csrc/kernels/spd_inverse.hip
+++ b/csrc/kernels/spd_inverse.hip
@@ -1,4 +1,5 @@
 #include "gadmm_common.h"
+#include "gj_reg64.h"
 #include <stdlib.h>
 
 namespace {
@@ -90,18 +91,12 @@
     if (inj) o[i * d + j] = 0.5 * (M[i * d + j] + M[j * d + i]);
 }
 
-__device__ __forceinline__ double readlane_f64(double v, int l) {
-  const long long b = __double_as_longlong(v);
-  const int lo = __builtin_amdgcn_readlane((int)b, l), hi = __builtin_amdgcn_readlane((int)(b >> 32), l);
-  return __longlong_as_double(((long long)hi << 32) | (unsigned)lo);
-}
-
 template <int NW>
 __global__ void __launch_bounds__(64 * NW)
 spd_inverse_reg64_kernel(const double* __restrict__ A, const double* __restrict__ shift, int d, int nvar,
                          double* __restrict__ out, int* __restrict__ status) {
   constexpr int NC = 64 / NW;
-  __shared__ double Ms[64 * 65];
+  __shared__ double Ms[gj_reg64::MS_DOUBLES];
   __shared__ double colv[2][65];
   const int n = blockIdx.x, v = blockIdx.y;
   const double s = shift[n * nvar + v];
@@ -113,45 +108,9 @@
     const int j = w + NW * c;
     h[c] = (i < d && j < d) ? An[i * d + j] + (i == j ? s : 0.0) : 0.0;
   }
-  if (w == 0) {
-    colv[0][i] = h[0];
-    const double p0 = 1.0 / readlane_f64(h[0], 0);
-    if (i == 0) colv[0][64] = p0;
-  }
-  __syncthreads();
-  bool bad = false;
-  for (int k = 0; k < d; ++k) {
-    const double* cb = colv[k & 1];
-    const double pk = cb[k], aik = cb[i], p = cb[64];
-    bad |= !(pk > 0.0);
-#pragma unroll
-    for (int c = 0; c < NC; ++c) {
-      const int j = w + NW * c;
-      const double mkj = readlane_f64(h[c], k) * p;
-      double val = h[c];
-      if (j == k) val = (i == k) ? p : -aik * p;
-      else if (i == k) val = mkj;
-      else val -= aik * mkj;
-      h[c] = val;
-    }
-    const int kn = k + 1;
-    if (kn < d && w == kn % NW) {
-      double nxt = 0.0;
-#pragma unroll
-      for (int c = 0; c < NC; ++c) nxt = (c == kn / NW) ? h[c] : nxt;
-      colv[kn & 1][i] = nxt;
-      const double pn = 1.0 / readlane_f64(nxt, kn);
-      if (i == 0) colv[kn & 1][64] = pn;
-    }
-    __syncthreads();
-  }
+  const bool bad = gj_reg64::pivots<NW>(h, d, colv);
   if (threadIdx.x == 0 && bad && status) atomicExch(status, 1);
-#pragma unroll
-  for (int c = 0; c < NC; ++c) Ms[i * 65 + w + NW * c] = h[c];
-  __syncthreads();
-  double* o = out + ((long)n * nvar + v) * d * d;
-  for (int r = w; r < d; r += NW)
-    if (i < d) o[r * d + i] = 0.5 * (Ms[r * 65 + i] + Ms[i * 65 + r]);
+  gj_reg64::write_out<NW>(h, d, Ms, out + ((long)n * nvar + v) * d * d);
 }
 
 }
diff --git a/gadmm_amd/algorithms/gadmm.py b/gadmm_amd/algorithms/gadmm.py
--- a/gadmm_amd/algorithms/gadmm.py
+++ b/gadmm_amd/algorithms/gadmm.py
@@ -525,7 +525,7 @@
         _timing.host_stamp("native:early_draw")
     try:
         if eng is not None and refresh:
-            eng.refresh(model.X, model.y)
+            eng.refresh(model.X, model.y, defer=True)
             _timing.host_stamp("native:refresh")
         if eng is None:
             eng = NativeChainEngine(model.X, model.y, local_ids, n_total, kind, rho=rho, obj0=obj0, tol=tol,
diff --git a/gadmm_amd/engine/chain_engine.py b/gadmm_amd/engine/chain_engine.py
--- a/gadmm_amd/engine/chain_engine.py
+++ b/gadmm_amd/engine/chain_engine.py
@@ -292,11 +292,39 @@
     def _kernel_minv(self):
         return getattr(self, "Mpk", None) if self.d > 256 else self.Minv
 
-    def refresh(self, X_loc: torch.Tensor, y_loc: torch.Tensor):
+    @staticmethod
+    def _fused_on() -> bool:
+        return getenv("GADMM_FUSED_SETUP", "1") != "0"
+
+    def _fused_setup(self, reset=None):
+        fast = self._refresh_fast
+        self._setup_pending = False
+        if reset is None:
+            tail = (0, None, 0, 0, None, 0, None, 0, None, 0, None, 0, None)
+        else:
+            tail = (1, self.ctl.data_ptr(), int(reset[0]), int(reset[1]), self.theta.data_ptr(), self.theta.numel(),
+                    self.mu.data_ptr(), self.mu.numel(), self.trace.data_ptr(), self.trace.numel(),
+                    self.part.data_ptr(), self.part.numel(), self.t0stamp.data_ptr())
+        native.check(fast[2].gadmm_setup_small_f64(*(fast[5] + tail + (self.stream.cuda_stream,))), "setup_small_f64")
+        self._minv_version = getattr(self, "_minv_version", 0) + 1
+        if fast[5][11] is not None and fast[6] is getattr(self, "_minv_pad", None):
+            self._minv_pad_version = self._minv_version
+
+    def _flush_setup(self):
+        if getattr(self, "_setup_pending", False):
+            self._fused_setup(None)
+
+    def refresh(self, X_loc: torch.Tensor, y_loc: torch.Tensor, defer: bool = False):
         if getattr(self, "_shared_inverses", False):
             raise RuntimeError("this engine's inverses belong to a shared table: refresh its owner")
         fast = getattr(self, "_refresh_fast", None)
         if fast is not None and fast[0] is X_loc and fast[1] is y_loc:
+            if fast[5] is not None and self._fused_on():
+                if defer:
+                    self._setup_pending = True
+                else:
+                    self._fused_setup(None)
+                return
             lib, g_args, i_args = fast[2], fast[3], fast[4]
             native.check(lib.gadmm_gram_f64(*g_args), "gram_f64")
             native.check(lib.gadmm_spd_inverse_small_f64(*i_args), "spd_inverse_small_f64")
@@ -321,8 +349,21 @@
                       self.yy.data_ptr(), self._refresh_ws.data_ptr() if self._refresh_ws is not None else None, st)
             i_args = (self.A.data_ptr(), self._shifts.data_ptr(), N, d, int(self._shifts.shape[1]),
                       self.Minv.data_ptr(), self._inv_status.data_ptr(), st)
-            self._refresh_fast = (X_loc, y_loc, lib, g_args, i_args)
-            return self.refresh(X_loc, y_loc)
+            s_args = None
+            if d <= 64 and hasattr(lib, "gadmm_setup_small_f64") and int(lib.gadmm_setup_small_ok(N, m, d)):
+                nv = int(self._shifts.shape[1])
+                if d <= 52 and getattr(self, "_minv_pad", None) is None:
+                    with torch.cuda.stream(self.stream):
+                        self._minv_pad = torch.zeros((N * nv, int(lib.gadmm_chain_blocked_pad_len(d))),
+                                                     dtype=torch.float64, device=self.device)
+                    self._minv_pad_version = -1
+                pad = self._minv_pad.data_ptr() if (d <= 52 and self._minv_pad.is_contiguous()) else None
+                s_args = (X_loc.data_ptr(), y_loc.data_ptr(), N, m, d, self._shifts.data_ptr(), nv,
+                          self.A.data_ptr(), self.b.data_ptr(), self.yy.data_ptr(), self.Minv.data_ptr(), pad,
+                          self._inv_status.data_ptr())
+            self._refresh_fast = (X_loc, y_loc, lib, g_args, i_args, s_args, getattr(self, "_minv_pad", None))
+            return self.refresh(X_loc, y_loc, defer)
+        self._setup_pending = False
         with torch.cuda.stream(self.stream):
             if self.model == "linear":
                 gram(X_loc, y_loc, out=(self.A, self.b, self.yy))
@@ -331,9 +372,14 @@
                 self.X.copy_(X_loc)
                 self.Y.copy_(y_loc)
 
+    def refresh_reset(self, X_loc: torch.Tensor, y_loc: torch.Tensor, start_iter: int = 1, pending: int = 0):
+        self.refresh(X_loc, y_loc, defer=True)
+        self.reset(start_iter, pending)
+
     def set_rho(self, rho: float):
         if getattr(self, "_shared_inverses", False):
             raise RuntimeError("this engine's inverses belong to a shared table: rho is fixed")
+        self._flush_setup()
         self.rho = float(rho)
         if self.model == "linear":
             with torch.cuda.stream(self.stream):
@@ -419,6 +465,11 @@
         if self.rres is not None and zero_state:
             with torch.cuda.stream(self.stream):
                 self.rres.zero_()
+        if getattr(self, "_setup_pending", False):
+            if zero_state:
+                self._fused_setup((start_iter, pending))
+                return
+            self._fused_setup(None)
         if zero_state:
             native.check(self.lib.gadmm_chain_reset_state_stamp(
                 self.ctl.data_ptr(), int(start_iter), int(pending), self.theta.data_ptr(), self.theta.numel(),
@@ -438,6 +489,7 @@
 
     def run(self, stop_iter: int = 0, use_graph: bool = True, block: Optional[int] = None) -> EngineRun:
         self._tr_valid = False
+        self._flush_setup()
         st = native.RunStats()
         blk = self.block if block is None else int(block)
         if blk > self.ring and self.nranks > 1:
@@ -691,6 +743,9 @@
                 self._blk_tab = torch.zeros((ng * 4,), dtype=torch.int32, device=self.device)
         pa.blk_k, pa.blk_len, pa.blk_pw = plan[0], plan[1], plan[3]
         pa.blk_tab = self._blk_tab.data_ptr()
+        if not dynamic and plan[3] == 1 and self._fused_on() and getattr(self, "_minv_pad", None) is not None \
+                and self._minv_pad_version == self._minv_version:
+            pa.minv_pad = self._minv_pad.data_ptr()
 
     def _queue_readback(self, fetch_trace: bool) -> bool:
         nt = self.trace.numel()
@@ -713,6 +768,7 @@
         return done, conv, nxt
 
     def prepare_blocked(self, lag: int = 4, timeout_s: float = 20.0, start_iter: int = 1):
+        self._flush_setup()
         if self.nranks != 1 or self.n_local != self.n_total or not self.persistent_eligible(None):
             raise ValueError("persistent kernel not eligible for this engine/config")
         plan = self.blocked_plan(None) if self.model == "linear" else None
@@ -767,6 +823,7 @@
 
     def prepare_blocked_dyn(self, starts: np.ndarray, P: np.ndarray, lag: int = 4, timeout_s: float = 20.0,
                             start_iter: int = 1, pending_in: int = 0, hard_stop: int = 0, cont: bool = False):
+        self._flush_setup()
         if self.nranks != 1 or not self.dynamic_eligible(None):
             raise ValueError("dynamic persistent kernel not eligible for this engine/config")
         plan = self.blocked_plan(None) if self.model == "linear" else None
@@ -787,6 +844,7 @@
         return EngineRun(conv, done, nxt - start_iter, 1, wall_ms, 0, 0, 0, 0)
 
     def adopt_stream(self, stream: torch.cuda.Stream):
+        self._flush_setup()
         stream.wait_stream(self.stream)
         self.stream = stream
         self._desc.stream = stream.cuda_stream
@@ -800,6 +858,7 @@
                        fetch_trace: bool = False, blocked_dyn: Optional[bool] = None,
                        on_enqueued=None) -> EngineRun:
         _timing.host_stamp("rp:start")
+        self._flush_setup()
         if self.quant is not None:
             if fabric is not None or epochs is not None or pending_in or hard_stop or cont or timeline_iters:
                 raise RuntimeError("persistent Q kernel: a static chain on one GPU, one launch per solve")
diff --git a/gadmm_amd/engine/multigpu.py b/gadmm_amd/engine/multigpu.py
--- a/gadmm_amd/engine/multigpu.py
+++ b/gadmm_amd/engine/multigpu.py
@@ -189,8 +189,12 @@
                 raise RuntimeError("blocked kernel: a hand-off timed out")
             pay = self.blk.exchange_bytes_per_solve(it)
             return SolveOut(it, done, pay, 2 * pay, self.blk.monitor_bytes_per_solve(it))
-        self.eng.refresh(self.X, self.y)
-        self.eng.reset()
+        rr = getattr(self.eng, "refresh_reset", None)
+        if rr is not None:
+            rr(self.X, self.y)
+        else:
+            self.eng.refresh(self.X, self.y)
+            self.eng.reset()
         if self.persistent:
             r = self.eng.run_persistent(fabric=self.fab, timeout_s=self.timeout_s)
         else:
diff --git a/gadmm_amd/ops/native.py b/gadmm_amd/ops/native.py
--- a/gadmm_amd/ops/native.py
+++ b/gadmm_amd/ops/native.py
@@ -214,6 +214,11 @@
         "gadmm_memcpy_h2d_async": (c_int, [c_void_p, c_void_p, ctypes.c_size_t, c_void_p]),
         "gadmm_memcpy_d2h_async": (c_int, [c_void_p, c_void_p, ctypes.c_size_t, c_void_p]),
         "gadmm_readback_d2h": (c_int, [c_void_p, c_void_p, ctypes.c_size_t, c_void_p]),
+        "gadmm_setup_small_ok": (c_int, [c_int, c_int, c_int]),
+        "gadmm_setup_small_f64": (c_int, [c_void_p, c_void_p, c_int, c_int, c_int, c_void_p, c_int, c_void_p,
+                                          c_void_p, c_void_p, c_void_p, c_void_p, c_void_p, c_int, c_void_p, c_int,
+                                          c_int, c_void_p, c_long, c_void_p, c_long, c_void_p, c_long, c_void_p,
+                                          c_long, c_void_p, c_void_p]),
         "gadmm_chain_blocked_tab_granules": (c_long, [c_int, c_int, c_int]),
         "gadmm_chain_blocked_tab_granules_dyn": (c_long, [c_int, c_int, c_int]),
         "gadmm_epoch_tables": (c_int, [c_void_p, c_int, c_int, c_void_p, c_int, c_void_p, c_void_p]),
```

After: 1.690 ms, median of 6. Within noise of the previous version (-0.7%).
